# TSultanov/cfd-demo

Measured on AMD Instinct MI355X. Metric: cell-updates/s (Poisson iter) + ms/timestep, 4096² grid, 1/2/4/8 GPU, higher is better.
Workload: dtype f32

## Files before the change

cfd-demo_amd/cfdamd/__init__.py:

```python
from __future__ import annotations

import ctypes as C
import enum
from dataclasses import dataclass
from typing import List, Optional

import numpy as np

from . import _lib
from ._lib import (CFD_ENONFINITE, CfdError, CfdGrid, CfdParams, CfdResiduals, CfdState, check,
                   load)

__all__ = [
    "VelocityScheme", "InletProfile", "PressureSolver", "BoundaryKind", "Cylinder", "Grid",
    "SimulationParams", "Residuals", "SimSnapshot", "Model", "SimulationControlHandle",
    "CfdError", "default_grid", "cavity_grid", "rccl_unique_id", "device_count", "load", "LocalHub",
    "VisualizationMode", "CFD_ENONFINITE",
]


class VelocityScheme(enum.IntEnum):
    FirstOrder = 0
    SecondOrder = 1

# ... 222 lines not shown
        p = params._c()
        check("cfd_set_params", load().cfd_set_params(self._hh(), C.byref(p)))
        self.params = params

    def get_snapshot(self) -> SimSnapshot:
        su, sv, sp = self._sizes()
        u, v, p = (np.empty(n, np.float32) for n in (su, sv, sp))
        dt = C.c_float()
        check("cfd_get_snapshot",
              load().cfd_get_snapshot(self._hh(), _fp(u), _fp(v), _fp(p), C.byref(dt)))
        return SimSnapshot(p=p, u=u, v=v, dt=float(dt.value))

    def get_residuals(self) -> Residuals:
        r = CfdResiduals()
        check("cfd_get_residuals", load().cfd_get_residuals(self._hh(), C.byref(r)))
        return Residuals(int(r.simulation_step), float(r.simulation_time), float(r.dt),
                         float(r.p), float(r.u), float(r.v), float(r.step_time_s),
                         int(r.piso_substeps), int(r.jacobi_sweeps_total))

    def get_state(self) -> dict:
        su, sv, sp = self._sizes()
        arrs = {k: np.empty(n, np.float32) for k, n in
                (("u", su), ("v", sv), ("p", sp), ("u_star", su), ("v_star", sv),
                 ("p_prime", sp), ("rhs", sp))}
        st = CfdState(*(_fp(arrs[k]) for k in ("u", "v", "p", "u_star", "v_star", "p_prime",
                                               "rhs")))
        check("cfd_get_state", load().cfd_get_state(self._hh(), C.byref(st)))
        arrs.update(dt=np.float32(st.dt), simulation_time=np.float32(st.simulation_time),
                    simulation_step=int(st.simulation_step),
                    last_p_residual=np.float32(st.last_p_residual),
                    last_u_residual=np.float32(st.last_u_residual),
                    last_v_residual=np.float32(st.last_v_residual),
                    jacobi_sweeps_total=int(st.jacobi_sweeps_total))
        return arrs

    def set_state(self, **kw) -> None:
        cur = self.get_state()
        arrs = {}
        for k in ("u", "v", "p", "u_star", "v_star", "p_prime", "rhs"):
            a = kw.get(k, cur[k])
            arrs[k] = np.ascontiguousarray(a, dtype=np.float32)
            if arrs[k].size != cur[k].size:
                raise ValueError(f"{k}: expected {cur[k].size} values, got {arrs[k].size}")
        st = CfdState(*(_fp(arrs[k]) for k in ("u", "v", "p", "u_star", "v_star", "p_prime",
                                               "rhs")))
        st.dt = float(kw.get("dt", cur["dt"]))
        st.simulation_time = float(kw.get("simulation_time", cur["simulation_time"]))
        st.simulation_step = int(kw.get("simulation_step", cur["simulation_step"]))
        st.last_p_residual = float(kw.get("last_p_residual", cur["last_p_residual"]))
        st.last_u_residual = float(kw.get("last_u_residual", cur["last_u_residual"]))
        st.last_v_residual = float(kw.get("last_v_residual", cur["last_v_residual"]))
        st.jacobi_sweeps_total = int(kw.get("jacobi_sweeps_total", cur["jacobi_sweeps_total"]))
        check("cfd_set_state", load().cfd_set_state(self._hh(), C.byref(st)))

    def get_masks(self):
        su, sv, _ = self._sizes()
        mu, mv = np.empty(su, np.uint8), np.empty(sv, np.uint8)
        check("cfd_get_masks", load().cfd_get_masks(
            self._hh(), mu.ctypes.data_as(C.POINTER(C.c_uint8)),
            mv.ctypes.data_as(C.POINTER(C.c_uint8))))
        return mu, mv

    def profile_sweeps(self, n: int) -> float:
        ms = C.c_double()
        check("cfd_profile_sweeps", load().cfd_profile_sweeps(self._hh(), n, C.byref(ms)))
        return float(ms.value)

    def timing_begin(self) -> None:
        check("cfd_timing_begin", load().cfd_timing_begin(self._hh()))

    def timing_end(self):
        a, b, c, d = C.c_double(), C.c_uint64(), C.c_double(), C.c_uint64()
        check("cfd_timing_end", load().cfd_timing_end(self._hh(), C.byref(a), C.byref(b),
                                                      C.byref(c), C.byref(d)))
        return {"solve_ms": a.value, "sweeps": int(b.value), "step_ms": c.value,
                "steps": int(d.value)}

    def timing_phases(self, on: bool = True) -> None:
        check("cfd_timing_phases", load().cfd_timing_phases(self._hh(), 1 if on else 0))

    def timing_phase_ms(self) -> dict:
        a, b = C.c_double(), C.c_double()
        check("cfd_timing_phase_ms",
              load().cfd_timing_phase_ms(self._hh(), C.byref(a), C.byref(b)))
        return {"predict_ms": a.value, "finish_ms": b.value}

    def timing_exchange_ms(self) -> dict:
        a, n = C.c_double(), C.c_uint64()
        check("cfd_timing_exchange_ms",
              load().cfd_timing_exchange_ms(self._hh(), C.byref(a), C.byref(n)))
        return {"exchange_ms": a.value, "exchanges": int(n.value)}

    @property
    def kernel_config(self) -> dict:
        fd, tb = C.c_int(), C.c_int()
        check("cfd_get_kernel_config",
              load().cfd_get_kernel_config(self._hh(), C.byref(fd), C.byref(tb)))
        return {"fastdiv": fd.value, "temporal": tb.value}

    def render(self, mode: "VisualizationMode" = VisualizationMode.Pressure):
        img = np.empty((self.nyl, self.grid.nx, 4), np.uint8)
        mm = np.empty(2, np.float32)
        check("cfd_render", load().cfd_render(
            self._hh(), int(mode), img.ctypes.data_as(C.POINTER(C.c_uint8)), _fp(mm)))
        return img, (float(mm[0]), float(mm[1]))

    def derive_field(self, mode: "VisualizationMode"):
        out = np.empty((self.nyl, self.grid.nx), np.float32)
        mm = np.empty(2, np.float32)
        check("cfd_derive_field", load().cfd_derive_field(self._hh(), int(mode), _fp(out), _fp(mm)))
        return out, (float(mm[0]), float(mm[1]))

    def launches_per_solve(self) -> int:
        tmax = self.kernel_config["temporal"]
        iters = self.params.jacobi_iters
        hg = self.halo_depth if self.n_ranks > 1 else 0
        T, lo, hi, ex = C.c_int(), C.c_int(), C.c_int(), C.c_int()
        it = n = 0
        while it < iters:
            check("cfd_plan_block", load().cfd_plan_block(
                self.j0, self.nyl, self.grid.ny, hg, it, tmax, iters, C.byref(T), C.byref(lo),
                C.byref(hi), C.byref(ex)))
            it += T.value
            n += 1
        return n

    @property
    def jacobi_kernel(self) -> dict:
        kind, name = C.c_int(), C.create_string_buffer(96)
        check("cfd_get_jacobi_kernel",
              load().cfd_get_jacobi_kernel(self._hh(), C.byref(kind), name, 96))
        return {"kind": kind.value, "name": name.value.decode()}

    def jacobi_geometry(self, persist: bool = True) -> dict:
        v = [C.c_int32() for _ in range(4)]
        check("cfd_get_jacobi_geometry",
              load().cfd_get_jacobi_geometry(self._hh(), int(bool(persist)), *(C.byref(x) for x in v)))
        return dict(lds_pad=v[0].value, wgs_per_cu=v[1].value, wave_cols=v[2].value,
                    segments=v[3].value)

    @property
    def persist_steals(self) -> int:
        n = C.c_uint64()
        check("cfd_get_persist_steals", load().cfd_get_persist_steals(self._hh(), C.byref(n)))
        return int(n.value)

    @property
    def persist_sums(self) -> int:
        n = C.c_uint64()
        check("cfd_get_persist_sums", load().cfd_get_persist_sums(self._hh(), C.byref(n)))
        return int(n.value)

    @property
    def comm_calls(self) -> int:
        n = C.c_uint64()
        check("cfd_get_comm_calls", load().cfd_get_comm_calls(self._hh(), C.byref(n)))
        return int(n.value)

    @property
    def recoveries(self) -> int:
        n = C.c_uint64()
        check("cfd_get_recoveries", load().cfd_get_recoveries(self._hh(), C.byref(n)))
        return int(n.value)

    @property
    def resident_solves(self) -> int:
        n = C.c_uint64()
        check("cfd_get_resident_solves", load().cfd_get_resident_solves(self._hh(), C.byref(n)))
        return int(n.value)

    @property
    def persist_blocks(self) -> int:
        n = C.c_int()
        check("cfd_get_persist_blocks", load().cfd_get_persist_blocks(self._hh(), C.byref(n)))
        return n.value

    @property
    def comm_size(self) -> int:
        n = C.c_int()
        check("cfd_get_comm_size", load().cfd_get_comm_size(self._hh(), C.byref(n)))
        return int(n.value)

    @property
    def halo_depth(self) -> int:
        return int(load().cfd_get_halo_depth(self._hh()))

    def run(self) -> "SimulationControlHandle":
        return SimulationControlHandle(self)

    def _hh(self):
        if self._runner is not None:
            raise CfdError("Model", -4, "the model is owned by a running SimulationControlHandle; "
                                        "stop() it first")
        return self._h

    def close(self) -> None:
        r = getattr(self, "_runner", None)
        if r is not None:
            r.stop()
        if getattr(self, "_h", None) and self._h.value:
            load().cfd_destroy(self._h)
            self._h = C.c_void_p()

    def __del__(self):
        try:
            self.close()
        except Exception:
            pass


class SimulationControlHandle:

    def __init__(self, model: Model):
        self._model = model
        self._r = C.c_void_p()
        check("cfd_run_start", load().cfd_run_start(model._hh(), C.byref(self._r)))
        model._runner = self

    def _live(self):
        if not self._r.value:
            raise CfdError("cfd_run", -4, "runner stopped")
        return self._r

    def stop(self):
        if self._r.value:
            check("cfd_run_stop", load().cfd_run_stop(self._r))
            self._r = C.c_void_p()
            if self._model._runner is self:
                self._model._runner = None

    def join(self, timeout=None):
        self.stop()

    def status(self):
        buf = C.create_string_buffer(256)
        rc = load().cfd_run_status(self._live(), buf, 256)
        return rc, buf.value.decode()

    @property
    def steps(self) -> int:
        return int(load().cfd_run_steps(self._live()))

    def get_last_available_snapshot(self) -> Optional[SimSnapshot]:
        su, sv, sp = self._model._sizes()
        u, v, p = (np.empty(n, np.float32) for n in (su, sv, sp))
        dt, paused, avail = C.c_float(), C.c_int(), C.c_int()
        check("cfd_run_last_snapshot", load().cfd_run_last_snapshot(
            self._live(), _fp(u), _fp(v), _fp(p), C.byref(dt), C.byref(paused), C.byref(avail)))
        if not avail.value:
            return None
        return SimSnapshot(p=p, u=u, v=v, dt=float(dt.value), paused=bool(paused.value))

    def get_new_log_messages(self) -> List[Residuals]:
        out: List[Residuals] = []
        buf = (CfdResiduals * 256)()
        n = C.c_int()
        while True:
            check("cfd_run_new_residuals",
                  load().cfd_run_new_residuals(self._live(), buf, 256, C.byref(n)))
            for r in buf[:n.value]:
                out.append(Residuals(int(r.simulation_step), float(r.simulation_time),
                                     float(r.dt), float(r.p), float(r.u), float(r.v),
                                     float(r.step_time_s), int(r.piso_substeps),
                                     int(r.jacobi_sweeps_total)))
            if n.value < 256:
                return out

    def request_snapshot(self):
        check("cfd_run_request_snapshot", load().cfd_run_request_snapshot(self._live()))

    def set_params(self, params: SimulationParams):
        p = params._c()
        check("cfd_run_set_params", load().cfd_run_set_params(self._live(), C.byref(p)))
        self._model.params = params

    def pause(self):
        check("cfd_run_pause", load().cfd_run_pause(self._live()))

    def resume(self):
        check("cfd_run_resume", load().cfd_run_resume(self._live()))

    def __del__(self):
        try:
            self.stop()
        except Exception:
            pass
```

cfd-demo_amd/cfdamd/_lib.py:

```python
from __future__ import annotations

import ctypes as C
import os

PKG_DIR = os.path.dirname(os.path.abspath(__file__))
ROOT = os.path.dirname(PKG_DIR)
LIB_PATH = os.environ.get("CFD_LIB") or os.path.join(ROOT, "lib", "libcfd_amd.so")

EXPORTS = [
    "cfd_default_params", "cfd_default_grid", "cfd_create", "cfd_rccl_unique_id",
    "cfd_create_sharded", "cfd_local_hub_create", "cfd_local_hub_destroy",
    "cfd_create_sharded_local", "cfd_device_count", "cfd_get_comm_size", "cfd_get_slab", "cfd_update", "cfd_update_n", "cfd_piso_step",
    "cfd_pressure_solve", "cfd_run_phase", "cfd_set_params", "cfd_get_snapshot",
    "cfd_get_residuals", "cfd_get_state", "cfd_set_state", "cfd_get_masks", "cfd_synchronize",
    "cfd_profile_sweeps", "cfd_timing_begin", "cfd_timing_end", "cfd_timing_phases",
    "cfd_timing_phase_ms", "cfd_timing_exchange_ms", "cfd_get_halo_depth",
    "cfd_get_kernel_config", "cfd_get_jacobi_kernel", "cfd_get_persist_blocks", "cfd_get_persist_steals", "cfd_get_persist_sums", "cfd_get_recoveries", "cfd_get_comm_calls", "cfd_get_resident_solves", "cfd_get_jacobi_geometry", "cfd_plan_slab", "cfd_plan_sweep", "cfd_plan_halo", "cfd_plan_block", "cfd_plan_overlap",
    "cfd_render", "cfd_derive_field", "cfd_last_error", "cfd_abi_version", "cfd_destroy",
    "cfd_get_config", "cfd_run_start", "cfd_run_stop", "cfd_run_pause", "cfd_run_resume",
    "cfd_run_set_params", "cfd_run_request_snapshot", "cfd_run_last_snapshot",
    "cfd_run_new_residuals", "cfd_run_status", "cfd_run_steps",
    "cfd_polygon_new", "cfd_polygon_new_rect", "cfd_polygon_new_regular", "cfd_polygon_add_hole",
    "cfd_polygon_contains_point", "cfd_polygon_intersects_aabb",
    "cfd_polygon_edges_intersect_aabb", "cfd_polygon_bounding_box",
    "cfd_polygon_bounding_square", "cfd_polygon_edges", "cfd_polygon_destroy",
    "cfd_geom_do_intersect", "cfd_geom_segment_intersection", "cfd_geom_intersect_quad_edge",
    "cfd_tesselate", "cfd_quadtree_size", "cfd_quadtree_nodes", "cfd_quadtree_destroy",
    "cfd_mesh_from_quadtree", "cfd_mesh_sizes", "cfd_mesh_cells", "cfd_mesh_neighbors",
    "cfd_mesh_intersections", "cfd_mesh_full_bounding_box", "cfd_mesh_build_ms",
    "cfd_mesh_destroy",
]


class CfdGrid(C.Structure):
    _fields_ = [("nx", C.c_uint64), ("ny", C.c_uint64), ("lx", C.c_float), ("ly", C.c_float),
                ("has_cylinder", C.c_int32), ("cylinder_x", C.c_float),
                ("cylinder_y", C.c_float), ("cylinder_radius", C.c_float)]


class CfdParams(C.Structure):
    _fields_ = [("dt", C.c_float), ("viscosity", C.c_float),
                ("target_inlet_velocity", C.c_float), ("velocity_scheme", C.c_int32),
                ("inlet_profile", C.c_int32), ("pressure_solver", C.c_int32),
                ("jacobi_iters", C.c_int32), ("corrector_passes", C.c_int32),
                ("tol_enabled", C.c_int32), ("p_tol", C.c_float), ("bc_kind", C.c_int32)]


class CfdResiduals(C.Structure):
    _fields_ = [("simulation_step", C.c_uint64), ("simulation_time", C.c_float),
                ("dt", C.c_float), ("p", C.c_float), ("u", C.c_float), ("v", C.c_float),
                ("step_time_s", C.c_double), ("piso_substeps", C.c_uint32),
                ("jacobi_sweeps_total", C.c_uint64)]


FP = C.POINTER(C.c_float)


class CfdState(C.Structure):
    _fields_ = [("u", FP), ("v", FP), ("p", FP), ("u_star", FP), ("v_star", FP),
                ("p_prime", FP), ("rhs", FP), ("dt", C.c_float), ("simulation_time", C.c_float),
                ("simulation_step", C.c_uint64), ("last_p_residual", C.c_float),
                ("last_u_residual", C.c_float), ("last_v_residual", C.c_float),
                ("jacobi_sweeps_total", C.c_uint64)]


class CfdPoint(C.Structure):
    _fields_ = [("x", C.c_double), ("y", C.c_double)]


class CfdAabb(C.Structure):
    _fields_ = [("center", CfdPoint), ("half_width", C.c_double), ("half_height", C.c_double)]


CFD_EINVAL, CFD_EHIP, CFD_ERCCL, CFD_ESTATE, CFD_ENONFINITE, CFD_ETIMEOUT = -1, -2, -3, -4, -5, -6


class CfdError(RuntimeError):
    def __init__(self, fn: str, code: int, msg: str):
        super().__init__(f"{fn} failed ({code}): {msg}")
        self.code = code


_lib = None


def load():
    global _lib
    if _lib is not None:
        return _lib
    if not os.path.exists(LIB_PATH):
        raise RuntimeError(
            f"HIP library {LIB_PATH} not built: run `make -C {ROOT}` "
            "(or __graft_entry__.build()). There is no CPU fallback.")
    L = C.CDLL(LIB_PATH)
    vp, i32, f32 = C.c_void_p, C.c_int, C.c_float
    sig = {
        "cfd_default_params": (None, [C.POINTER(CfdParams)]),
        "cfd_default_grid": (None, [C.POINTER(CfdGrid)]),
        "cfd_create": (i32, [C.POINTER(CfdGrid), C.POINTER(CfdParams), i32, C.POINTER(vp)]),
        "cfd_rccl_unique_id": (i32, [C.c_char_p]),
        "cfd_create_sharded": (i32, [C.POINTER(CfdGrid), C.POINTER(CfdParams), i32, i32, i32,
                                     C.c_char_p, C.POINTER(vp)]),
        "cfd_local_hub_create": (vp, [i32]),
        "cfd_local_hub_destroy": (None, [vp]),
        "cfd_create_sharded_local": (i32, [C.POINTER(CfdGrid), C.POINTER(CfdParams), i32, i32,
                                           i32, vp, C.POINTER(vp)]),
        "cfd_device_count": (i32, [C.POINTER(i32)]),
        "cfd_get_comm_size": (i32, [vp, C.POINTER(i32)]),
        "cfd_get_slab": (i32, [vp, C.POINTER(C.c_uint64), C.POINTER(C.c_uint64)]),
        "cfd_update": (i32, [vp]),
        "cfd_update_n": (i32, [vp, i32]),
        "cfd_piso_step": (i32, [vp, f32]),
        "cfd_pressure_solve": (i32, [vp, FP]),
        "cfd_run_phase": (i32, [vp, i32, f32]),
        "cfd_set_params": (i32, [vp, C.POINTER(CfdParams)]),
        "cfd_get_snapshot": (i32, [vp, FP, FP, FP, FP]),
        "cfd_get_residuals": (i32, [vp, C.POINTER(CfdResiduals)]),
        "cfd_get_state": (i32, [vp, C.POINTER(CfdState)]),
        "cfd_set_state": (i32, [vp, C.POINTER(CfdState)]),
        "cfd_get_masks": (i32, [vp, C.POINTER(C.c_uint8), C.POINTER(C.c_uint8)]),
        "cfd_synchronize": (i32, [vp]),
        "cfd_profile_sweeps": (i32, [vp, i32, C.POINTER(C.c_double)]),
        "cfd_timing_begin": (i32, [vp]),
        "cfd_timing_end": (i32, [vp, C.POINTER(C.c_double), C.POINTER(C.c_uint64),
                                 C.POINTER(C.c_double), C.POINTER(C.c_uint64)]),
        "cfd_timing_phases": (i32, [vp, i32]),
        "cfd_timing_phase_ms": (i32, [vp, C.POINTER(C.c_double), C.POINTER(C.c_double)]),
        "cfd_timing_exchange_ms": (i32, [vp, C.POINTER(C.c_double), C.POINTER(C.c_uint64)]),
        "cfd_get_halo_depth": (i32, [vp]),
        "cfd_get_kernel_config": (i32, [vp, C.POINTER(i32), C.POINTER(i32)]),
        "cfd_get_jacobi_kernel": (i32, [vp, C.POINTER(i32), C.c_char_p, C.c_size_t]),
        "cfd_get_persist_blocks": (i32, [vp, C.POINTER(i32)]),
        "cfd_get_persist_steals": (i32, [vp, C.POINTER(C.c_uint64)]),
        "cfd_get_persist_sums": (i32, [vp, C.POINTER(C.c_uint64)]),
        "cfd_get_recoveries": (i32, [vp, C.POINTER(C.c_uint64)]),
        "cfd_get_comm_calls": (i32, [vp, C.POINTER(C.c_uint64)]),
        "cfd_get_resident_solves": (i32, [vp, C.POINTER(C.c_uint64)]),
        "cfd_get_jacobi_geometry": (i32, [vp, i32, C.POINTER(i32), C.POINTER(i32), C.POINTER(i32),
                                          C.POINTER(i32)]),
        "cfd_plan_slab": (i32, [C.c_uint64, i32, i32, C.POINTER(C.c_uint64),
                                C.POINTER(C.c_uint64)]),
        "cfd_plan_sweep": (i32, [i32, i32, i32, i32, i32, i32, C.POINTER(i32), C.POINTER(i32),
                                 C.POINTER(i32)]),
        "cfd_plan_halo": (i32, [i32, i32, i32, i32, i32, C.POINTER(i32)]),
        "cfd_plan_overlap": (i32, [i32, i32, i32, i32, i32, i32, C.POINTER(i32)]),
        "cfd_plan_block": (i32, [i32, i32, i32, i32, i32, i32, i32, C.POINTER(i32),
                                 C.POINTER(i32), C.POINTER(i32), C.POINTER(i32)]),
        "cfd_render": (i32, [vp, i32, C.POINTER(C.c_uint8), FP]),
        "cfd_derive_field": (i32, [vp, i32, FP, FP]),
        "cfd_last_error": (C.c_char_p, []),
        "cfd_abi_version": (i32, []),
        "cfd_destroy": (None, [vp]),
        "cfd_get_config": (i32, [vp, C.POINTER(CfdGrid), C.POINTER(CfdParams)]),
        "cfd_run_start": (i32, [vp, C.POINTER(vp)]),
        "cfd_run_stop": (i32, [vp]),
        "cfd_run_pause": (i32, [vp]),
        "cfd_run_resume": (i32, [vp]),
        "cfd_run_set_params": (i32, [vp, C.POINTER(CfdParams)]),
        "cfd_run_request_snapshot": (i32, [vp]),
        "cfd_run_last_snapshot": (i32, [vp, FP, FP, FP, FP, C.POINTER(i32), C.POINTER(i32)]),
        "cfd_run_new_residuals": (i32, [vp, C.POINTER(CfdResiduals), i32, C.POINTER(i32)]),
        "cfd_run_status": (i32, [vp, C.c_char_p, C.c_size_t]),
        "cfd_run_steps": (C.c_uint64, [vp]),
        "cfd_polygon_new": (i32, [C.POINTER(CfdPoint), C.c_size_t, C.POINTER(C.c_uint64),
                                  C.c_size_t, C.POINTER(vp), C.POINTER(i32)]),
        "cfd_polygon_new_rect": (i32, [C.c_double] * 4 + [C.POINTER(vp)]),
        "cfd_polygon_new_regular": (i32, [CfdPoint, C.c_double, C.c_size_t, C.c_double,
                                          C.POINTER(vp)]),
        "cfd_polygon_add_hole": (i32, [vp, vp, C.POINTER(i32)]),
        "cfd_polygon_contains_point": (i32, [vp, CfdPoint, C.POINTER(i32)]),
        "cfd_polygon_intersects_aabb": (i32, [vp, C.POINTER(CfdAabb), C.POINTER(i32)]),
        "cfd_polygon_edges_intersect_aabb": (i32, [vp, C.POINTER(CfdAabb), C.POINTER(i32)]),
        "cfd_polygon_bounding_box": (i32, [vp, C.POINTER(CfdAabb)]),
        "cfd_polygon_bounding_square": (i32, [vp, C.POINTER(CfdAabb)]),
        "cfd_polygon_edges": (i32, [vp, C.POINTER(CfdPoint), C.c_size_t, C.POINTER(C.c_size_t)]),
        "cfd_polygon_destroy": (None, [vp]),
        "cfd_geom_do_intersect": (i32, [CfdPoint] * 4 + [C.POINTER(i32)]),
        "cfd_geom_segment_intersection": (i32, [CfdPoint] * 4 + [C.POINTER(CfdPoint),
                                                                 C.POINTER(i32)]),
        "cfd_geom_intersect_quad_edge": (i32, [CfdPoint, C.c_double, C.c_double, CfdPoint,
                                               CfdPoint, C.POINTER(CfdPoint), C.POINTER(i32)]),
        "cfd_tesselate": (i32, [vp, C.c_double, C.c_double, C.POINTER(vp)]),
        "cfd_quadtree_size": (i32, [vp, C.POINTER(C.c_uint64), C.POINTER(C.c_uint64)]),
        "cfd_quadtree_nodes": (i32, [vp, C.POINTER(CfdAabb), C.POINTER(C.c_int64)]),
        "cfd_quadtree_destroy": (None, [vp]),
        "cfd_mesh_from_quadtree": (i32, [vp, vp, i32, C.POINTER(vp)]),
        "cfd_mesh_sizes": (i32, [vp, C.POINTER(C.c_uint64)]),
        "cfd_mesh_cells": (i32, [vp] + [C.POINTER(C.c_double)] * 4),
        "cfd_mesh_neighbors": (i32, [vp, i32, C.POINTER(C.c_uint64), C.POINTER(C.c_uint64)]),
        "cfd_mesh_intersections": (i32, [vp, C.POINTER(C.c_uint64), C.POINTER(CfdPoint)]),
        "cfd_mesh_full_bounding_box": (i32, [vp, C.POINTER(CfdAabb)]),
        "cfd_mesh_build_ms": (i32, [vp, C.POINTER(C.c_double)]),
        "cfd_mesh_destroy": (None, [vp]),
    }
    for name, (res, args) in sig.items():
        if os.environ.get("CFD_LIB") and not hasattr(L, name):
            continue
        fn = getattr(L, name)
        fn.restype = res
        fn.argtypes = args
    _lib = L
    return L


def check(fn: str, rc: int):
    if rc != 0:
        msg = load().cfd_last_error()
        raise CfdError(fn, rc, msg.decode() if msg else "")
```

cfd-demo_amd/csrc/cfd_device.h:

```cpp
#pragma once
#include "cfd_internal.h"

#include <algorithm>

namespace cfd {
namespace {

inline int cdiv(long a, long b) { return (int)((a + b - 1) / b); }


constexpr int kBlock = 256;
typedef unsigned int u32x4 __attribute__((ext_vector_type(4)));

__device__ __forceinline__ float dt_of(const Ctl *c, float dt_override) {
    return __builtin_isnan(dt_override) ? c->dt : dt_override;
}

__device__ __forceinline__ bool pass_off(const Ctl *c, int pass) {
    return pass >= 0 && c->go[pass] == 0;
}

__device__ __forceinline__ float wave_max(float m) {
#pragma unroll
    for (int o = 32; o > 0; o >>= 1) m = fmaxf(m, __shfl_xor(m, o, 64));
    return m;
}

__device__ __forceinline__ void publish_max(uint32_t *set, int key, float m) {
    if (m > 0.0f) atomicMax(&set[(key & (kResSlots - 1)) * kResStride], __float_as_uint(m));
}

__device__ __forceinline__ bool nonfinite(float x) { return !(fabsf(x) <= 3.40282347e38f); }
__device__ __forceinline__ void flag_nonfinite(Ctl *c, bool bad) {
    if (bad) atomicOr(&c->red[4], 1u);
}

__device__ __forceinline__ float read_max(const uint32_t *set, uint32_t base) {
    const int lane = (int)threadIdx.x & 63;
    const float v = lane < kResSlots ? __uint_as_float(set[lane * kResStride]) : 0.0f;
    return fmaxf(wave_max(v), __uint_as_float(base));
}

__device__ __forceinline__ int xcd_block(const Geom &g) {
    const int b = (int)blockIdx.x, G = (int)gridDim.x;
    if (!g.xcd_remap) return b;
    const int per = G >> 3;
    if (b >= (per << 3)) return b;
    return (b & 7) * per + (b >> 3);
}

__device__ __forceinline__ float from_left(float x) {
    return __builtin_bit_cast(
        float, __builtin_amdgcn_update_dpp(0, __builtin_bit_cast(int, x), 0x138, 0xf, 0xf, true));
}
__device__ __forceinline__ float from_right(float x) {
    return __builtin_bit_cast(
        float, __builtin_amdgcn_update_dpp(0, __builtin_bit_cast(int, x), 0x130, 0xf, 0xf, true));
}

constexpr float kDivGuardMin = 0x1p-96f;
template <int FAST>
__device__ __forceinline__ float fdiv(float x, float c, float r) {
    if (FAST == 1) return x * r;
    if (FAST == 2) {
        const float q0 = x * r;
        const float q = __builtin_fmaf(__builtin_fmaf(-q0, c, x), r, q0);
        return __builtin_isfinite(q0) ? q : q0;
    }
    if (FAST == 3) {
        const float q0 = x * r;
        const float qc = __builtin_fmaf(__builtin_fmaf(-q0, c, x), r, q0);
        float q = __builtin_isfinite(q0) && x != 0.0f ? qc : q0;
        const bool ok = __builtin_fabsf(x) >= kDivGuardMin || x == 0.0f;
        if (__builtin_expect(!__all(ok), 0)) q = ok ? q : x / c;
        return q;
    }
    return x / c;
}

template <int SP>
__device__ __forceinline__ float sdiv(float x, float c, float r) {
    return SP ? x * r : x / c;
}

typedef float f2 __attribute__((ext_vector_type(2)));

template <int FAST>
__device__ __forceinline__ f2 fdiv2(f2 x, float c, float r) {
    if (FAST == 1) return x * r;
    return (f2){fdiv<FAST>(x.x, c, r), fdiv<FAST>(x.y, c, r)};
}

__device__ __forceinline__ void solve_finalize_body(const Geom &g, const Fields &f, int pass,
                                                    int iters, int check_break, int flips,
                                                    int exact_flips) {
    Ctl *c = f.ctl;
    __shared__ int go_s;
    const int k_lo = g.tol_enabled ? 0 : (iters > 0 ? iters - 1 : 0);
    const int wv = (int)threadIdx.x >> 6, nw = (int)blockDim.x >> 6;
    for (int k = k_lo + wv; k < iters; k += nw) {
        uint32_t *set = f.err_slots + (size_t)k * kResSlots * kResStride;
        const float v = read_max(set, c->err[k]);
        if ((threadIdx.x & 63) < kResSlots) set[(threadIdx.x & 63) * kResStride] = 0u;
        if ((threadIdx.x & 63) == 0) c->err[k] = __float_as_uint(v);
    }
    __syncthreads();
    if (threadIdx.x == 0) {
        const int go = pass < 0 ? 1 : c->go[pass];
        if (go) {
            int n = iters;
            if (g.tol_enabled && iters > 0) {
                n = 1;
                while (n < iters && !(__uint_as_float(c->err[n - 1]) < g.p_tol)) ++n;
            }
            const float res = n > 0 ? __uint_as_float(c->err[n - 1]) : 0.0f;
            c->cur = (c->cur + (exact_flips == 2 ? c->spec_launches
                                : (g.tol_enabled && !exact_flips) ? n : flips)) & 1;
            c->last_p = res;
            c->red[5] = __float_as_uint(res);
            c->n_exec_last = (uint32_t)n;
            c->sweeps_total += (uint64_t)n;
        }
        if (pass >= 0 && pass + 1 <= kMaxPasses)
            c->go[pass + 1] = (go && !(check_break && g.tol_enabled && c->last_p < g.p_tol)) ? 1 : 0;
        if (exact_flips >= 2) c->spec_stop = c->spec_redo = c->spec_launch = c->spec_launches = 0;
        go_s = go;
    }
    __syncthreads();
    if (go_s)
        for (int k = threadIdx.x; k < iters; k += blockDim.x) c->err[k] = 0u;
}

template <int FAST>
__device__ __forceinline__ float4 jacobi_row4(const float4 &B, const float4 &C, const float4 &T,
                                              const float4 &Rh, float L0, float R3, float dx_sq,
                                              float dy_sq, float denom, float r_dx_sq,
                                              float r_dy_sq, float r_denom) {
    const f2 c01 = {C.x, C.y}, c23 = {C.z, C.w};
    const f2 h01 = __builtin_shufflevector(c01, c01, 1, 0) + (f2){L0, C.z};
    const f2 h23 = __builtin_shufflevector(c23, c23, 1, 0) + (f2){C.y, R3};
    const f2 v01 = (f2){T.x, T.y} + (f2){B.x, B.y};
    const f2 v23 = (f2){T.z, T.w} + (f2){B.z, B.w};
    const f2 hz01 = fdiv2<FAST>(h01, dx_sq, r_dx_sq), hz23 = fdiv2<FAST>(h23, dx_sq, r_dx_sq);
    const f2 vt01 = fdiv2<FAST>(v01, dy_sq, r_dy_sq), vt23 = fdiv2<FAST>(v23, dy_sq, r_dy_sq);
    const f2 pu01 = fdiv2<FAST>(hz01 + vt01 - (f2){Rh.x, Rh.y}, denom, r_denom);
    const f2 pu23 = fdiv2<FAST>(hz23 + vt23 - (f2){Rh.z, Rh.w}, denom, r_denom);
    const float omega = 0.75f;
    const float om1 = 1.0f - omega;
    const f2 n01 = omega * pu01 + om1 * c01;
    const f2 n23 = omega * pu23 + om1 * c23;
    return make_float4(n01.x, n01.y, n23.x, n23.y);
}

}
}
```

cfd-demo_amd/csrc/cfd_internal.h:

```cpp
#pragma once
#include <hip/hip_runtime.h>
#include <stdint.h>

#include "../../include/cfd.h"

namespace cfd {

constexpr int kGhostUV = 2;
constexpr int kMaxSweeps = 4096;
constexpr int kMaxPasses = 64;

constexpr int kResSlots = 32;
constexpr int kResStride = 16;
constexpr int kPersistFlagStride = 16;
constexpr int kPersistHeadLines = 21;
constexpr int kPersistBlockBits = 10;
static_assert((1 << kPersistBlockBits) > kMaxSweeps / 8, "persistent flag layout");
constexpr int kPersistMaxGroups = 16384;
constexpr size_t kPersistWords = (size_t)(kPersistMaxGroups + kPersistHeadLines) * kPersistFlagStride;
constexpr size_t kSlotWords = (size_t)(kMaxSweeps + 16) * kResSlots * kResStride + kPersistWords;

struct Ctl {
    float dt;
    float time;
    uint32_t step;
    float inlet;
    int32_t cur;
    uint32_t n_exec_last;
    float last_p;
    float res_u, res_v;
    uint32_t red[7];
    uint32_t nonfinite_step;
    uint32_t vis[2];
    uint32_t done;
    uint64_t sweeps_total;
    int32_t spec_stop, spec_redo, spec_launch, spec_launches;
    uint32_t spec_done;
    int32_t go[kMaxPasses + 1];
    uint32_t err[kMaxSweeps];
};

struct Geom {
    int32_t nx, ny;
    int32_t j0, nyl;
    int32_t hg;
    float dx, dy, nu, ly;
    float target_inlet;
    int32_t scheme, profile, bc_kind;
    int32_t tol_enabled;
    float p_tol;
    int32_t jacobi_iters;
    float dx_sq, dy_sq, denom;
    float r_dx_sq, r_dy_sq, r_denom;
    int32_t fastdiv;
    int32_t tb_rows;
    int32_t tb_bpc;
    int32_t n_cu;
    int32_t tb_kind;
    int32_t xcd_remap;
    float r_dx, r_dy, r_dxx, r_dyy;
    int32_t sp_pow2;
    int32_t pred_div;
    int32_t res_div;
};

struct Fields {
    float *u, *v, *u_old, *v_old, *u_star, *v_star;
    float *p, *rhs;
    float *pp[2];
    const uint8_t *mask_u, *mask_v;
    const int32_t *obs;
    uint32_t *err_slots;
    uint32_t *red_slots;
    uint32_t *vis_slots;
    int32_t n_obs;
    int32_t any_pmask;
    size_t u_alloc, v_alloc;
    float *u_alloc_base, *v_alloc_base, *u_old_base, *v_old_base, *u_star_base, *v_star_base;
    Ctl *ctl;
    uint32_t *host_nonfinite;
    uint32_t *host_progress;
    uint32_t *persist;
};

void launch_step_begin(const Geom &g, const Fields &f, int copy, hipStream_t s);
void launch_copy_star(const Geom &g, const Fields &f, int pass, hipStream_t s);
void launch_copy_star_div(const Geom &g, const Fields &f, int pass, float dt_override,
                          hipStream_t s);
void launch_u_predictor(const Geom &g, const Fields &f, float dt_override, hipStream_t s);
void launch_v_predictor(const Geom &g, const Fields &f, float dt_override, hipStream_t s);
void launch_predict(const Geom &g, const Fields &f, float dt_override, hipStream_t s);
bool predict_div_fused(const Geom &g, const Fields &f);
void launch_predict_div(const Geom &g, const Fields &f, float dt_override, hipStream_t s);
bool predict_march_ok(const Geom &g, const Fields &f);
void launch_predict_march(const Geom &g, const Fields &f, float dt_override, hipStream_t s,
                          bool set_inlet = false, int row_lo = 0, int row_hi = -1);
void launch_divergence(const Geom &g, const Fields &f, int pass, float dt_override,
                       hipStream_t s);
void launch_jacobi_sweep(const Geom &g, const Fields &f, int pass, int it, int row_lo,
                         int row_hi, int res, hipStream_t s);
void launch_jacobi_block(const Geom &g, const Fields &f, int pass, int it, int par, int T,
                         int out_lo, int out_hi, int res, hipStream_t s);
bool launch_jacobi_persist(const Geom &g, const Fields &f, int pass, int par0, int nblk,
                           int out_lo, int out_hi, uint32_t epoch, int res_it, hipStream_t s);
void lds_geometry8(const Geom &g, int out_lo, int out_hi, bool persist, int *pad, int *occ, int *nwc,
                   int *nseg);
void launch_tb1(const Geom &g, const Fields &f, int T, int pass, int it, int par, int out_lo,
                int out_hi, uint32_t *res_slots, hipStream_t s);
void launch_pipe4(const Geom &g, const Fields &f, int T, int pass, int it, int par, int out_lo,
                  int out_hi, uint32_t *res_slots, hipStream_t s);
void launch_pipe2(const Geom &g, const Fields &f, int T, int pass, int it, int par, int out_lo,
                  int out_hi, uint32_t *res_slots, hipStream_t s);
bool launch_lds_persist8(const Geom &g, const Fields &f, int pass, int par0, int nblk, int out_lo,
                         int out_hi, uint32_t epoch, uint32_t *rs, hipStream_t s);
void launch_lds(const Geom &g, const Fields &f, int T, int pass, int it, int par, int out_lo,
                int out_hi, uint32_t *res_slots, hipStream_t s, int mode = 0, int lag = 0);
void launch_jacobi_spec(const Geom &g, const Fields &f, int pass, int it, int par, int T,
                        int out_lo, int out_hi, hipStream_t s, int lag = 0);
void launch_spec_check(const Geom &g, const Fields &f, int pass, int it, int T, int par,
                       hipStream_t s);
bool launch_jacobi_resident(const Geom &g, const Fields &f, int pass, int iters, int fin,
                            int check_break, hipStream_t s);
bool jacobi_resident_geometry(const Geom &g, int *br, int *bc, int *tiles, int *wgs);
void launch_spec_align(const Geom &g, const Fields &f, int pass, int n, hipStream_t s);
void launch_jacobi_redo(const Geom &g, const Fields &f, int pass, int out_lo, int out_hi,
                        hipStream_t s, int last_it = 0, int last_par = 0, int last_T = 0);
void launch_fold_slots(uint32_t *dst, uint32_t *slots, int n, hipStream_t s);
void launch_vis_field(const Geom &g, const Fields &f, int mode, float *out, uint32_t *slots,
                      hipStream_t s);
void launch_vis_color(const Geom &g, const Fields &f, int mode, const float *field, uint32_t *px,
                      const uint32_t *keys, int has_cyl, float cx, float cy, float radius,
                      hipStream_t s);
void launch_verify_division(float c, float r, unsigned long long *dev_counts, hipStream_t s);
void launch_finalize_solve(const Geom &g, const Fields &f, int pass, int iters, int check_break,
                           int flips, hipStream_t s, int exact_flips = 0);

struct SorConst {
    double dx2, dy2, denom;
    double r_dx2, r_dy2, r_denom;
    int32_t fast;
};
struct MgLevel {
    float *a, *b, *rhs, *r;
    int32_t nx, ny;
    double dx2, dy2, denom;
    double r_dx2, r_dy2, r_denom;
    int32_t fast;
    int32_t ys, ye;
    int32_t lo, hi;
};
constexpr int kMgMaxLevels = 40;
void launch_sor_color(float *pp, const float *rhs, int nx, int ny, const SorConst &k, int color,
                      Ctl *ctl, uint32_t *err_slots, int pass, int it, int tol, float p_tol, int res,
                      hipStream_t s);
bool sor_fused_ok(int nx, int nrows);
void launch_sor_fused(float *pa, float *pb, const float *rhs, int nx, int ny, const SorConst &k,
                      Ctl *ctl, uint32_t *err_slots, int pass, int it, int tol, float p_tol, int res,
                      int row_lo, int row_hi, int j0, int lo_clamp, int hi_clamp, hipStream_t s);
void launch_fill_zero(float *p, size_t n, const Ctl *ctl, int pass, hipStream_t s);
void launch_mg_smooth(const MgLevel &L, const float *src, float *dst, const Ctl *ctl, int pass,
                      hipStream_t s);
void launch_mg_smooth5(const MgLevel &L, const float *src, float *dst, const Ctl *ctl, int pass,
                       hipStream_t s);
bool mg_smooth_wave_form();
void launch_mg_prolong_smooth5(const MgLevel &Cl, const float *e, const MgLevel &L, const float *src,
                               float *dst, const Ctl *ctl, int pass, hipStream_t s);
void launch_mg_smooth5_residual(const MgLevel &L, const float *src, float *dst, const Ctl *ctl,
                                int pass, hipStream_t s);
void launch_mg_residual(const MgLevel &L, const float *p, const Ctl *ctl, int pass, hipStream_t s);
void launch_mg_restrict(const MgLevel &F, const MgLevel &Cl, const Ctl *ctl, int pass, hipStream_t s);
void launch_mg_prolong_add(const MgLevel &Cl, const float *e, const MgLevel &F, float *p,
                           const Ctl *ctl, int pass, hipStream_t s);
void launch_mg_tail(const MgLevel *dev_levels, int s_level, int coarsest, float *a0, float *b0,
                    int fast, const Ctl *ctl, int pass, hipStream_t s);
void launch_mg_final_residual(const MgLevel &L, const float *p, uint32_t *slots, const Ctl *ctl,
                              int pass, hipStream_t s);
void launch_corrector(const Geom &g, const Fields &f, int pass, float dt_override,
                      hipStream_t s);
void launch_boundary(const Geom &g, const Fields &f, hipStream_t s);
void launch_correct_finish(const Geom &g, const Fields &f, float dt_override, hipStream_t s);
void launch_step_reduce(const Geom &g, const Fields &f, hipStream_t s);
bool correct_head_ok(const Geom &g, const Fields &f);
void launch_correct_head(const Geom &g, const Fields &f, int pass, float dt_override, bool has_next,
                         hipStream_t s);
void launch_step_finalize(const Geom &g, const Fields &f, hipStream_t s);
void launch_abort_to_red(const Fields &f, hipStream_t s);
void launch_abort_from_red(const Fields &f, hipStream_t s);

constexpr int kJacRowsPerWave = 16;
constexpr int kMaxTemporal = 8;
constexpr int kTbRowsPerWave = 32;
constexpr int kJacWavesPerBlock = 4;

}
```

cfd-demo_amd/csrc/cfd_jacobi_lds.h:

```cpp
#pragma once
#include <cmath>
#include <type_traits>

#include "cfd_device.h"

namespace cfd {
namespace {

constexpr int kLdsWaves = 4;
#ifndef CFD_LDS_SB
#define CFD_LDS_SB 0
#endif
#ifndef CFD_LDS_PD
#define CFD_LDS_PD 3
#endif
#ifndef CFD_LDS_DIAG
#define CFD_LDS_DIAG 0
#endif
#ifndef CFD_LDS_WPE
#define CFD_LDS_WPE 0
#endif
typedef unsigned int u32x2 __attribute__((ext_vector_type(2)));
#ifndef CFD_LDS_PRIO
#define CFD_LDS_PRIO 1
#endif
#ifndef CFD_LDS_COMPACT
#define CFD_LDS_COMPACT 0
#endif
#ifndef CFD_LDS_STAMP
#define CFD_LDS_STAMP 0
#endif
#if CFD_LDS_STAMP
constexpr int kStampWaves = 1 << 15;
__device__ unsigned long long g_lds_stamp[kStampWaves * 4];
#endif

#ifndef CFD_LDS_ST_AUX
#define CFD_LDS_ST_AUX 16
#endif

#ifndef CFD_LDS_LD_AUX
#define CFD_LDS_LD_AUX 0
#endif

#ifndef CFD_LDS_HOIST
#define CFD_LDS_HOIST 0
#endif

#ifndef CFD_LDS_SPLIT
#define CFD_LDS_SPLIT 1
#endif
constexpr int lds_gcd(int a, int b) { return b == 0 ? a : lds_gcd(b, a % b); }
constexpr int lds_off(int s, int T, int G) { return s <= 0 ? 0 : ((s - 1) * G) / T; }
constexpr int lds_nw(int G) { return G > 1 ? 4 : 3; }
constexpr int ring_depth(int T, int PD, int G) {
    const int nw = lds_nw(G);
    const int q = nw / lds_gcd(nw, PD) * PD;
    const int need = T + lds_off(T, T, G) + 1;
    return ((need + q - 1) / q) * q;
}

template <int T, int FAST, int MODE, bool SUMS = false>
struct LdsMarch {
    static constexpr bool RES = MODE == 1 || MODE == 5, SPEC = MODE == 2, REDO = MODE == 3;
    static constexpr bool PERSIST = MODE == 4 || MODE == 5;
#ifndef CFD_PROBE_NOTRACK
#define CFD_PROBE_NOTRACK 0
#endif
    static constexpr bool TRACK_IN = PERSIST && !SUMS && !CFD_PROBE_NOTRACK;
    static constexpr bool TRACK_OUT = PERSIST && !CFD_PROBE_NOTRACK;
    static_assert(!SUMS || FAST == 1, "SUMS: reciprocal multiply");
    static constexpr int PLD_AUX = PERSIST ? 16 : CFD_LDS_LD_AUX;
    static constexpr int PST_AUX = PERSIST ? 16 : CFD_LDS_ST_AUX;
    static constexpr int G = CFD_LDS_SPLIT;
    static constexpr int NW = lds_nw(G);
    static constexpr int PD = CFD_LDS_PD;
    static constexpr int OFFT = lds_off(T, T, G);
    static constexpr int D = ring_depth(T, PD, G);
    static constexpr int U = D;
    static constexpr int WARM = 2 * T + OFFT;
    static constexpr int H = (T + 1) / 2;
    static constexpr int OUTL = 64 - 2 * H;
    static constexpr int off(int s) { return lds_off(s, T, G); }
    static constexpr int start(int s) { return 2 * s + off(s); }
    static_assert(D % PD == 0 && D % NW == 0 && D >= T + OFFT + 1, "ring geometry");
    static_assert(G >= 1 && G <= T, "stage groups");

    f2 W[T][NW];
    f2 PQ[PD];
    f2 RQ[PD];
    f2 *ring;
    int lane;
    int k_first, S, lo_clamp, hi_clamp, nch, g_first, g_last, g_top, g_zero, row_bytes;
    int wbase;
    int ch, vo_ld, vo_st, abase, dir;
    bool e0, e1;
    float dx_sq, r_dx_sq, dy_sq, r_dy_sq, denom, r_denom;
    __amdgpu_buffer_rsrc_t rs_p, rs_r, rs_d;
    float m;
    float omax, imax, rmax;
    float mm[SPEC ? T : 1];
    int r0v, r1v;
    int nst;
    int nyl_;

    LdsMarch() = default;

    __device__ __forceinline__ int act(int vrow) const { return abase + dir * vrow; }

    template <int AUX = 0>
    __device__ __forceinline__ f2 ld(__amdgpu_buffer_rsrc_t rs, int vrow) const {
        if (CFD_LDS_DIAG & 1) return (f2){__int_as_float(vo_ld + vrow), 1.0f};
        vrow = vrow < k_first + S ? vrow : k_first + S - 1;
        int row = act(vrow);
        row = row < lo_clamp ? lo_clamp : (row > hi_clamp ? hi_clamp : row);
        const u32x2 v = __builtin_amdgcn_raw_buffer_load_b64(rs, vo_ld, (row - wbase) * row_bytes, AUX);
        return (f2){__uint_as_float(v.x), __uint_as_float(v.y)};
    }
    __device__ __forceinline__ void st(const f2 &x, int row) const {
        if (CFD_LDS_DIAG & 4) {
            asm volatile("" ::"v"(x.x), "v"(x.y));
            return;
        }
        const u32x2 v = {__float_as_uint(x.x), __float_as_uint(x.y)};
        __builtin_amdgcn_raw_buffer_store_b64(v, rs_d, vo_st, (row - wbase) * row_bytes, PST_AUX);
    }

    __device__ __forceinline__ f2 update(const f2 &B, const f2 &C, const f2 &Tp, const f2 &Rh) const {
        const float hx = C.y + from_left(C.y);
        const float hy = C.x + from_right(C.x);
        const f2 h = {hx, hy};
        const f2 v = Tp + B;
        f2 s;
        if constexpr (SUMS) {
            s = (h + v) * r_dx_sq;
        } else {
            const f2 hz = fdiv2<FAST>(h, dx_sq, r_dx_sq);
            const f2 vt = fdiv2<FAST>(v, dy_sq, r_dy_sq);
            s = hz + vt;
        }
        const f2 pu = fdiv2<FAST>(s - Rh, denom, r_denom);
        const float omega = 0.75f;
        const float om1 = 1.0f - omega;
        return omega * pu + om1 * C;
    }

    static constexpr int kCol = 1, kRow = 2;

    template <int E>
    __device__ __forceinline__ f2 stage(const f2 &B, const f2 &C, const f2 &Tp, const f2 &Rh) const {
        f2 o = update(B, C, Tp, Rh);
        if (E & kCol) {
            if (ch == 0) o.x = o.y;
            if (ch == nch - 1) o.y = 0.0f;
        }
        return o;
    }

    template <int V_, int GUARD, int E>
    __device__ __forceinline__ void slot(int v) {
        if ((GUARD == 2 || GUARD == 3) && v >= S) return;
        if (CFD_LDS_SB >= 1) __builtin_amdgcn_sched_barrier(0);
        const int k = k_first + v;
        W[0][V_ % NW] = PQ[V_ % PD];
        PQ[V_ % PD] = ld<PLD_AUX>(rs_p, k + PD);
        if (!(CFD_LDS_DIAG & 2))
            ring[(V_ % D) * 64 + lane] = RQ[V_ % PD];
        RQ[V_ % PD] = ld(rs_r, k + PD);
        f2 rhv[T];
        if (CFD_LDS_HOIST && !(CFD_LDS_DIAG & 2)) {
#pragma unroll
            for (int s = 1; s <= T; ++s) rhv[s - 1] = ring[((V_ - s - off(s) + 8 * D) % D) * 64 + lane];
        }
#pragma unroll
        for (int s = 1; s <= T; ++s) {
            if (GUARD == 0 && V_ < start(s)) continue;
            if (GUARD == 3 && v < start(s)) continue;
            if (CFD_LDS_SB >= 2 && s > 1) __builtin_amdgcn_sched_barrier(0);
            const int r = k - s - off(s);
            const f2 rh = (CFD_LDS_DIAG & 2) ? RQ[(V_ + s) % PD]
                                             : (CFD_LDS_HOIST ? rhv[s - 1]
                                                              : ring[((V_ - s - off(s) + 8 * D) % D) * 64 + lane]);
            constexpr int kW = 4 * NW;
            const int dl = off(s) - off(s - 1);
            const f2 &B = W[s - 1][(V_ - dl - 2 + kW) % NW];
            const f2 &C = W[s - 1][(V_ - dl - 1 + kW) % NW];
            const f2 &Tp = W[s - 1][(V_ - dl + kW) % NW];
            if (REDO && s > nst) continue;
            if constexpr (TRACK_IN) {
                if (s == 1) {
                    imax = fmaxf(fmaxf(imax, fabsf(Tp.x)), fabsf(Tp.y));
                    rmax = fmaxf(fmaxf(rmax, fabsf(rh.x)), fabsf(rh.y));
                }
            }
            f2 n = stage<E>(B, C, Tp, rh);
            if constexpr (SPEC) {
                bool in_seg;
                if constexpr (!(E & kRow))
                    in_seg = true;
                else if constexpr (GUARD == 0)
                    in_seg = V_ - s - T >= 0 && v - s - T < r1v - r0v;
                else
                    in_seg = v - s - T >= 0 && v - s - T < r1v - r0v;
                if (in_seg) {
                    const f2 d = n - C;
                    if (!(E & kCol)) {
                        mm[s - 1] = fmaxf(fmaxf(mm[s - 1], fabsf(d.x)), fabsf(d.y));
                    } else {
                        if (e0) mm[s - 1] = fmaxf(mm[s - 1], fabsf(d.x));
                        if (e1) mm[s - 1] = fmaxf(mm[s - 1], fabsf(d.y));
                    }
                }
            }
            if (REDO && s == nst) {
                if (r >= r0v && r < r1v) {
                    const int ra = act(r);
                    st(n, ra);
                    if ((E & kRow) && r == g_first) st(n, g_zero);
                    if ((E & kRow) && r == g_last) st(n, g_top);
                }
            } else if (s < T) {
                if ((E & kRow) && r == g_top) n = W[s][(V_ - 1 + kW) % NW];
                W[s][V_ % NW] = n;
                if ((E & kRow) && r == g_first) W[s][(V_ - 1 + kW) % NW] = n;
            } else {
                const int ra = act(r);
                if (RES && ra >= 0 && ra < nyl_) {
                    const f2 d = n - C;
                    if (!(E & kCol)) {
                        m = fmaxf(fmaxf(m, fabsf(d.x)), fabsf(d.y));
                    } else {
                        if (e0) m = fmaxf(m, fabsf(d.x));
                        if (e1) m = fmaxf(m, fabsf(d.y));
                    }
                }
                st(n, ra);
                if ((E & kRow) && r == g_first) st(n, g_zero);
                if ((E & kRow) && r == g_last) st(n, g_top);
#ifndef CFD_PROBE_NOOMAX
#define CFD_PROBE_NOOMAX 0
#endif
                if constexpr (TRACK_OUT && !CFD_PROBE_NOOMAX)
                    omax = fmaxf(fmaxf(omax, fabsf(n.x)), fabsf(n.y));
            }
        }
    }

    template <int V_, int E>
    __device__ __forceinline__ void warmup() {
        if constexpr (V_ < WARM) {
            slot<V_, 0, E>(V_);
            warmup<V_ + 1, E>();
        }
    }

    template <int J, int GUARD, int E, int OFF = WARM>
    __device__ __forceinline__ void group(int base) {
        if constexpr (J < U) {
            slot<OFF + J, GUARD, E>(base + J);
            group<J + 1, GUARD, E, OFF>(base);
        }
    }

    __device__ __forceinline__ void set_prio(int done) const {
        if (!CFD_LDS_PRIO) return;
        const int rows = S - WARM, d4 = 4 * done;
        if (d4 >= 3 * rows)
            __builtin_amdgcn_s_setprio(0);
        else if (d4 >= 2 * rows)
            __builtin_amdgcn_s_setprio(1);
        else if (d4 >= rows)
            __builtin_amdgcn_s_setprio(2);
        else
            __builtin_amdgcn_s_setprio(3);
    }

    template <int E>
    __device__ __forceinline__ void run() {
        if (CFD_LDS_COMPACT) {
            static_assert(2 * U >= WARM, "warm-up fits two groups");
            set_prio(0);
            group<0, 3, E, 0>(0);
            group<0, 3, E, 0>(U);
            int base = 2 * U;
            for (; base + U <= S; base += U) {
                set_prio(base - WARM);
                group<0, 1, E, 0>(base);
            }
            set_prio(base - WARM);
            if (base < S) group<0, 3, E, 0>(base);
            return;
        }
        set_prio(0);
        warmup<0, E>();
        int base = WARM;
        const int full_end = WARM + ((S - WARM) / U) * U;
        for (; base < full_end; base += U) {
            set_prio(base - WARM);
            group<0, 1, E>(base);
        }
        set_prio(base - WARM);
        if (base < S) group<0, 2, E>(base);
    }
};

template <int T, int FAST, int MODE, bool SUMS = false>
__device__ __forceinline__ void lds_block(const Geom &g, float *__restrict__ pa,
                                          float *__restrict__ pb, const float *__restrict__ rhs,
                                          Ctl *ctl, uint32_t *res_slots, int par, int out_lo,
                                          int out_hi, int nwc, int nseg, int wlo, int whi, f2 *lds,
                                          int nst, int bid, float *trk = nullptr) {
    using M = LdsMarch<T, FAST, MODE, SUMS>;
    constexpr bool RES = M::RES;
    M w;
    w.nst = nst;
    const int wave = __builtin_amdgcn_readfirstlane((int)threadIdx.x >> 6);
    const int lane = (int)threadIdx.x & 63;
    if (M::PERSIST && trk && lane == 0) trk[3 * wave] = trk[3 * wave + 1] = trk[3 * wave + 2] = 0.0f;
    const int wc = bid % nwc;
    const int seg = (bid / nwc) * kLdsWaves + wave;
    const int nrows = out_hi - out_lo;
    if (seg >= nseg) return;
    const long total = nseg == 1 ? 16 : wlo + whi + 16L * (nseg - 2);
    auto cum = [&](int i) -> long { return i <= 0 ? 0 : (i >= nseg ? total : wlo + 16L * (i - 1)); };
    const int r0 = out_lo + (int)(cum(seg) * nrows / total);
    const int r1 = out_lo + (int)(cum(seg + 1) * nrows / total);
    if (r0 >= r1) return;
    const int nx = g.nx;
    w.ring = lds + wave * M::D * 64;
    w.lane = lane;
    w.nch = nx / 2;
    w.nyl_ = g.nyl;
    w.lo_clamp = -g.hg;
    w.hi_clamp = g.nyl + g.hg - 1;
    w.ch = wc * M::OUTL - M::H + lane;
    const bool in_dom = w.ch >= 0 && w.ch < w.nch;
    const bool out_lane = in_dom && lane >= M::H && lane < 64 - M::H;
    const int col = 2 * w.ch;
    w.row_bytes = nx * 4;
    constexpr int kFar = 0x7FFF0000;
    w.vo_ld = in_dom ? col * 4 : kFar;
    w.vo_st = out_lane ? col * 4 : kFar;
    const int si = (ctl->cur + par) & 1;
    float *src_alloc = si ? pb : pa;
    float *dst_alloc = si ? pa : pb;
    const int wb = max(w.lo_clamp, r0 - T - 1), wt = min(w.hi_clamp, r1 + T);
    w.wbase = wb;
    const long woff = (long)(wb - w.lo_clamp) * nx;
    const int wbytes = (wt - wb + 1) * nx * 4;
    w.rs_p = __builtin_amdgcn_make_buffer_rsrc(src_alloc + woff, 0, wbytes, 0x00020000);
    w.rs_d = __builtin_amdgcn_make_buffer_rsrc(dst_alloc + woff, 0, wbytes, 0x00020000);
    w.rs_r = __builtin_amdgcn_make_buffer_rsrc((void *)(rhs - (long)g.hg * nx + woff), 0, wbytes,
                                               0x00020000);
    w.dx_sq = g.dx_sq;
    w.r_dx_sq = g.r_dx_sq;
    w.dy_sq = g.dy_sq;
    w.r_dy_sq = g.r_dy_sq;
    w.denom = g.denom;
    w.r_denom = g.r_denom;
    w.e0 = out_lane && col >= 1 && col <= nx - 8;
    w.e1 = out_lane && col + 1 >= 1 && col + 1 <= nx - 8;
    w.g_first = 1 - g.j0;
    w.g_last = g.ny - 2 - g.j0;
    w.g_top = g.ny - 1 - g.j0;
    w.g_zero = -g.j0;
    w.m = 0.0f;
    w.omax = w.imax = w.rmax = 0.0f;
#pragma unroll
    for (int s = 0; s < (M::SPEC ? T : 1); ++s) w.mm[s] = 0.0f;
    w.r0v = r0;
    w.r1v = r1;
    w.k_first = r0 - T;
    w.S = (r1 - r0) + M::WARM;
    w.abase = 0;
    w.dir = 1;
    const f2 z = {0.0f, 0.0f};
#pragma unroll
    for (int s = 0; s < T; ++s)
#pragma unroll
        for (int q = 0; q < M::NW; ++q) w.W[s][q] = z;
    const int ch_lo = wc * M::OUTL - M::H, ch_hi = ch_lo + 63;
    const bool col_edge = ch_lo <= 0 || 2 * (ch_hi + 1) > nx - 8;
    const int lo_row = w.k_first - 2, hi_row = r1 + T + M::OFFT + 2;
    auto hits = [&](int r) { return r >= lo_row && r <= hi_row; };
    const bool row_edge = hits(w.g_zero) || hits(w.g_first) || hits(w.g_last) || hits(w.g_top);
    const bool edge = col_edge || row_edge;
    if (!edge && (seg & 1)) {
        w.abase = r0 + r1 - 1;
        w.dir = -1;
    }
#pragma unroll
    for (int q = 0; q < M::PD; ++q) {
        w.PQ[q] = w.template ld<M::PLD_AUX>(w.rs_p, w.k_first + q);
        w.RQ[q] = w.ld(w.rs_r, w.k_first + q);
    }
    if (row_edge)
        w.template run<M::kCol | M::kRow>();
    else if (col_edge)
        w.template run<M::kCol>();
    else
        w.template run<0>();
    if (M::PERSIST && trk) {
        const float o = wave_max(out_lane ? w.omax : 0.0f);
        const float im = M::TRACK_IN ? wave_max(w.imax) : 0.0f;
        const float rm = M::TRACK_IN ? wave_max(w.rmax) : 0.0f;
        if (lane == 0) {
            trk[3 * wave] = o;
            trk[3 * wave + 1] = im;
            trk[3 * wave + 2] = rm;
        }
    }
    if (M::SPEC) {
#pragma unroll
        for (int s = 0; s < T; ++s) {
            const float ms = wave_max(out_lane ? w.mm[s] : 0.0f);
            if (lane == 0 && ms > 0.0f)
                atomicMax(res_slots + (size_t)s * kResSlots * kResStride +
                              ((bid * kLdsWaves + wave) & (kResSlots - 1)) * kResStride,
                          __float_as_uint(ms));
        }
    }
    if (!RES) return;
    const float m = wave_max(out_lane ? w.m : 0.0f);
    if (lane == 0) publish_max(res_slots, bid * kLdsWaves + wave, m);
}

#ifndef CFD_LDS_SPEC_WPE
#define CFD_LDS_SPEC_WPE 5
#endif
constexpr int lds_min_waves(int mode) {
    return mode == 2 ? CFD_LDS_SPEC_WPE : (CFD_LDS_WPE > 0 ? CFD_LDS_WPE : 1);
}
__device__ __forceinline__ int spec_lag_first(const Geom &g, Ctl *ctl, const uint32_t *set0, int it0,
                                              int T, int lpar, bool stop = true) {
    __shared__ float e_s[kMaxTemporal];
    const int wv = (int)threadIdx.x >> 6;
    for (int s = wv; s < T; s += kLdsWaves) {
        const float v = read_max(set0 + (size_t)s * kResSlots * kResStride, ctl->err[it0 + s]);
        if ((threadIdx.x & 63) == 0) e_s[s] = v;
    }
    __syncthreads();
    int j = 0;
    while (j < T && !(e_s[j] < g.p_tol)) ++j;
    if (blockIdx.x == 0 && threadIdx.x == 0) {
        ctl->spec_launches = lpar + 1;
        if (stop && j < T) {
            ctl->spec_stop = 1;
            ctl->spec_launch = lpar;
            ctl->spec_redo = j + 1 < T ? j + 1 : 0;
        }
    }
    return j;
}

template <int T, int FAST, int MODE>
__global__ __launch_bounds__(kLdsWaves * 64, lds_min_waves(MODE)) void k_jacobi_lds(
    Geom g, float *__restrict__ pa, float *__restrict__ pb, const float *__restrict__ rhs,
    Ctl *ctl, uint32_t *res_slots, int pass, int par, int out_lo, int out_hi, int nwc, int nseg,
    int wlo, int whi, int it, int lag) {
    using M = LdsMarch<T, FAST, MODE>;
    [[maybe_unused]] constexpr bool RES = M::RES;
    __shared__ f2 lds[kLdsWaves * M::D * 64];
#if CFD_LDS_STAMP
    const unsigned long long st_rt0 = __builtin_amdgcn_s_memrealtime();
    const unsigned long long st_t0 = __builtin_amdgcn_s_memtime();
    struct StampOnExit {
        unsigned long long rt0, t0;
        unsigned long long bid;
        __device__ ~StampOnExit() {
            if (RES) return;
            const unsigned long long rt1 = __builtin_amdgcn_s_memrealtime();
            const unsigned long long t1 = __builtin_amdgcn_s_memtime();
            const unsigned hw = __builtin_amdgcn_s_getreg(4 | (31 << 11));
            const unsigned xcc = __builtin_amdgcn_s_getreg(20 | (31 << 11));
            const int idx = (int)blockIdx.x * kLdsWaves + ((int)threadIdx.x >> 6);
            if ((threadIdx.x & 63) == 0 && idx < kStampWaves) {
                g_lds_stamp[idx * 4 + 0] = rt0;
                g_lds_stamp[idx * 4 + 1] = rt1;
                g_lds_stamp[idx * 4 + 2] = (bid << 40) | ((t1 - t0) & 0xFFFFFFFFFFull);
                g_lds_stamp[idx * 4 + 3] = ((unsigned long long)xcc << 32) | hw;
            }
        }
    } stamp_guard{st_rt0, st_t0, (unsigned long long)xcd_block(g)};
#endif
    if (pass_off(ctl, pass)) return;
    int nst = 0;
    if constexpr (M::SPEC) {
        if (lag > 0) {
            __shared__ int stop_s;
            if (threadIdx.x == 0) stop_s = ctl->spec_stop;
            __syncthreads();
            if (stop_s) return;
            if (spec_lag_first(g, ctl, res_slots - (size_t)lag * kResSlots * kResStride, it - lag, lag,
                               par - 1) < lag)
                return;
        } else if (ctl->spec_stop) {
            return;
        }
    }
    if constexpr (M::REDO) {
        if (lag > 0 && !ctl->spec_stop) {
            const int j = spec_lag_first(g, ctl, res_slots, it, lag, par, false);
            nst = j + 1 < lag ? j + 1 : 0;
        } else {
            nst = ctl->spec_redo;
            par = ctl->spec_launch;
        }
        if (nst <= 0) return;
    }
    lds_block<T, FAST, MODE>(g, pa, pb, rhs, ctl, res_slots, par, out_lo, out_hi, nwc, nseg, wlo,
                             whi, lds, nst, xcd_block(g));
}

constexpr int kStealDepth = 16;
#ifndef CFD_PERSIST_WPE
#define CFD_PERSIST_WPE 3
#endif
template <int T, int FAST>
__global__ __launch_bounds__(kLdsWaves * 64, CFD_PERSIST_WPE) void k_jacobi_persist(
    Geom g, float *__restrict__ pa, float *__restrict__ pb, const float *__restrict__ rhs,
    Ctl *ctl, uint32_t *persist, uint32_t *host_fail, uint32_t *res_slots, uint32_t epoch, int pass,
    int par0, int nblk, int out_lo, int out_hi, int nwc, int nseg, int wlo, int whi, int ngrp,
    int acq, uint32_t deadline, uint32_t steal, int late, int sums, float plim, float rlim) {
    using M = LdsMarch<T, FAST, 4>;
    __shared__ f2 lds[kLdsWaves * M::D * 64];
    __shared__ int run_tile_s, run_blk_s, abort_s, own_next_s, sp_s, fast_s;
    __shared__ int stk_tile[kStealDepth], stk_blk[kStealDepth];
    __shared__ float trk_s[3 * kLdsWaves], own_im_s[2], own_rm_s;
    __shared__ int own_ok_s[2], nfast_s;
    if (pass_off(ctl, pass)) return;
    const int ntiles = ngrp * nwc;
    const int own = xcd_block(g);
    if (own >= ntiles) return;
    const unsigned base = epoch << kPersistBlockBits;
    uint32_t *lines = persist + kPersistHeadLines * kPersistFlagStride;
    const int lane = (int)threadIdx.x & 63;
    auto count = [&](unsigned v) -> int { return v < base ? 0 : (int)(v - base); };
    auto claim = [&](int t, unsigned v, bool all) -> int {
        uint32_t *w = lines + (size_t)t * kPersistFlagStride + 1;
        for (;;) {
            const int c = count(v);
            if (c >= nblk) return -1;
            unsigned exp = v;
            if (__hip_atomic_compare_exchange_strong(w, &exp, base + (unsigned)(all ? nblk : c + 1),
                                                     __ATOMIC_RELAXED, __ATOMIC_RELAXED,
                                                     __HIP_MEMORY_SCOPE_AGENT))
                return c;
            if (!all) return -1;
            v = exp;
        }
    };
    if (threadIdx.x == 0) {
        sp_s = 0;
        own_next_s = -2;
        own_ok_s[0] = own_ok_s[1] = 0;
        own_im_s[0] = own_im_s[1] = own_rm_s = 0.0f;
        nfast_s = 0;
        abort_s = __hip_atomic_load(persist + 1, __ATOMIC_RELAXED, __HIP_MEMORY_SCOPE_AGENT) != 0;
        if (late > 0 && own % late == 1) {
            const uint64_t t0 = __builtin_amdgcn_s_memrealtime();
            while (__builtin_amdgcn_s_memrealtime() - t0 < 200000u) __builtin_amdgcn_s_sleep(127);
        }
    }
    __syncthreads();
    if (abort_s) return;
    for (;;) {
        if (threadIdx.x < 64) {
            int sp = sp_s, run_t = -1, run_b = -1;
            bool fail = false, fast = false;
            if (sp == 0) {
                int nb = own_next_s;
                if (nb == -2) {
                    int c = -1;
                    if (lane == 0) c = claim(own, 0u, true);
                    nb = __builtin_amdgcn_readfirstlane(c);
                }
                if (nb >= 0) {
                    if (lane == 0) {
                        stk_tile[0] = own;
                        stk_blk[0] = nb;
                    }
                    sp = 1;
                }
                own_next_s = -1;
            }
            while (sp > 0) {
                __builtin_amdgcn_fence(__ATOMIC_RELEASE, "workgroup");
                const int tt = stk_tile[sp - 1], bb = stk_blk[sp - 1];
                if (bb == 0) {
                    run_t = tt, run_b = bb;
                    --sp;
                    break;
                }
                const int wc = tt % nwc, gi = tt / nwc;
                const int c = wc + lane % 3 - 1, r = gi + lane / 3 - 1;
                const bool nbr = lane < 9 && c >= 0 && c < nwc && r >= 0 && r < ngrp;
                const int nt = nbr ? r * nwc + c : -1;
                const uint32_t *w = nbr ? lines + (size_t)nt * kPersistFlagStride
                                        : (lane == 9 ? persist + 1 : nullptr);
                const unsigned want = base + (unsigned)bb;
                const uint64_t t0 = __builtin_amdgcn_s_memrealtime();
                bool ready = false, pushed = false;
                for (;;) {
                    const unsigned v = w ? __hip_atomic_load(w, __ATOMIC_RELAXED, __HIP_MEMORY_SCOPE_AGENT)
                                         : 0u;
                    const bool ok = lane < 9 ? (!nbr || v >= want) : v == 0u;
                    if (__all(ok)) {
                        ready = true;
                        break;
                    }
                    const uint64_t el = __builtin_amdgcn_s_memrealtime() - t0;
                    if (__any(lane == 9 && v != 0u) || el > (uint64_t)deadline) {
                        fail = true;
                        break;
                    }
                    if (el > (uint64_t)steal && sp < kStealDepth) {
                        const unsigned cw = nbr && v < want
                                                ? __hip_atomic_load(w + 1, __ATOMIC_RELAXED,
                                                                    __HIP_MEMORY_SCOPE_AGENT)
                                                : 0u;
                        const bool cand = nbr && v < want && count(cw) < bb;
                        const uint64_t m = __ballot(cand);
                        if (m) {
                            const int l = __builtin_ctzll(m);
                            const int st = __shfl(nt, l, 64);
                            const unsigned sv = __shfl(cw, l, 64);
                            int got = -1;
                            if (lane == 0) {
                                got = claim(st, sv, false);
                                if (got >= 0)
                                    __hip_atomic_fetch_add(persist + 2, 1u, __ATOMIC_RELAXED,
                                                           __HIP_MEMORY_SCOPE_AGENT);
                            }
                            got = __builtin_amdgcn_readfirstlane(got);
                            if (got >= 0) {
                                if (lane == 0) {
                                    stk_tile[sp] = st;
                                    stk_blk[sp] = got;
                                }
                                ++sp;
                                pushed = true;
                                break;
                            }
                        }
                    }
                    __builtin_amdgcn_s_sleep(2);
                }
                if (fail) break;
                if (pushed) continue;
                if (ready) {
                    run_t = tt, run_b = bb;
                    --sp;
                    if (acq) {
                        __builtin_amdgcn_fence(__ATOMIC_ACQUIRE, "agent");
                        asm volatile("s_waitcnt vmcnt(0)" ::: "memory");
                    } else {
                        __builtin_amdgcn_fence(__ATOMIC_ACQUIRE, "wavefront");
                    }
                    if (sums && tt == own && bb >= 2 && own_ok_s[bb & 1] && own_rm_s < rlim &&
                        own_im_s[bb & 1] < plim) {
                        float mo = 0.0f;
                        if (nbr) {
                            const uint32_t *q = w + 2 + 4 * ((bb - 1) & 1);
#pragma unroll
                            for (int k = 0; k < kLdsWaves; ++k)
                                mo = fmaxf(mo, __uint_as_float(__hip_atomic_load(
                                                   q + k, __ATOMIC_RELAXED, __HIP_MEMORY_SCOPE_AGENT)));
                        }
                        fast = wave_max(mo) < plim;
                    }
                    break;
                }
            }
            if (lane == 0) {
                sp_s = sp;
                run_tile_s = run_t;
                run_blk_s = run_b;
                fast_s = fast;
                abort_s = fail;
                if (fail) {
                    __hip_atomic_store(persist + 1, 1u, __ATOMIC_RELAXED, __HIP_MEMORY_SCOPE_AGENT);
                    if (host_fail)
                        __hip_atomic_store(host_fail, 1u, __ATOMIC_RELAXED, __HIP_MEMORY_SCOPE_SYSTEM);
                }
            }
        }
        __syncthreads();
        const int tile = run_tile_s, b = run_blk_s;
        if (abort_s || tile < 0) {
            if (threadIdx.x == 0 && nfast_s)
                __hip_atomic_fetch_add(persist + 3, (uint32_t)nfast_s, __ATOMIC_RELAXED,
                                       __HIP_MEMORY_SCOPE_AGENT);
            return;
        }
        const bool fast = fast_s;
        const bool res = res_slots && b == nblk - 1;
#ifndef CFD_PROBE_NOSUMS
#define CFD_PROBE_NOSUMS 0
#endif
        if constexpr (FAST == 1 && !CFD_PROBE_NOSUMS) {
            if (fast) {
                if (res)
                    lds_block<T, FAST, 5, true>(g, pa, pb, rhs, ctl, res_slots, par0 + b, out_lo, out_hi,
                                                nwc, nseg, wlo, whi, lds, 0, tile, trk_s);
                else
                    lds_block<T, FAST, 4, true>(g, pa, pb, rhs, ctl, nullptr, par0 + b, out_lo, out_hi,
                                                nwc, nseg, wlo, whi, lds, 0, tile, trk_s);
            }
        }
        if (!fast) {
            if (res)
                lds_block<T, FAST, 5>(g, pa, pb, rhs, ctl, res_slots, par0 + b, out_lo, out_hi, nwc,
                                      nseg, wlo, whi, lds, 0, tile, trk_s);
            else
                lds_block<T, FAST, 4>(g, pa, pb, rhs, ctl, nullptr, par0 + b, out_lo, out_hi, nwc,
                                      nseg, wlo, whi, lds, 0, tile, trk_s);
        }
        if (sums && lane == 0) {
            const int wv = (int)threadIdx.x >> 6;
            __hip_atomic_store(lines + (size_t)tile * kPersistFlagStride + 2 + 4 * (b & 1) + wv,
                               __float_as_uint(trk_s[3 * wv]), __ATOMIC_RELAXED, __HIP_MEMORY_SCOPE_AGENT);
        }
        asm volatile("s_waitcnt vmcnt(0)" ::: "memory");
        __syncthreads();
        if (threadIdx.x == 0) {
            if (tile == own) {
                own_next_s = b + 1 < nblk ? b + 1 : -1;
                if (fast) {
                    ++nfast_s;
                } else {
                    float im = 0.0f, rm = 0.0f;
#pragma unroll
                    for (int k = 0; k < kLdsWaves; ++k) {
                        im = fmaxf(im, trk_s[3 * k + 1]);
                        rm = fmaxf(rm, trk_s[3 * k + 2]);
                    }
                    own_im_s[b & 1] = fmaxf(own_im_s[b & 1], im);
                    own_ok_s[b & 1] = 1;
                    own_rm_s = fmaxf(own_rm_s, rm);
                }
            }
            __hip_atomic_store(lines + (size_t)tile * kPersistFlagStride, base + (unsigned)b + 1u,
                               __ATOMIC_RELAXED, __HIP_MEMORY_SCOPE_AGENT);
        }
    }
}

inline int lds_pad_bytes(const Geom &g, int mode) {
    static const int forced = [] {
        const char *e = getenv("CFD_LDS_PAD");
        return e ? std::max(0, std::min(64 * 1024, atoi(e))) : -1;
    }();
    if (forced >= 0) return forced;
    constexpr uint64_t kMallResident = 200ull << 20;
    const uint64_t ws = 3ull * (uint64_t)g.nyl * (uint64_t)g.nx * 4u;
    return mode <= 1 && ws <= kMallResident ? 24 * 1024 : 0;
}
template <int T, int FAST, int MODE>
int lds_blocks_per_cu(int pad) {
    static int cache[2] = {0, 0};
    int &nb = cache[pad > 0 ? 1 : 0];
    if (nb == 0) {
        int n = 0;
        if (hipOccupancyMaxActiveBlocksPerMultiprocessor(
                &n, reinterpret_cast<const void *>(&k_jacobi_lds<T, FAST, MODE>), kLdsWaves * 64, pad) !=
                hipSuccess ||
            n < 1)
            n = 1;
        nb = n;
    }
    return nb;
}

template <int T, int FAST, int MODE>
int lds_segments(const Geom &g, int nrows, int nwc, int pad, int occ_override = 0) {
    if (g.tb_rows > 0) return cdiv(nrows, g.tb_rows);
    constexpr int kMaxRows = 160, kMinRows = 8;
    const int bpc = occ_override > 0 ? occ_override : lds_blocks_per_cu<T, FAST, MODE>(pad);
    const int wgs_per_col = std::max(1, g.n_cu * bpc / nwc);
    const int per_round = kLdsWaves * wgs_per_col;
    const int rounds =
        occ_override > 0 ? 1 : std::max(1, cdiv(nrows, (long)per_round * kMaxRows));
    return std::max(1, std::min(per_round * rounds, nrows / kMinRows));
}

template <int T, int MODE>
void launch_lds_t(const Geom &g, const Fields &f, int pass, int par, int it, int out_lo, int out_hi,
                  uint32_t *rs, hipStream_t s, int lag = 0) {
    const int nch = g.nx / 2;
    const int nwc = cdiv(nch, LdsMarch<T, 1, MODE>::OUTL);
    const int nrows = out_hi - out_lo;
    const int pad = lds_pad_bytes(g, MODE);
    const int nseg = g.fastdiv == 1   ? lds_segments<T, 1, MODE>(g, nrows, nwc, pad)
                     : g.fastdiv == 2 ? lds_segments<T, 2, MODE>(g, nrows, nwc, pad)
                                      : lds_segments<T, 0, MODE>(g, nrows, nwc, pad);
    const dim3 grid(nwc * cdiv(nseg, kLdsWaves)), block(kLdsWaves * 64);
    float *pa = f.pp[0] - (long)g.hg * g.nx, *pb = f.pp[1] - (long)g.hg * g.nx;
    constexpr int kEdgeWeight = 11;
    const int reach = T + 2;
    const int wlo = out_lo - reach <= 1 - g.j0 ? kEdgeWeight : 16;
    const int whi = out_hi + reach >= g.ny - 2 - g.j0 ? kEdgeWeight : 16;
#define CFD_LDS_LAUNCH(FASTV)                                                                      \
    hipLaunchKernelGGL((k_jacobi_lds<T, FASTV, MODE>), grid, block, pad, s, g, pa, pb, f.rhs, f.ctl, \
                       rs, pass, par, out_lo, out_hi, nwc, nseg, wlo, whi, it, lag)
    if (g.fastdiv == 1)
        CFD_LDS_LAUNCH(1);
    else if (g.fastdiv == 2)
        CFD_LDS_LAUNCH(2);
    else
        CFD_LDS_LAUNCH(0);
#undef CFD_LDS_LAUNCH
}

template <int T>
void launch_lds_T(const Geom &g, const Fields &f, int pass, int par, int it, int out_lo, int out_hi,
                  uint32_t *rs, int mode, hipStream_t s, int lag = 0) {
    if (mode == 2) {
        launch_lds_t<T, 2>(g, f, pass, par, it, out_lo, out_hi, rs, s, lag);
        return;
    }
    if constexpr (T == 8) {
        if (mode == 3) {
            launch_lds_t<8, 3>(g, f, pass, par, it, out_lo, out_hi, rs, s, lag);
            return;
        }
    }
    if (rs)
        launch_lds_t<T, 1>(g, f, pass, par, it, out_lo, out_hi, rs, s);
    else
        launch_lds_t<T, 0>(g, f, pass, par, it, out_lo, out_hi, rs, s);
}

template <int T, int FAST>
int persist_blocks_per_cu(int pad) {
    static int cache[2] = {0, 0};
    int &nb = cache[pad > 0 ? 1 : 0];
    if (nb == 0) {
        int n = 0;
        if (hipOccupancyMaxActiveBlocksPerMultiprocessor(
                &n, reinterpret_cast<const void *>(&k_jacobi_persist<T, FAST>), kLdsWaves * 64, pad) !=
                hipSuccess ||
            n < 1)
            n = 1;
        nb = std::min(n, 6);
    }
    return nb;
}

template <int T>
bool launch_lds_persist_t(const Geom &g, const Fields &f, int pass, int par0, int nblk, int out_lo,
                          int out_hi, uint32_t epoch, uint32_t *rs, hipStream_t s) {
    const int nch = g.nx / 2;
    const int nwc = cdiv(nch, LdsMarch<T, 1, 0>::OUTL);
    const int nrows = out_hi - out_lo;
    const int pad = lds_pad_bytes(g, 0);
    const int occ = g.fastdiv == 1   ? persist_blocks_per_cu<T, 1>(pad)
                    : g.fastdiv == 2 ? persist_blocks_per_cu<T, 2>(pad)
                                     : persist_blocks_per_cu<T, 0>(pad);
    const int nseg = g.fastdiv == 1   ? lds_segments<T, 1, 0>(g, nrows, nwc, pad, occ)
                     : g.fastdiv == 2 ? lds_segments<T, 2, 0>(g, nrows, nwc, pad, occ)
                                      : lds_segments<T, 0, 0>(g, nrows, nwc, pad, occ);
    const int ngrp = cdiv(nseg, kLdsWaves);
    if (ngrp * nwc > kPersistMaxGroups || nrows < ngrp * 2 * T) return false;
    const char *ge = getenv("CFD_PERSIST_GRID");
    const int nwg = std::max(ngrp * nwc, ge ? atoi(ge) : 0);
    const dim3 grid(nwg), block(kLdsWaves * 64);
    float *pa = f.pp[0] - (long)g.hg * g.nx, *pb = f.pp[1] - (long)g.hg * g.nx;
    constexpr int kEdgeWeight = 11;
    const int reach = T + 2;
    const int wlo = out_lo - reach <= 1 - g.j0 ? kEdgeWeight : 16;
    const int whi = out_hi + reach >= g.ny - 2 - g.j0 ? kEdgeWeight : 16;
    const int acq = 1;
    const char *de = getenv("CFD_PERSIST_DEADLINE_US");
    const double dl_us = de ? std::max(0.0, atof(de)) : 10e6;
    const uint32_t deadline = (uint32_t)std::min(4.0e9, dl_us * 100.0);
    const char *se = getenv("CFD_PERSIST_STEAL_US");
    const double st_us = se ? std::max(0.0, atof(se)) : 50.0;
    const uint32_t steal = (uint32_t)std::min(4.0e9, st_us * 100.0);
    const char *le = getenv("CFD_PERSIST_LATE");
    const int late = le ? std::max(0, atoi(le)) : 0;
    const char *ue = getenv("CFD_JACOBI_SUMS");
    int exp2 = 0;
    const float R = g.r_dx_sq;
    const bool pow2 = R >= 1.0f && std::frexp(R, &exp2) == 0.5f;
    const int sums = !(ue && atoi(ue) == 0) && g.fastdiv == 1 && g.dx_sq == g.dy_sq &&
                     g.r_dx_sq == g.r_dy_sq && pow2;
    const float plim = sums ? std::ldexp(1.0f, 124) / R : 0.0f, rlim = std::ldexp(1.0f, 124);
#define CFD_LDS_PLAUNCH(FASTV)                                                                     \
    hipLaunchKernelGGL((k_jacobi_persist<T, FASTV>), grid, block, pad, s, g, pa, pb, f.rhs, f.ctl, \
                       f.persist, f.host_nonfinite ? f.host_nonfinite + 2 : nullptr, rs, epoch, pass, \
                       par0, nblk, out_lo, out_hi, nwc, nseg, wlo, whi, ngrp, acq, deadline, steal,  \
                       late, sums, plim, rlim)
    if (g.fastdiv == 1)
        CFD_LDS_PLAUNCH(1);
    else if (g.fastdiv == 2)
        CFD_LDS_PLAUNCH(2);
    else
        CFD_LDS_PLAUNCH(0);
#undef CFD_LDS_PLAUNCH
    return true;
}

}

void launch_lds_t567(const Geom &g, const Fields &f, int T, int pass, int par, int it, int out_lo,
                     int out_hi, uint32_t *rs, int mode, hipStream_t s, int lag);
void launch_lds_t8(const Geom &g, const Fields &f, int pass, int par, int it, int out_lo, int out_hi,
                   uint32_t *rs, int mode, hipStream_t s, int lag);
bool launch_lds_persist8(const Geom &g, const Fields &f, int pass, int par0, int nblk, int out_lo,
                         int out_hi, uint32_t epoch, uint32_t *rs, hipStream_t s);

}
```

cfd-demo_amd/csrc/cfd_kernels.hip:

```cpp
#include "cfd_device.h"
#include "cfd_predict.h"

namespace cfd {

typedef float f4u __attribute__((ext_vector_type(4), aligned(4)));

namespace {
__global__ __launch_bounds__(kBlock) void k_verify_division(float c, float r,
                                                            unsigned long long *counts) {
    const uint32_t tid = blockIdx.x * blockDim.x + threadIdx.x;
    const uint32_t stride = gridDim.x * blockDim.x;
    uint32_t bad1 = 0, bad2 = 0, bad3 = 0;
    for (uint64_t k = tid; k < (1ull << 32); k += stride) {
        const float x = __uint_as_float((uint32_t)k);
        const float ref = x / c;
        const float m1 = fdiv<1>(x, c, r);
        const float m2 = fdiv<2>(x, c, r);
        const float m3 = fdiv<3>(x, c, r);
        const bool rn = ref != ref;
        bad1 += (rn ? (m1 == m1) : (__float_as_uint(m1) != __float_as_uint(ref))) ? 1u : 0u;
        bad2 += (rn ? (m2 == m2) : (__float_as_uint(m2) != __float_as_uint(ref))) ? 1u : 0u;
        bad3 += (rn ? (m3 == m3) : (__float_as_uint(m3) != __float_as_uint(ref))) ? 1u : 0u;
    }
#pragma unroll
// ... 896 lines not shown
}

template <int SP>
__device__ __forceinline__ float cf_u_face(const Geom &g, float inlet, float dt, int i, int j,
                                           float ustar, float p_right, float p_left) {
    const int nx = g.nx;
    if (j == 0) return 0.0f;
    if (j == g.ny - 1) return (g.bc_kind == 1 && i > 0 && i < nx) ? inlet : 0.0f;
    if (i == 0) return g.bc_kind == 0 ? inlet_value(g, inlet, j) : 0.0f;
    if (i == nx)
        return g.bc_kind == 0 ? ustar - sdiv<SP>(dt * (p_right - p_left), g.dx, g.r_dx) : 0.0f;
    return (i >= nx - 7) ? ustar - sdiv<SP>(dt * (p_right - p_left), g.dx, g.r_dx)
                         : ustar - dt * sdiv<SP>(p_right - p_left, g.dx, g.r_dx);
}

__device__ __forceinline__ void step_finalize_body(const Geom &g, const Fields &f) {
    auto ld_ctl = [](const uint32_t *p) { return *p; };
    Ctl *c = f.ctl;
    if (threadIdx.x < 4) {
        uint32_t *set = f.red_slots + (size_t)threadIdx.x * kResSlots * kResStride;
        uint32_t v = ld_ctl(&c->red[threadIdx.x]);
        for (int s = 0; s < kResSlots; ++s) {
            v = max(v, ld_ctl(&set[s * kResStride]));
            set[s * kResStride] = 0u;
        }
        c->red[threadIdx.x] = v;
    }
    __syncthreads();
    if (threadIdx.x != 0) return;
    if (ld_ctl(&c->red[4]) && !c->nonfinite_step) {
        c->nonfinite_step = c->step + 1u;
        if (f.host_nonfinite) *f.host_nonfinite = c->step + 1u;
    }
    c->res_u = __uint_as_float(c->red[0]);
    c->res_v = __uint_as_float(c->red[1]);
    const float max_vel = fmaxf(__uint_as_float(c->red[2]), __uint_as_float(c->red[3]));
    c->step += 1u;
    if (f.host_progress) *f.host_progress = c->step;
    c->time = c->time + c->dt;
    const float previous_dt = c->dt;
    float new_dt;
    if (max_vel == 0.0f) {
        new_dt = c->dt;
    } else {
        const float cfl = 0.2f;
        const float dt_cfl = cfl * fminf(g.dx, g.dy) / max_vel;
        new_dt = fminf(dt_cfl, c->dt);
    }
    c->dt = (new_dt > previous_dt) ? fminf(new_dt, previous_dt * 1.1f) : new_dt;
    c->last_p = __uint_as_float(ld_ctl(&c->red[5]));
    c->red[0] = c->red[1] = c->red[2] = c->red[3] = c->red[4] = c->red[5] = 0u;
    if (ld_ctl(&c->red[6])) {
        if (f.persist) __hip_atomic_store(f.persist + 1, 1u, __ATOMIC_RELAXED, __HIP_MEMORY_SCOPE_AGENT);
        if (f.host_nonfinite)
            __hip_atomic_store(f.host_nonfinite + 2, 1u, __ATOMIC_RELAXED, __HIP_MEMORY_SCOPE_SYSTEM);
    }
}

__global__ void k_abort_to_red(Fields f) {
    if (threadIdx.x == 0 && f.persist)
        f.ctl->red[6] = __hip_atomic_load(f.persist + 1, __ATOMIC_RELAXED, __HIP_MEMORY_SCOPE_AGENT) ? 1u : 0u;
}

__global__ void k_abort_from_red(Fields f) {
    if (threadIdx.x != 0 || !f.ctl->red[6]) return;
    if (f.persist) __hip_atomic_store(f.persist + 1, 1u, __ATOMIC_RELAXED, __HIP_MEMORY_SCOPE_AGENT);
    if (f.host_nonfinite)
        __hip_atomic_store(f.host_nonfinite + 2, 1u, __ATOMIC_RELAXED, __HIP_MEMORY_SCOPE_SYSTEM);
}

__global__ void k_step_finalize(Geom g, Fields f) { step_finalize_body(g, f); }

template <int SP>
__device__ __forceinline__ void cf4_row(const Geom &g, const Fields &f, const float *__restrict__ pp,
                                        float inlet, float dt, int i0, int lj, const float4 &pc,
                                        const float4 &pb, float &du, float &dv, float &mu,
                                        float &mv, bool &bad) {
    const int nx = g.nx, W = nx + 1;
    const int j = g.j0 + lj;
    const long rp = (long)lj * nx + i0;
    const bool vrow = (j != 0 && j != g.ny);
    if (lj < g.nyl) {
        const long k = (long)lj * W + i0;
        const float pl = (i0 > 0) ? pp[rp - 1] : 0.0f;
        const f4u su = *reinterpret_cast<const f4u *>(f.u_star + k);
        const float s0 = su.x, s1 = su.y, s2 = su.z, s3 = su.w;
        float n0 = cf_u_face<SP>(g, inlet, dt, i0, j, s0, pc.x, pl);
        float n1 = cf_u_face<SP>(g, inlet, dt, i0 + 1, j, s1, pc.y, pc.x);
        float n2 = cf_u_face<SP>(g, inlet, dt, i0 + 2, j, s2, pc.z, pc.y);
        float n3 = cf_u_face<SP>(g, inlet, dt, i0 + 3, j, s3, pc.w, pc.z);
        if (f.n_obs > 0) {
            if (f.mask_u[k] & 2) n0 = 0.0f;
            if (f.mask_u[k + 1] & 2) n1 = 0.0f;
            if (f.mask_u[k + 2] & 2) n2 = 0.0f;
            if (f.mask_u[k + 3] & 2) n3 = 0.0f;
        }
        const f4u uo = *reinterpret_cast<const f4u *>(f.u + k);
        const float o0 = uo.x, o1 = uo.y, o2 = uo.z, o3 = uo.w;
        *reinterpret_cast<f4u *>(f.u + k) = (f4u){n0, n1, n2, n3};
        du = fmaxf(fmaxf(fmaxf(du, fabsf(n0 - o0)), fmaxf(fabsf(n1 - o1), fabsf(n2 - o2))),
                   fabsf(n3 - o3));
        mu = fmaxf(fmaxf(fmaxf(mu, fabsf(n0)), fmaxf(fabsf(n1), fabsf(n2))), fabsf(n3));
        bad |= nonfinite(n0) || nonfinite(n1) || nonfinite(n2) || nonfinite(n3);
        if (i0 + 4 == nx) {
            float n4 = cf_u_face<SP>(g, inlet, dt, nx, j, s3, pc.w, pc.z);
            if (f.n_obs > 0 && (f.mask_u[k + 4] & 2)) n4 = 0.0f;
            const float o4 = f.u[k + 4];
            f.u[k + 4] = n4;
            du = fmaxf(du, fabsf(n4 - o4));
            mu = fmaxf(mu, fabsf(n4));
            bad |= nonfinite(n4);
        }
    }
    float4 nv = make_float4(0.f, 0.f, 0.f, 0.f);
    if (vrow) {
        const float4 vs = *reinterpret_cast<const float4 *>(f.v_star + rp);
        nv.x = vs.x - dt * sdiv<SP>(pc.x - pb.x, g.dy, g.r_dy);
        nv.y = vs.y - dt * sdiv<SP>(pc.y - pb.y, g.dy, g.r_dy);
        nv.z = vs.z - dt * sdiv<SP>(pc.z - pb.z, g.dy, g.r_dy);
        nv.w = vs.w - dt * sdiv<SP>(pc.w - pb.w, g.dy, g.r_dy);
    }
    if (f.n_obs > 0) {
        if (f.mask_v[rp] & 2) nv.x = 0.0f;
        if (f.mask_v[rp + 1] & 2) nv.y = 0.0f;
        if (f.mask_v[rp + 2] & 2) nv.z = 0.0f;
        if (f.mask_v[rp + 3] & 2) nv.w = 0.0f;
    }
    const float4 ov = *reinterpret_cast<const float4 *>(f.v + rp);
    *reinterpret_cast<float4 *>(f.v + rp) = nv;
    dv = fmaxf(fmaxf(fmaxf(dv, fabsf(nv.x - ov.x)), fmaxf(fabsf(nv.y - ov.y), fabsf(nv.z - ov.z))),
               fabsf(nv.w - ov.w));
    mv = fmaxf(fmaxf(fmaxf(mv, fabsf(nv.x)), fmaxf(fabsf(nv.y), fabsf(nv.z))), fabsf(nv.w));
    bad |= nonfinite(nv.x) || nonfinite(nv.y) || nonfinite(nv.z) || nonfinite(nv.w);
    if (lj < g.nyl) {
        float4 p = *reinterpret_cast<const float4 *>(f.p + rp);
        p.x = p.x + pc.x;
        p.y = p.y + pc.y;
        p.z = p.z + pc.z;
        p.w = p.w + pc.w;
        *reinterpret_cast<float4 *>(f.p + rp) = p;
    }
}

#ifndef CFD_CF_ROWS
#define CFD_CF_ROWS 16
#endif
constexpr int kCfRows = CFD_CF_ROWS;
template <int SP, int ROWS>
__global__ __launch_bounds__(kBlock) void k_correct_finish4m(Geom g, Fields f, float dt_override,
                                                             int nbx) {
    Ctl *c = f.ctl;
    const int nx = g.nx;
    float du = 0.f, dv = 0.f, mu = 0.f, mv = 0.f;
    bool bad = false;
    const int bid = xcd_block(g);
    const int i0 = 4 * ((bid % nbx) * kBlock + (int)threadIdx.x);
    const int l0 = (bid / nbx) * ROWS, l1 = min(l0 + ROWS, g.nyl + 1);
    const float dt = dt_of(c, dt_override);
    const float inlet = c->inlet;
    const float *__restrict__ pp = c->cur ? f.pp[1] : f.pp[0];
    if (i0 < nx) {
        float4 pb = make_float4(0.f, 0.f, 0.f, 0.f);
        {
            const int j = g.j0 + l0;
            if (j != 0 && j != g.ny) pb = *reinterpret_cast<const float4 *>(pp + (long)(l0 - 1) * nx + i0);
        }
        for (int lj = l0; lj < l1; ++lj) {
            const int j = g.j0 + lj;
            const bool vrow = (j != 0 && j != g.ny);
            float4 pc = make_float4(0.f, 0.f, 0.f, 0.f);
            if (lj < g.nyl || vrow) pc = *reinterpret_cast<const float4 *>(pp + (long)lj * nx + i0);
            cf4_row<SP>(g, f, pp, inlet, dt, i0, lj, pc, vrow ? pb : make_float4(0.f, 0.f, 0.f, 0.f),
                        du, dv, mu, mv, bad);
            pb = pc;
        }
    }
    flag_nonfinite(c, bad);
    __shared__ float red[kBlock / 64][4];
    du = wave_max(du);
    dv = wave_max(dv);
    mu = wave_max(mu);
    mv = wave_max(mv);
    const int wv = threadIdx.x >> 6;
    if ((threadIdx.x & 63) == 0) {
        red[wv][0] = du;
        red[wv][1] = dv;
        red[wv][2] = mu;
        red[wv][3] = mv;
    }
    __syncthreads();
    if (threadIdx.x < 4) {
        float r = 0.f;
#pragma unroll
        for (int w = 0; w < kBlock / 64; ++w) r = fmaxf(r, red[w][threadIdx.x]);
        publish_max(f.red_slots + (size_t)threadIdx.x * kResSlots * kResStride, bid, r);
    }
}


__global__ __launch_bounds__(kBlock) void k_step_reduce(Geom g, Fields f) {
    const size_t tid = blockIdx.x * (size_t)blockDim.x + threadIdx.x;
    const size_t stride = (size_t)gridDim.x * blockDim.x;
    const size_t nu = (size_t)g.nyl * (g.nx + 1), nv = (size_t)(g.nyl + 1) * g.nx;
    float du = 0.f, dv = 0.f, mu = 0.f, mv = 0.f;
    bool bad = false;
    for (size_t k = tid; k < nu; k += stride) {
        const float a = f.u[k];
        du = fmaxf(du, fabsf(a - f.u_old[k]));
        mu = fmaxf(mu, fabsf(a));
        bad |= nonfinite(a);
    }
    for (size_t k = tid; k < nv; k += stride) {
        const float a = f.v[k];
        dv = fmaxf(dv, fabsf(a - f.v_old[k]));
        mv = fmaxf(mv, fabsf(a));
        bad |= nonfinite(a);
    }
    flag_nonfinite(f.ctl, bad);
    du = wave_max(du);
    dv = wave_max(dv);
    mu = wave_max(mu);
    mv = wave_max(mv);
    if ((threadIdx.x & 63) == 0) {
        const int key = (int)(tid >> 6);
        constexpr size_t S = (size_t)kResSlots * kResStride;
        publish_max(f.red_slots, key, du);
        publish_max(f.red_slots + S, key, dv);
        publish_max(f.red_slots + 2 * S, key, mu);
        publish_max(f.red_slots + 3 * S, key, mv);
    }
}



inline int copy_grid(size_t n4) {
    long b = cdiv((long)n4, kBlock);
    return (int)(b < 2048 ? (b < 1 ? 1 : b) : 2048);
}

}


void launch_step_begin(const Geom &g, const Fields &f, int copy, hipStream_t s) {
    size_t n4 = f.u_alloc > f.v_alloc ? f.u_alloc / 4 : f.v_alloc / 4;
    hipLaunchKernelGGL(k_step_begin, dim3(copy ? copy_grid(n4) : 1), dim3(kBlock), 0, s, g, f,
                       copy);
}

void launch_copy_star(const Geom &g, const Fields &f, int pass, hipStream_t s) {
    size_t n4 = f.u_alloc > f.v_alloc ? f.u_alloc / 4 : f.v_alloc / 4;
    hipLaunchKernelGGL(k_copy_star, dim3(copy_grid(n4)), dim3(kBlock), 0, s, f, pass);
}

void launch_u_predictor(const Geom &g, const Fields &f, float dt_override, hipStream_t s) {
    const int glo = g.j0 > 1 ? g.j0 : 1;
    const int ghi = (g.j0 + g.nyl - 1) < (g.ny - 2) ? (g.j0 + g.nyl - 1) : (g.ny - 2);
    if (ghi < glo) return;
    const int nbx = cdiv(g.nx, kBlock);
    const dim3 grid(nbx * (ghi - glo + 1));
#define CFD_LAUNCH_U(SC, SPV) hipLaunchKernelGGL((k_u_predictor<SC, SPV>), grid, dim3(kBlock), 0, s, \
                                                 g, f, dt_override, glo - g.j0, nbx)
    if (g.scheme == 0) {
        if (g.sp_pow2) CFD_LAUNCH_U(0, 1); else CFD_LAUNCH_U(0, 0);
    } else {
        if (g.sp_pow2) CFD_LAUNCH_U(1, 1); else CFD_LAUNCH_U(1, 0);
    }
#undef CFD_LAUNCH_U
}

void launch_v_predictor(const Geom &g, const Fields &f, float dt_override, hipStream_t s) {
    const int glo = g.j0 > 1 ? g.j0 : 1;
    const int ghi = (g.j0 + g.nyl) < (g.ny - 1) ? (g.j0 + g.nyl) : (g.ny - 1);
    if (ghi < glo) return;
    const int nbx = cdiv(g.nx - 1, kBlock);
    const dim3 grid(nbx * (ghi - glo + 1));
#define CFD_LAUNCH_V(SC, SPV) hipLaunchKernelGGL((k_v_predictor<SC, SPV>), grid, dim3(kBlock), 0, s, \
                                                 g, f, dt_override, glo - g.j0, nbx)
    if (g.scheme == 0) {
        if (g.sp_pow2) CFD_LAUNCH_V(0, 1); else CFD_LAUNCH_V(0, 0);
    } else {
        if (g.sp_pow2) CFD_LAUNCH_V(1, 1); else CFD_LAUNCH_V(1, 0);
    }
#undef CFD_LAUNCH_V
}

void launch_predict(const Geom &g, const Fields &f, float dt_override, hipStream_t s) {
    const int glo = g.j0 > 1 ? g.j0 : 1;
    const int u_hi = (g.j0 + g.nyl - 1) < (g.ny - 2) ? (g.j0 + g.nyl - 1) : (g.ny - 2);
    const int v_hi = (g.j0 + g.nyl) < (g.ny - 1) ? (g.j0 + g.nyl) : (g.ny - 1);
    const int ghi = u_hi > v_hi ? u_hi : v_hi;
    if (ghi < glo) return;
    static const int vec = [] {
        const char *e = getenv("CFD_PRED_VEC");
        return e ? atoi(e) : 1;
    }();
    auto a16 = [](const void *p) { return ((uintptr_t)p & 15u) == 0; };
    if (vec && g.scheme == 0 && g.nx % 4 == 0 && a16(f.v) && a16(f.v_star)) {
        const int nbx4 = cdiv(g.nx / 4, kBlock);
        const dim3 gr(nbx4 * cdiv(ghi - glo + 1, 2));
        if (g.sp_pow2)
            hipLaunchKernelGGL((k_predict4r<1, 2>), gr, dim3(kBlock), 0, s, g, f, dt_override,
                               glo - g.j0, u_hi - g.j0, v_hi - g.j0, nbx4);
        else
            hipLaunchKernelGGL((k_predict4r<0, 2>), gr, dim3(kBlock), 0, s, g, f, dt_override,
                               glo - g.j0, u_hi - g.j0, v_hi - g.j0, nbx4);
        return;
    }
    const int nbx = cdiv(g.nx, kBlock);
    const dim3 grid(nbx * (ghi - glo + 1));
#define CFD_LAUNCH_P(SC, SPV) hipLaunchKernelGGL((k_predict<SC, SPV>), grid, dim3(kBlock), 0, s, g, f, \
                                                 dt_override, glo - g.j0, u_hi - g.j0, v_hi - g.j0, nbx)
    if (g.scheme == 0) {
        if (g.sp_pow2) CFD_LAUNCH_P(0, 1); else CFD_LAUNCH_P(0, 0);
    } else {
        if (g.sp_pow2) CFD_LAUNCH_P(1, 1); else CFD_LAUNCH_P(1, 0);
    }
#undef CFD_LAUNCH_P
}

bool predict_div_fused(const Geom &g, const Fields &f) {
    auto a16 = [](const void *p) { return ((uintptr_t)p & 15u) == 0; };
    return g.pred_div == 1 && g.scheme == 0 && g.nx % 4 == 0 && g.nx >= 8 && a16(f.v) && a16(f.v_star) &&
           a16(f.rhs);
}

void launch_predict_div(const Geom &g, const Fields &f, float dt_override, hipStream_t s) {
    const int glo = (g.j0 > 1 ? g.j0 : 1) - g.j0;
    const int u_hi = ((g.j0 + g.nyl - 1) < (g.ny - 2) ? (g.j0 + g.nyl - 1) : (g.ny - 2)) - g.j0;
    const int v_hi = ((g.j0 + g.nyl) < (g.ny - 1) ? (g.j0 + g.nyl) : (g.ny - 1)) - g.j0;
    constexpr int rpt = 2;
// ... 212 lines not shown
```

cfd-demo_amd/csrc/cfd_model.hip:

```cpp
#include <hip/hip_runtime.h>
#include <rccl/rccl.h>

#include <chrono>
#include <cmath>
#include <initializer_list>
#include <condition_variable>
#include <memory>
#include <mutex>
#include <thread>
#include <cstdio>
#include <cstring>
#include <string>
#include <functional>
#include <vector>

#include "../../include/cfd.h"
#include "cfd_internal.h"
#include "slab_plan.h"

using namespace cfd;

namespace {

thread_local std::string g_last_error;
// ... 1461 lines not shown
        launch_step_finalize(g, f, stream);
        HIP_TRY(hipGetLastError());
        if (rec_step) HIP_TRY(hipEventRecord(ev_step1, stream));
        if (timing) timed_steps++;
        if (rec_step) stepped = true;
        return 0;
    }
    std::vector<hipEvent_t> step_events;

    hipGraphExec_t step_graph = nullptr;
    int graph_cur_delta = 0;
    int graph_steps = 4;
    bool graph_enabled = [] {
        const char *e = getenv("CFD_GRAPH");
        return e && atoi(e) != 0;
    }();
    bool graph_ok() const {
        return graph_enabled && !sharded() && !timing &&
               params.pressure_solver == CFD_SOLVER_JACOBI;
    }
    void drop_graph() {
        if (step_graph) (void)hipGraphExecDestroy(step_graph);
        step_graph = nullptr;
    }
    int update_graph(int n) {
        if (!step_graph) {
            const int hc0 = host_cur;
            HIP_TRY(hipStreamBeginCapture(stream, hipStreamCaptureModeThreadLocal));
            int rc = 0;
            capturing = true;
            for (int k = 0; k < graph_steps && !rc; ++k) rc = enqueue_update(false);
            capturing = false;
            hipGraph_t graph = nullptr;
            const hipError_t ce = hipStreamEndCapture(stream, &graph);
            if (rc || ce != hipSuccess) {
                if (graph) (void)hipGraphDestroy(graph);
                host_cur = hc0;
                return rc ? rc : fail(CFD_EHIP, std::string("hipStreamEndCapture: ") + hipGetErrorString(ce));
            }
            const hipError_t ie = hipGraphInstantiate(&step_graph, graph, nullptr, nullptr, 0);
            (void)hipGraphDestroy(graph);
            if (ie != hipSuccess) {
                step_graph = nullptr;
                host_cur = hc0;
                return fail(CFD_EHIP, std::string("hipGraphInstantiate: ") + hipGetErrorString(ie));
            }
            graph_cur_delta = (host_cur - hc0) & 1;
            host_cur = hc0;
        }
        int k = 0;
        for (; k + graph_steps <= n - 1; k += graph_steps) {
            HIP_TRY(hipGraphLaunch(step_graph, stream));
            host_cur = (host_cur + graph_cur_delta) & 1;
        }
        for (; k < n; ++k) {
            int rc = enqueue_update(k == n - 1);
            if (rc) return rc;
        }
        return 0;
    }

    int abort_allreduce() {
        if (!(sharded() && persist_env && persist_sharded_env)) return 0;
        launch_abort_to_red(f, stream);
        int rc = allreduce_max_u32(f.ctl->red + 6, 1);
        if (rc) return rc;
        launch_abort_from_red(f, stream);
        HIP_TRY(hipGetLastError());
        return 0;
    }

    int sync() {
        HIP_TRY(hipSetDevice(device));
        int rc = wait_done(nullptr);
        if (rc) return rc;
        rc = persist_timeout_check(true);
        if (rc) return rc;
        ck_commit();
        return 0;
    }
    int persist_timeout_check(bool at_sync) {
        if (!h_nonfinite || !*(volatile uint32_t *)(h_nonfinite + 2)) return 0;
        if (!at_sync && sharded()) return 0;
        const char *which = last_abort_resident ? "resident tolerance-mode" : "persistent";
        HIP_TRY(hipStreamSynchronize(stream));
        if (cstream) HIP_TRY(hipStreamSynchronize(cstream));
        *(volatile uint32_t *)(h_nonfinite + 2) = 0u;
        persist_env = false;
        resident_off = true;
        if (ck_open) {
            const size_t n_entries = ck_replay.size();
            int rc = recover();
            if (rc) return rc;
            return fail(CFD_ETIMEOUT, std::string(which) + " Jacobi solve timed out waiting for a "
                                      "workgroup; recovered: the state was restored from the "
                                      "model's checkpoint and " + std::to_string(n_entries) +
                                      " call(s) re-run with one launch per block (the state is "
                                      "valid); per-launch solves from now on");
        }
        clear_abort_words();
        return fail(CFD_ETIMEOUT, std::string(which) + " Jacobi solve timed out waiting for a "
                                  "workgroup (no checkpoint was open); its result is invalid; "
                                  "per-launch solves from now on");
    }

    struct CkSeg {
        void *ptr;
        size_t bytes;
    };
    std::vector<CkSeg> ck_segs;
    char *ck_pool = nullptr;
    size_t ck_bytes = 0;
    bool ck_open = false;
    int ck_host_cur = 0;
    bool ck_shallow = false;
    std::vector<std::function<int()>> ck_replay;
    uint64_t recoveries = 0;
    bool last_abort_resident = false;
    bool ckpt_env = [] {
        const char *e = getenv("CFD_CKPT");
        return !(e && atoi(e) == 0);
    }();
    bool ckpt_needed() const {
        if (!ckpt_env || params.pressure_solver != CFD_SOLVER_JACOBI) return false;
        if (persist_env && (sharded() ? persist_sharded_env : persist_req > 0)) return true;
        return resident_mode();
    }
    int ck_begin() {
        if (ck_open || !ckpt_needed()) return 0;
        if (!ck_pool) {
            size_t tot = 0;
            for (const CkSeg &sg : ck_segs) tot += (sg.bytes + 255) & ~(size_t)255;
            HIP_TRY(hipMalloc((void **)&ck_pool, tot));
            ck_bytes = tot;
        }
        size_t off = 0;
        for (const CkSeg &sg : ck_segs) {
            HIP_TRY(hipMemcpyAsync(ck_pool + off, sg.ptr, sg.bytes, hipMemcpyDeviceToDevice, stream));
            off += (sg.bytes + 255) & ~(size_t)255;
        }
        ck_host_cur = host_cur;
        ck_shallow = pp_ghosts_shallow;
        ck_replay.clear();
        ck_open = true;
        return 0;
    }
    void ck_record(std::function<int()> fn) {
        if (ck_open) ck_replay.push_back(std::move(fn));
    }
    void ck_commit() {
        ck_open = false;
        ck_replay.clear();
    }
    int clear_abort_words() {
        HIP_TRY(hipMemset(f.persist, 0, (size_t)kPersistHeadLines * kPersistFlagStride * 4));
        return 0;
    }
    int recover() {
        size_t off = 0;
        for (const CkSeg &sg : ck_segs) {
            HIP_TRY(hipMemcpy(sg.ptr, ck_pool + off, sg.bytes, hipMemcpyDeviceToDevice));
            off += (sg.bytes + 255) & ~(size_t)255;
        }
        HIP_TRY(hipMemset(f.err_slots, 0, (size_t)kMaxSweeps * kResSlots * kResStride * 4));
        int rc = clear_abort_words();
        if (rc) return rc;
        *(volatile uint32_t *)h_nonfinite = 0u;
        host_cur = ck_host_cur;
        pp_ghosts_shallow = ck_shallow;
        ++recoveries;
        std::vector<std::function<int()>> replay;
        replay.swap(ck_replay);
        ck_open = false;
        const bool tm = timing;
        timing = false;
        for (auto &fn : replay) {
            rc = fn();
            if (rc) break;
        }
        timing = tm;
        if (rc) return rc;
        rc = wait_done(nullptr);
        if (rc) return rc;
        if (*(volatile uint32_t *)(h_nonfinite + 2))
            return fail(CFD_ETIMEOUT, "the re-run after a solve timeout timed out");
        return 0;
    }

    int read_ctl(Ctl *out) {
        int rc = sync();
        if (rc) return rc;
        HIP_TRY(hipMemcpy(out, f.ctl, offsetof(Ctl, go), hipMemcpyDeviceToHost));
        return 0;
    }

    void destroy() {
        {
            PersistGate &gate = persist_gate(device);
            std::lock_guard<std::mutex> lk(gate.mu);
            if (gate.last == stream) gate.last = nullptr;
        }
        (void)hipSetDevice(device);
        if (stream) (void)hipStreamSynchronize(stream);
        if (comm) ncclCommDestroy(comm);
        comm = nullptr;
        for (hipEvent_t e : ev_res)
            if (e) (void)hipEventDestroy(e);
        if (h_res) (void)hipHostFree(h_res);
        for (hipEvent_t e : ev_spec)
            if (e) (void)hipEventDestroy(e);
        if (h_spec) (void)hipHostFree(h_spec);
        for (void *ptr : {(void *)u_all, (void *)v_all, (void *)uo_all, (void *)vo_all,
                          (void *)us_all, (void *)vs_all, (void *)p, (void *)rhs,
                          (void *)pp_all[0], (void *)pp_all[1], (void *)mask_u, (void *)mask_v,
                          (void *)obs, (void *)ctl, (void *)slots, (void *)vis_buf,
                          (void *)mg_pool, (void *)mg_dev})
            if (ptr) (void)hipFree(ptr);
        if (h_nonfinite) (void)hipHostFree(h_nonfinite);
        if (ck_pool) (void)hipFree(ck_pool);
        drop_graph();
        for (hipEvent_t e : ev_pool) (void)hipEventDestroy(e);
        if (ev_step0) (void)hipEventDestroy(ev_step0);
        if (ev_step1) (void)hipEventDestroy(ev_step1);
        if (ev_prof0) (void)hipEventDestroy(ev_prof0);
        if (ev_prof1) (void)hipEventDestroy(ev_prof1);
        if (stream) (void)hipStreamDestroy(stream);
        if (cstream) (void)hipStreamDestroy(cstream);
        if (ev_ov0) (void)hipEventDestroy(ev_ov0);
        if (ev_ov1) (void)hipEventDestroy(ev_ov1);
        if (ev_rhs) (void)hipEventDestroy(ev_rhs);
        if (ev_uv) (void)hipEventDestroy(ev_uv);
    }
};

namespace {

int validate(const cfd_grid *grid, const cfd_params *p) {
    if (!grid || !p) return fail(CFD_EINVAL, "null grid or params");
    if (grid->nx < 16 || grid->nx % 8 != 0)
        return fail(CFD_EINVAL, "nx must be a multiple of 8 and >= 16 (model.rs:541 precondition)");
    if (grid->ny < 4) return fail(CFD_EINVAL, "ny must be >= 4");
    if ((grid->nx + 1) * grid->ny > (1ull << 31))
        return fail(CFD_EINVAL, "grid too large for 32-bit row indexing");
    if (!(grid->lx > 0.f) || !(grid->ly > 0.f)) return fail(CFD_EINVAL, "lx, ly must be > 0");
    if (p->jacobi_iters < 0 || p->jacobi_iters > kMaxSweeps)
        return fail(CFD_EINVAL, "jacobi_iters out of range [0, 4096]");
    if (p->corrector_passes < 0 || p->corrector_passes > kMaxPasses - 1)
        return fail(CFD_EINVAL, "corrector_passes out of range [0, 63]");
    if (p->velocity_scheme != 0 && p->velocity_scheme != 1)
        return fail(CFD_EINVAL, "velocity_scheme must be 0 or 1");
    if (p->inlet_profile != 0 && p->inlet_profile != 1)
        return fail(CFD_EINVAL, "inlet_profile must be 0 or 1");
    if (p->pressure_solver < CFD_SOLVER_JACOBI || p->pressure_solver > CFD_SOLVER_MULTIGRID)
        return fail(CFD_EINVAL, "pressure_solver must be 0 (Jacobi), 1 (SOR) or 2 (multigrid)");
    if (p->bc_kind != 0 && p->bc_kind != 1) return fail(CFD_EINVAL, "bc_kind must be 0 or 1");
    return 0;
}

int validate_sharded(const cfd_model *m, const cfd_params *p) {
    if (m->n_ranks <= 1 || p->pressure_solver != CFD_SOLVER_SOR) return 0;
    const int lo = std::max(0, 1 - (int)m->j0);
    const int hi = std::min((int)(m->j1 - m->j0), (int)m->grid.ny - 1 - (int)m->j0);
    if (p->jacobi_iters < 1 || m->g.hg < 2 || !sor_fused_ok((int)m->grid.nx, hi - lo))
        return fail(CFD_EINVAL, "sharded SOR needs >= 1 iteration, halo depth >= 2 and >= 16 "
                                "interior rows per slab (rank " + std::to_string(m->rank) + " has " +
                                    std::to_string(hi - lo) + ", halo depth " +
                                    std::to_string(m->g.hg) + ")");
    return 0;
}

void apply_params(cfd_model *m, const cfd_params *p) {
    m->params = *p;
    m->g.nu = p->viscosity;
    m->g.target_inlet = p->target_inlet_velocity;
    m->g.scheme = p->velocity_scheme;
    m->g.profile = p->inlet_profile;
    m->g.bc_kind = p->bc_kind;
    m->g.tol_enabled = p->tol_enabled ? 1 : 0;
    m->g.p_tol = p->p_tol;
    m->g.jacobi_iters = p->jacobi_iters;
}

std::mutex g_div_mu;
std::vector<std::pair<uint32_t, int>> g_div_cache;

int division_ok_mask(hipStream_t s, float c, float r, int *mask) {
    uint32_t bits;
    std::memcpy(&bits, &c, 4);
    {
        std::lock_guard<std::mutex> lk(g_div_mu);
        for (auto &e : g_div_cache)
            if (e.first == bits) {
                *mask = e.second;
                return 0;
            }
    }
    unsigned long long *d = nullptr, h[3] = {0, 0, 0};
    HIP_TRY(hipMalloc((void **)&d, 24));
    HIP_TRY(hipMemsetAsync(d, 0, 24, s));
    launch_verify_division(c, r, d, s);
    HIP_TRY(hipGetLastError());
    HIP_TRY(hipMemcpyAsync(h, d, 24, hipMemcpyDeviceToHost, s));
    HIP_TRY(hipStreamSynchronize(s));
    HIP_TRY(hipFree(d));
    *mask = (h[0] == 0 ? 1 : 0) | (h[1] == 0 ? 2 : 0) | (h[2] == 0 ? 4 : 0);
    std::lock_guard<std::mutex> lk(g_div_mu);
    g_div_cache.emplace_back(bits, *mask);
    return 0;
}

int choose_division(hipStream_t s, Geom &g) {
    g.fastdiv = 0;
    g.res_div = 0;
    const char *env = getenv("CFD_FASTDIV");
    if (env && atoi(env) == 0) return 0;
    int m1, m2, m3;
    int rc;
    if ((rc = division_ok_mask(s, g.dx_sq, g.r_dx_sq, &m1)) ||
        (rc = division_ok_mask(s, g.dy_sq, g.r_dy_sq, &m2)) ||
        (rc = division_ok_mask(s, g.denom, g.r_denom, &m3)))
        return rc;
    const int all = m1 & m2 & m3;
    g.fastdiv = (all & 1) ? 1 : (all & 2) ? 2 : 0;
    if (env && atoi(env) == 2 && (all & 2)) g.fastdiv = 2;
    const char *rd = getenv("CFD_RESIDENT_DIV");
    g.res_div = g.fastdiv != 0 ? g.fastdiv : (rd && atoi(rd) == 3 && (all & 4)) ? 3 : 0;
    return 0;
}

int build_model(cfd_model *m, const cfd_grid *grid, const cfd_params *p, int device, int hg) {
    m->device = device;
    m->grid = *grid;
    HIP_TRY(hipSetDevice(device));
    HIP_TRY(hipStreamCreateWithFlags(&m->stream, hipStreamNonBlocking));
    HIP_TRY(hipStreamCreateWithFlags(&m->cstream, hipStreamNonBlocking));
    HIP_TRY(hipEventCreateWithFlags(&m->ev_ov0, hipEventDisableTiming));
    HIP_TRY(hipEventCreateWithFlags(&m->ev_ov1, hipEventDisableTiming));
    HIP_TRY(hipEventCreateWithFlags(&m->ev_rhs, hipEventDisableTiming));
    HIP_TRY(hipEventCreateWithFlags(&m->ev_uv, hipEventDisableTiming));
    HIP_TRY(hipEventCreate(&m->ev_step0));
    HIP_TRY(hipEventCreate(&m->ev_step1));
    HIP_TRY(hipEventCreate(&m->ev_prof0));
    HIP_TRY(hipEventCreate(&m->ev_prof1));
    const int nx = (int)grid->nx, ny = (int)grid->ny;
    Geom &g = m->g;
    g.nx = nx;
    g.ny = ny;
    g.j0 = (int)m->j0;
    g.nyl = (int)(m->j1 - m->j0);
    g.hg = hg;
    if ((uint64_t)(g.nyl + 2 * hg + 2 * kGhostUV + 1) * (uint64_t)(nx + 1) * 4u >= (1ull << 31))
        return fail(CFD_EINVAL, "slab too large for 32-bit buffer offsets (2 GiB per field)");
    g.dx = grid->lx / (float)grid->nx;
    g.dy = grid->ly / (float)grid->ny;
    g.ly = grid->ly;
    apply_params(m, p);
    g.dx_sq = g.dx * g.dx;
    g.dy_sq = g.dy * g.dy;
    g.denom = 2.0f / (g.dx * g.dx) + 2.0f / (g.dy * g.dy);
    g.r_dx_sq = 1.0f / g.dx_sq;
    g.r_dy_sq = 1.0f / g.dy_sq;
    g.r_denom = 1.0f / g.denom;
    {
        auto pow2f = [](float c) {
            int e;
            return c > 0.0f && std::isfinite(c) && std::frexp(c, &e) == 0.5f &&
                   std::isnormal(1.0f / c);
        };
        g.r_dx = 1.0f / g.dx;
        g.r_dy = 1.0f / g.dy;
        g.r_dxx = 1.0f / (g.dx * g.dx);
        g.r_dyy = 1.0f / (g.dy * g.dy);
        g.sp_pow2 = pow2f(g.dx) && pow2f(g.dy) && pow2f(g.dx * g.dx) && pow2f(g.dy * g.dy) ? 1 : 0;
        if (const char *e = getenv("CFD_FASTDIV"))
            if (atoi(e) == 0) g.sp_pow2 = 0;
    }
    {
        int rc0 = choose_division(m->stream, g);
        if (rc0) return rc0;
    }
    g.tb_kind = g.fastdiv == 1 ? 5 : 4;
    g.pred_div = 2;
    if (const char *e = getenv("CFD_PRED_DIV")) g.pred_div = std::min(std::max(atoi(e), 0), 2);
    if (const char *kv = getenv("CFD_TB_KIND")) {
        const int k = atoi(kv);
        g.tb_kind = (k == 3 || k == 4 || k == 5) ? k : 1;
    }
    if (g.tb_kind != 5 && (uint64_t)(g.nyl + 2 * g.hg) * (uint64_t)nx * 4u > (1ull << 30))
        g.tb_kind = 1;
    m->t_max = g.tb_kind == 3 ? 6 : 4;
    {
        const uint64_t jac_ws = 3ull * (uint64_t)(g.nyl + 2 * g.hg) * (uint64_t)nx * 4u;
        if (g.tb_kind == 4 && g.fastdiv == 1 && m->n_ranks == 1 && jac_ws > (256ull << 20))
            m->t_max = 8;
        if (g.tb_kind == 5) m->t_max = 8;
    }
    if (const char *tv = getenv("CFD_TEMPORAL")) m->t_max = std::max(1, atoi(tv));
    m->t_max = std::min(m->t_max, g.tb_kind == 1 ? 4 : kMaxTemporal);
    g.tb_rows = g.tb_kind == 5 ? 0 : 24;
    if (const char *rv = getenv("CFD_TB_ROWS")) g.tb_rows = std::max(4, std::min(1024, atoi(rv)));
    g.tb_bpc = 3;
    if (const char *bv = getenv("CFD_TB_BPC")) {
        g.tb_bpc = std::max(1, std::min(16, atoi(bv)));
        g.tb_rows = 0;
    }
    g.xcd_remap = 1;
    if (const char *xv = getenv("CFD_XCD_REMAP")) g.xcd_remap = atoi(xv) ? 1 : 0;
    {
        int ncu = 0;
        if (hipDeviceGetAttribute(&ncu, hipDeviceAttributeMultiprocessorCount, device) != hipSuccess ||
            ncu <= 0)
            ncu = 256;
        g.n_cu = ncu;
    }


    const size_t W = (size_t)nx + 1, nyl = (size_t)g.nyl;
    const size_t u_alloc = round4(m->u_rows_alloc() * W);
    const size_t v_alloc = round4(m->v_rows_alloc() * (size_t)nx);
    const size_t p_n = nyl * nx;
    const size_t pp_n = (nyl + 2 * (size_t)hg) * nx;
    auto zalloc = [&](void **ptr, size_t bytes) -> int {
        HIP_TRY(hipMalloc(ptr, bytes));
        HIP_TRY(hipMemsetAsync(*ptr, 0, bytes, m->stream));
        return 0;
    };
    int rc = 0;
    if ((rc = zalloc((void **)&m->u_all, u_alloc * 4)) || (rc = zalloc((void **)&m->v_all, v_alloc * 4)) ||
        (rc = zalloc((void **)&m->uo_all, u_alloc * 4)) || (rc = zalloc((void **)&m->vo_all, v_alloc * 4)) ||
        (rc = zalloc((void **)&m->us_all, u_alloc * 4)) || (rc = zalloc((void **)&m->vs_all, v_alloc * 4)) ||
        (rc = zalloc((void **)&m->p, p_n * 4)) || (rc = zalloc((void **)&m->rhs, pp_n * 4)) ||
        (rc = zalloc((void **)&m->pp_all[0], pp_n * 4)) || (rc = zalloc((void **)&m->pp_all[1], pp_n * 4)) ||
        (rc = zalloc((void **)&m->mask_u, nyl * W + 16)) || (rc = zalloc((void **)&m->mask_v, (nyl + 1) * nx + 16)) ||
        (rc = zalloc((void **)&m->ctl, sizeof(Ctl))) ||
        (rc = zalloc((void **)&m->slots, kSlotWords * 4)))
        return rc;
    m->ck_segs = {{m->u_all, u_alloc * 4}, {m->v_all, v_alloc * 4}, {m->uo_all, u_alloc * 4},
                  {m->vo_all, v_alloc * 4}, {m->us_all, u_alloc * 4}, {m->vs_all, v_alloc * 4},
                  {m->p, p_n * 4},         {m->rhs, pp_n * 4},        {m->pp_all[0], pp_n * 4},
                  {m->pp_all[1], pp_n * 4}, {m->ctl, sizeof(Ctl)}};
    HIP_TRY(hipHostMalloc((void **)&m->h_nonfinite, 16, hipHostMallocMapped | hipHostMallocCoherent));
    *(volatile uint32_t *)m->h_nonfinite = 0u;
    *(volatile uint32_t *)(m->h_nonfinite + 1) = 0u;
    *(volatile uint32_t *)(m->h_nonfinite + 2) = 0u;
    HIP_TRY(hipHostMalloc((void **)&m->h_res, 4 * cfd_model::kResRing, hipHostMallocDefault));
    for (hipEvent_t &e : m->ev_res) HIP_TRY(hipEventCreateWithFlags(&e, hipEventDisableTiming));
    HIP_TRY(hipHostMalloc((void **)&m->h_spec, 4 * cfd_model::kSpecRing * kMaxTemporal, hipHostMallocDefault));
    for (hipEvent_t &e : m->ev_spec) HIP_TRY(hipEventCreateWithFlags(&e, hipEventDisableTiming));
    if (const char *to = getenv("CFD_RCCL_TIMEOUT_S")) m->rccl_timeout_s = std::max(1.0, atof(to));

    std::vector<uint8_t> mu(nyl * W, 0), mv((nyl + 1) * nx, 0);
    std::vector<int32_t> obs;
    if (grid->has_cylinder) {
        for (int j = 0; j < ny; ++j) {
            for (int i = 0; i < nx; ++i) {
                const float x = ((float)i + 0.5f) * g.dx;
                const float y = ((float)j + 0.5f) * g.dy;
                const float ddx = x - grid->cylinder_x;
                const float ddy = y - grid->cylinder_y;
                const float distance = std::sqrt(ddx * ddx + ddy * ddy);
                if (!(distance < grid->cylinder_radius)) continue;
                const long lj = (long)j - (long)m->j0;
                if (lj >= 0 && lj < (long)nyl) {
                    if (i > 0) mu[lj * W + i] = 1;
                    if (i < nx) mu[lj * W + i + 1] = 1;
                }
                if (j > 0 && lj >= 0 && lj <= (long)nyl) mv[lj * nx + i] = 1;
                if (j < ny && lj + 1 >= 0 && lj + 1 <= (long)nyl) mv[(lj + 1) * nx + i] = 1;
                if (lj >= 0 && lj <= (long)nyl) {
                    obs.push_back(i);
                    obs.push_back(j);
                }
            }
        }
    }
    m->h_mask_u = mu;
    m->h_mask_v = mv;
    std::vector<uint8_t> dmu(mu), dmv(mv);
    for (size_t k = 0; k < obs.size(); k += 2) {
        const long oi = obs[k], lj = (long)obs[k + 1] - (long)m->j0;
        if (lj >= 0 && lj < (long)nyl) dmu[lj * W + oi] |= 2;
        if (lj >= 0 && lj <= (long)nyl) dmv[lj * nx + oi] |= 2;
    }
    m->dmask_u = std::move(dmu);
    m->dmask_v = std::move(dmv);
    HIP_TRY(hipMemcpyAsync(m->mask_u, m->dmask_u.data(), m->dmask_u.size(), hipMemcpyHostToDevice,
                           m->stream));
    HIP_TRY(hipMemcpyAsync(m->mask_v, m->dmask_v.data(), m->dmask_v.size(), hipMemcpyHostToDevice,
                           m->stream));
    if (!obs.empty()) {
        HIP_TRY(hipMalloc((void **)&m->obs, obs.size() * 4));
        HIP_TRY(hipMemcpyAsync(m->obs, obs.data(), obs.size() * 4, hipMemcpyHostToDevice, m->stream));
    }

    Fields &f = m->f;
    const size_t uoff = (size_t)kGhostUV * W, voff = (size_t)kGhostUV * nx;
    f.u_alloc_base = m->u_all;
    f.v_alloc_base = m->v_all;
    f.u_old_base = m->uo_all;
    f.v_old_base = m->vo_all;
    f.u_star_base = m->us_all;
    f.v_star_base = m->vs_all;
    f.u_alloc = u_alloc;
    f.v_alloc = v_alloc;
    f.u = m->u_all + uoff;
    f.v = m->v_all + voff;
    f.u_old = m->uo_all + uoff;
    f.v_old = m->vo_all + voff;
    f.u_star = m->us_all + uoff;
    f.v_star = m->vs_all + voff;
    f.p = m->p;
    f.rhs = m->rhs + (size_t)hg * nx;
    f.pp[0] = m->pp_all[0] + (size_t)hg * nx;
    f.pp[1] = m->pp_all[1] + (size_t)hg * nx;
    f.mask_u = m->mask_u;
    f.mask_v = m->mask_v;
    f.obs = m->obs;
    f.n_obs = (int32_t)(obs.size() / 2);
    f.any_pmask = 0;
    for (uint8_t b : m->h_mask_u) f.any_pmask |= b & 1;
    for (uint8_t b : m->h_mask_v) f.any_pmask |= b & 1;
    f.ctl = m->ctl;
    {
        void *dp = nullptr;
        HIP_TRY(hipHostGetDevicePointer(&dp, m->h_nonfinite, 0));
        f.host_nonfinite = (uint32_t *)dp;
        f.host_progress = m->n_ranks > 1 ? (uint32_t *)dp + 1 : nullptr;
    }
    f.err_slots = m->slots;
    f.red_slots = m->slots + (size_t)kMaxSweeps * kResSlots * kResStride;
    f.vis_slots = f.red_slots + (size_t)4 * kResSlots * kResStride;
    f.persist = m->slots + (size_t)(kMaxSweeps + 16) * kResSlots * kResStride;

    Ctl c0;
    std::memset(&c0, 0, sizeof(c0));
    c0.dt = p->dt;
    c0.go[0] = 1;
    HIP_TRY(hipMemcpyAsync(m->ctl, &c0, sizeof(Ctl), hipMemcpyHostToDevice, m->stream));
    HIP_TRY(hipStreamSynchronize(m->stream));
    return 0;
}

struct CommInitJob {
    std::mutex mu;
    std::condition_variable cv;
    bool done = false, abandoned = false;
    ncclComm_t comm = nullptr;
    ncclResult_t r = ncclSuccess;
    hipError_t he = hipSuccess;
};

int comm_init(cfd_model *m, const ncclUniqueId &id, int n_ranks, int rank) {
    auto job = std::make_shared<CommInitJob>();
    const int device = m->device;
    std::thread([job, id, n_ranks, rank, device] {
        ncclComm_t c = nullptr;
        ncclResult_t r = ncclInternalError;
        const hipError_t he = hipSetDevice(device);
        if (he == hipSuccess) r = ncclCommInitRank(&c, n_ranks, id, rank);
        std::lock_guard<std::mutex> lk(job->mu);
        if (job->abandoned) {
            if (r == ncclSuccess && c) ncclCommAbort(c);
            return;
        }
        job->comm = c;
        job->r = r;
        job->he = he;
        job->done = true;
        job->cv.notify_all();
    }).detach();
    std::unique_lock<std::mutex> lk(job->mu);
    const auto limit = std::chrono::duration<double>(m->rccl_timeout_s);
    if (!job->cv.wait_for(lk, limit, [&] { return job->done; })) {
        job->abandoned = true;
        return fail(CFD_ERCCL, "ncclCommInitRank: rank " + std::to_string(rank) + " of " +
                                   std::to_string(n_ranks) + ": not every rank joined within " +
                                   std::to_string((int)m->rccl_timeout_s) +
                                   " s (CFD_RCCL_TIMEOUT_S); creation abandoned");
    }
    if (job->he != hipSuccess)
        return fail(CFD_EHIP, std::string("hipSetDevice (RCCL init thread): ") + hipGetErrorString(job->he));
    if (job->r != ncclSuccess)
        return fail(CFD_ERCCL, std::string("ncclCommInitRank: ") + ncclGetErrorString(job->r));
    m->comm = job->comm;
    return 0;
}

int create_common(const cfd_grid *grid, const cfd_params *params, int device, int n_ranks, int rank,
                  const void *uid, LocalHub *hub, cfd_model **out) {
    if (!out) return fail(CFD_EINVAL, "null out");
    *out = nullptr;
    int rc = validate(grid, params);
    if (rc) return rc;
    if (n_ranks < 1 || rank < 0 || rank >= n_ranks) return fail(CFD_EINVAL, "bad rank/n_ranks");
    int ndev = 0;
    if (hipGetDeviceCount(&ndev) != hipSuccess || ndev == 0)
        return fail(CFD_EHIP, "no HIP device available");
    if (device < 0 || device >= ndev) return fail(CFD_EINVAL, "device ordinal out of range");
    cfd_model *m = new cfd_model();
    m->n_ranks = n_ranks;
    m->rank = rank;
    plan_slab(grid->ny, n_ranks, rank, &m->j0, &m->j1);
    int hg = 1;
    if (n_ranks > 1) {
        uint64_t min_rows = grid->ny / (uint64_t)n_ranks;
        const char *env = getenv("CFD_HALO_DEPTH");
        hg = env ? atoi(env)
                 : (int)std::max<uint64_t>(kMaxTemporal, std::min<uint64_t>(32, min_rows / 32));
        if (hg < 1) hg = 1;
        if ((uint64_t)hg + 2 > min_rows) hg = (int)(min_rows > 3 ? min_rows - 2 : 1);
        if (min_rows < 4) {
            delete m;
            return fail(CFD_EINVAL, "each slab needs at least 4 rows");
        }
    }
    rc = build_model(m, grid, params, device, hg);
    if (!rc) rc = validate_sharded(m, params);
    if (!rc && n_ranks > 1 && hub) {
        if (hub->n != n_ranks) {
            rc = fail(CFD_EINVAL, "local hub size != n_ranks");
        } else {
            std::lock_guard<std::mutex> lk(hub->mu);
            hub->members[rank] = m;
            m->hub = hub;
        }
    } else if (!rc && n_ranks > 1) {
        ncclUniqueId id;
        std::memcpy(&id, uid, sizeof(id));
        rc = comm_init(m, id, n_ranks, rank);
    }
    if (rc) {
        m->destroy();
        delete m;
        return rc;
    }
    *out = m;
    return 0;
}

}


extern "C" {

const char *cfd_last_error(void) { return g_last_error.c_str(); }
void cfdrt_set_error(const char *msg) { g_last_error = msg ? msg : ""; }
int cfdrt_check_params(const cfd_model *m, const cfd_params *p) {
    if (!m) return fail(CFD_EINVAL, "null model");
    int rc = validate(&m->grid, p);
    if (rc) return rc;
    return validate_sharded(m, p);
}

int cfd_get_config(const cfd_model *m, cfd_grid *grid, cfd_params *params) {
    if (!m) return fail(CFD_EINVAL, "null model");
    if (grid) *grid = m->grid;
    if (params) *params = m->params;
    return 0;
}
int cfd_abi_version(void) { return CFD_ABI_VERSION; }

void cfd_default_params(cfd_params *o) {
    if (!o) return;
    o->dt = 0.005f;
    o->viscosity = 0.000001f;
    o->target_inlet_velocity = 1.0f;
    o->velocity_scheme = CFD_SCHEME_FIRST_ORDER;
    o->inlet_profile = CFD_INLET_UNIFORM;
    o->pressure_solver = CFD_SOLVER_JACOBI;
    o->jacobi_iters = 50;
    o->corrector_passes = 20;
    o->tol_enabled = 1;
    o->p_tol = 1e-4f;
    o->bc_kind = CFD_BC_CHANNEL;
}

void cfd_default_grid(cfd_grid *o) {
    if (!o) return;
    o->nx = 800;
    o->ny = 264;
    o->lx = 30.0f;
    o->ly = 10.0f;
    o->has_cylinder = 1;
    o->cylinder_x = 30.0f / 4.0f;
    o->cylinder_y = 10.0f / 2.0f;
    o->cylinder_radius = 0.75f;
}

int cfd_create(const cfd_grid *grid, const cfd_params *params, int device_ordinal, cfd_model **out) {
    return create_common(grid, params, device_ordinal, 1, 0, nullptr, nullptr, out);
}

int cfd_rccl_unique_id(void *out) {
    if (!out) return fail(CFD_EINVAL, "null out");
    ncclUniqueId id;
    RCCL_TRY(ncclGetUniqueId(&id));
    static_assert(sizeof(ncclUniqueId) == 128, "ncclUniqueId is 128 bytes");
    std::memcpy(out, &id, sizeof(id));
    return 0;
}

int cfd_create_sharded(const cfd_grid *grid, const cfd_params *params, int device_ordinal,
                       int n_ranks, int rank, const void *uid, cfd_model **out) {
    if (n_ranks > 1 && !uid) return fail(CFD_EINVAL, "null rccl unique id");
    return create_common(grid, params, device_ordinal, n_ranks, rank, uid, nullptr, out);
}

void *cfd_local_hub_create(int n_ranks) {
    if (n_ranks < 1) return nullptr;
    LocalHub *h = new LocalHub();
    h->n = n_ranks;
    h->members.assign(n_ranks, nullptr);
    return h;
}

void cfd_local_hub_destroy(void *hub) { delete static_cast<LocalHub *>(hub); }

int cfd_create_sharded_local(const cfd_grid *grid, const cfd_params *params, int device_ordinal,
                             int n_ranks, int rank, void *hub, cfd_model **out) {
    if (!hub) return fail(CFD_EINVAL, "null local hub");
    return create_common(grid, params, device_ordinal, n_ranks, rank, nullptr,
                         static_cast<LocalHub *>(hub), out);
}

int cfd_device_count(int *n_out) {
    if (!n_out) return fail(CFD_EINVAL, "null out");
    *n_out = 0;
    int n = 0;
    const hipError_t e = hipGetDeviceCount(&n);
    if (e != hipSuccess && e != hipErrorNoDevice)
        return fail(CFD_EHIP, std::string("hipGetDeviceCount: ") + hipGetErrorString(e));
    *n_out = e == hipSuccess ? n : 0;
    return 0;
}

int cfd_get_comm_size(const cfd_model *m, int *n_out) {
    if (!m || !n_out) return fail(CFD_EINVAL, "null model or out");
    if (m->hub) {
        *n_out = m->hub->n;
    } else if (m->comm) {
        int n = 0;
        RCCL_TRY(ncclCommCount(m->comm, &n));
        *n_out = n;
    } else if (m->n_ranks > 1) {
        return fail(CFD_ERCCL, "the RCCL communicator was aborted after an earlier failure");
    } else {
        *n_out = 1;
    }
    return 0;
}

int cfd_get_slab(const cfd_model *m, uint64_t *j0, uint64_t *j1) {
    if (!m) return fail(CFD_EINVAL, "null model");
    if (j0) *j0 = m->j0;
    if (j1) *j1 = m->j1;
    return 0;
}

int cfd_update(cfd_model *m) { return cfd_update_n(m, 1); }

int cfd_update_n(cfd_model *m, int n) {
    if (!m) return fail(CFD_EINVAL, "null model");
    HIP_TRY(hipSetDevice(m->device));
    if (int rc = m->persist_timeout_check(false)) return rc;
    if (const uint32_t bad = *(volatile uint32_t *)m->h_nonfinite)
        return fail(CFD_ENONFINITE, "non-finite velocity (NaN/Inf) after step " + std::to_string(bad) +
                                        "; cfd_set_state clears it");
    if (n <= 0) return 0;
    if (int rc = m->ck_begin()) return rc;
    m->ck_record([m, n]() {
        for (int k = 0; k < n; ++k)
            if (int rc = m->enqueue_update(k == n - 1)) return rc;
        return 0;
    });
    if (m->timing) {
        hipEvent_t e0 = m->take_event();
        HIP_TRY(hipEventRecord(e0, m->stream));
        m->step_events.push_back(e0);
    }
    int rc = 0;
    if (m->graph_ok()) {
        rc = m->update_graph(n);
    } else {
        for (int k = 0; k < n && !rc; ++k) rc = m->enqueue_update(k == n - 1);
    }
    if (m->timing) {
        hipEvent_t e1 = m->take_event();
        HIP_TRY(hipEventRecord(e1, m->stream));
        m->step_events.push_back(e1);
    }
    return rc;
}

int cfd_piso_step(cfd_model *m, float dt_sub) {
    if (!m) return fail(CFD_EINVAL, "null model");
    HIP_TRY(hipSetDevice(m->device));
    if (int rc = m->ck_begin()) return rc;
    auto run = [m, dt_sub]() {
        int rc = m->exchange_uv();
        if (!rc) rc = m->enqueue_piso(dt_sub);
        return rc ? rc : m->abort_allreduce();
    };
    m->ck_record(run);
    return run();
}

int cfd_pressure_solve(cfd_model *m, float *residual_out) {
    if (!m) return fail(CFD_EINVAL, "null model");
    HIP_TRY(hipSetDevice(m->device));
    int rc;
    if (m->host_driven()) {
        return m->enqueue_solve_host_driven(residual_out);
    }
    if ((rc = m->ck_begin())) return rc;
    auto run = [m]() {
        int rc2 = m->enqueue_solve(-1);
        return rc2 ? rc2 : m->abort_allreduce();
    };
    m->ck_record(run);
    rc = run();
    if (rc) return rc;
    Ctl c;
    rc = m->read_ctl(&c);
    if (rc) return rc;
    if (residual_out) *residual_out = c.last_p;
    return 0;
}

int cfd_run_phase(cfd_model *m, int phase, float dt_sub) {
    if (!m) return fail(CFD_EINVAL, "null model");
    HIP_TRY(hipSetDevice(m->device));
    switch (phase) {
    case CFD_PHASE_U_PREDICTOR: {
        int rc = m->exchange_uv();
        if (rc) return rc;
        launch_u_predictor(m->g, m->f, dt_sub, m->stream);
        break;
    }
    case CFD_PHASE_V_PREDICTOR: {
        int rc = m->exchange_uv();
        if (rc) return rc;
        launch_v_predictor(m->g, m->f, dt_sub, m->stream);
        break;
    }
    case CFD_PHASE_DIVERGENCE: launch_divergence(m->g, m->f, -1, dt_sub, m->stream); break;
    case CFD_PHASE_CORRECTOR: launch_corrector(m->g, m->f, -1, dt_sub, m->stream); break;
    case CFD_PHASE_BOUNDARY: launch_boundary(m->g, m->f, m->stream); break;
    default: return fail(CFD_EINVAL, "unknown phase");
    }
    HIP_TRY(hipGetLastError());
    return m->sync();
}

int cfd_set_params(cfd_model *m, const cfd_params *p) {
    if (!m) return fail(CFD_EINVAL, "null model");
    int rc = validate(&m->grid, p);
    if (rc) return rc;
    rc = validate_sharded(m, p);
    if (rc) return rc;
    rc = m->sync();
    if (rc) return rc;
    m->drop_graph();
    {
        Ctl c;
        rc = m->read_ctl(&c);
        if (rc) return rc;
        m->host_cur = c.cur;
    }
    apply_params(m, p);
    HIP_TRY(hipMemcpy(&m->ctl->dt, &p->dt, 4, hipMemcpyHostToDevice));
    return 0;
}

int cfd_get_snapshot(cfd_model *m, float *u, float *v, float *p, float *dt_out) {
    if (!m) return fail(CFD_EINVAL, "null model");
    int rc = m->sync();
    if (rc) return rc;
    const size_t W = (size_t)m->g.nx + 1, nx = (size_t)m->g.nx, nyl = (size_t)m->g.nyl;
    if (u) HIP_TRY(hipMemcpy(u, m->f.u, nyl * W * 4, hipMemcpyDeviceToHost));
    if (v) HIP_TRY(hipMemcpy(v, m->f.v, (nyl + 1) * nx * 4, hipMemcpyDeviceToHost));
    if (p) HIP_TRY(hipMemcpy(p, m->f.p, nyl * nx * 4, hipMemcpyDeviceToHost));
    if (dt_out) HIP_TRY(hipMemcpy(dt_out, &m->ctl->dt, 4, hipMemcpyDeviceToHost));
    return 0;
}

namespace {

float decode_key(uint32_t k, bool is_min) {
    if (is_min) {
        if (!k) return INFINITY;
        k = ~k;
    } else if (!k) {
        return -INFINITY;
    }
    const uint32_t b = (k & 0x80000000u) ? (k & 0x7FFFFFFFu) : ~k;
    float x;
    std::memcpy(&x, &b, 4);
    return x;
}

int render_common(cfd_model *m, int mode, bool field, void *host_out, float *min_max_out) {
    if (!m) return fail(CFD_EINVAL, "null model");
    if (mode < CFD_VIS_PRESSURE || mode > CFD_VIS_VORTICITY)
        return fail(CFD_EINVAL, "unknown visualisation mode");
    HIP_TRY(hipSetDevice(m->device));
    const size_t n = (size_t)m->g.nx * (size_t)m->g.nyl;
    if (!m->vis_buf) HIP_TRY(hipMalloc((void **)&m->vis_buf, n * 4));
    if (mode == CFD_VIS_VORTICITY) {
        int rc = m->exchange_uv();
        if (rc) return rc;
    }
    Fields &f = m->f;
    launch_vis_field(m->g, f, mode, field ? m->vis_buf : nullptr, f.vis_slots, m->stream);
    launch_fold_slots(f.ctl->vis, f.vis_slots, 2, m->stream);
    int rc = m->allreduce_max_u32(f.ctl->vis, 2);
    if (rc) return rc;
    const cfd_grid &gr = m->grid;
    if (!field && host_out)
        launch_vis_color(m->g, f, mode, nullptr, (uint32_t *)m->vis_buf, f.ctl->vis,
                         gr.has_cylinder, gr.cylinder_x, gr.cylinder_y, gr.cylinder_radius,
                         m->stream);
    HIP_TRY(hipGetLastError());
    uint32_t keys[2] = {0u, 0u};
    HIP_TRY(hipMemcpyAsync(keys, f.ctl->vis, 8, hipMemcpyDeviceToHost, m->stream));
    HIP_TRY(hipMemsetAsync(f.ctl->vis, 0, 8, m->stream));
    if (host_out) HIP_TRY(hipMemcpyAsync(host_out, m->vis_buf, n * 4, hipMemcpyDeviceToHost, m->stream));
    if (int rc2 = m->wait_done(nullptr)) return rc2;
    if (min_max_out) {
        min_max_out[0] = decode_key(keys[1], true);
        min_max_out[1] = decode_key(keys[0], false);
    }
    return 0;
}

}

int cfd_render(cfd_model *m, int mode, uint8_t *rgba, float *min_max_out) {
    return render_common(m, mode, false, rgba, min_max_out);
}

int cfd_derive_field(cfd_model *m, int mode, float *out, float *min_max_out) {
    return render_common(m, mode, true, out, min_max_out);
}

int cfd_get_residuals(cfd_model *m, cfd_residuals *out) {
    if (!m || !out) return fail(CFD_EINVAL, "null argument");
    Ctl c;
    int rc = m->read_ctl(&c);
    if (rc) return rc;
    out->simulation_step = c.step;
    out->simulation_time = c.time;
    out->dt = c.dt;
    out->p = c.last_p;
    out->u = c.res_u;
    out->v = c.res_v;
    out->piso_substeps = 1;
    out->jacobi_sweeps_total = c.sweeps_total;
    float ms = 0.f;
    if (m->stepped && hipEventElapsedTime(&ms, m->ev_step0, m->ev_step1) == hipSuccess)
        out->step_time_s = ms * 1e-3;
    else
        out->step_time_s = 0.0;
    if (c.nonfinite_step)
        return fail(CFD_ENONFINITE, "non-finite velocity (NaN/Inf) after step " +
                                        std::to_string(c.nonfinite_step));
    return 0;
}

int cfd_get_state(cfd_model *m, cfd_state *st) {
    if (!m || !st) return fail(CFD_EINVAL, "null argument");
    Ctl c;
    int rc = m->read_ctl(&c);
    if (rc) return rc;
    const size_t W = (size_t)m->g.nx + 1, nx = (size_t)m->g.nx, nyl = (size_t)m->g.nyl;
    if (st->u) HIP_TRY(hipMemcpy(st->u, m->f.u, nyl * W * 4, hipMemcpyDeviceToHost));
    if (st->v) HIP_TRY(hipMemcpy(st->v, m->f.v, (nyl + 1) * nx * 4, hipMemcpyDeviceToHost));
    if (st->p) HIP_TRY(hipMemcpy(st->p, m->f.p, nyl * nx * 4, hipMemcpyDeviceToHost));
    if (st->u_star) HIP_TRY(hipMemcpy(st->u_star, m->f.u_star, nyl * W * 4, hipMemcpyDeviceToHost));
    if (st->v_star) HIP_TRY(hipMemcpy(st->v_star, m->f.v_star, (nyl + 1) * nx * 4, hipMemcpyDeviceToHost));
    if (st->p_prime) HIP_TRY(hipMemcpy(st->p_prime, m->f.pp[c.cur], nyl * nx * 4, hipMemcpyDeviceToHost));
    if (st->rhs) HIP_TRY(hipMemcpy(st->rhs, m->f.rhs, nyl * nx * 4, hipMemcpyDeviceToHost));
    st->dt = c.dt;
    st->simulation_time = c.time;
    st->simulation_step = c.step;
    st->last_p_residual = c.last_p;
    st->last_u_residual = c.res_u;
    st->last_v_residual = c.res_v;
    st->jacobi_sweeps_total = c.sweeps_total;
    return 0;
}

int cfd_set_state(cfd_model *m, const cfd_state *st) {
    if (!m || !st) return fail(CFD_EINVAL, "null argument");
    Ctl c;
    int rc = m->read_ctl(&c);
    if (rc) return rc;
    const size_t W = (size_t)m->g.nx + 1, nx = (size_t)m->g.nx, nyl = (size_t)m->g.nyl;
    if (st->u) HIP_TRY(hipMemcpy(m->f.u, st->u, nyl * W * 4, hipMemcpyHostToDevice));
    if (st->v) HIP_TRY(hipMemcpy(m->f.v, st->v, (nyl + 1) * nx * 4, hipMemcpyHostToDevice));
    if (st->p) HIP_TRY(hipMemcpy(m->f.p, st->p, nyl * nx * 4, hipMemcpyHostToDevice));
    if (st->u_star) HIP_TRY(hipMemcpy(m->f.u_star, st->u_star, nyl * W * 4, hipMemcpyHostToDevice));
    if (st->v_star) HIP_TRY(hipMemcpy(m->f.v_star, st->v_star, (nyl + 1) * nx * 4, hipMemcpyHostToDevice));
    if (st->p_prime) HIP_TRY(hipMemcpy(m->f.pp[c.cur], st->p_prime, nyl * nx * 4, hipMemcpyHostToDevice));
    if (st->rhs) HIP_TRY(hipMemcpy(m->f.rhs, st->rhs, nyl * nx * 4, hipMemcpyHostToDevice));
    c.dt = st->dt;
    c.time = st->simulation_time;
    c.step = (uint32_t)st->simulation_step;
    c.last_p = st->last_p_residual;
    c.res_u = st->last_u_residual;
    c.res_v = st->last_v_residual;
    c.sweeps_total = st->jacobi_sweeps_total;
    c.nonfinite_step = 0;
    c.red[4] = 0;
    c.red[6] = 0;
    rc = m->clear_abort_words();
    if (rc) return rc;
    HIP_TRY(hipMemcpy(m->f.ctl, &c, offsetof(Ctl, go), hipMemcpyHostToDevice));
    *(volatile uint32_t *)m->h_nonfinite = 0u;
    m->host_cur = c.cur;
    rc = m->exchange_uv();
    if (rc) return rc;
    rc = m->exchange_pp(c.cur, m->g.hg);
    if (rc) return rc;
    return m->sync();
}

int cfd_get_masks(cfd_model *m, uint8_t *mask_u, uint8_t *mask_v) {
    if (!m) return fail(CFD_EINVAL, "null model");
    if (mask_u) std::memcpy(mask_u, m->h_mask_u.data(), m->h_mask_u.size());
    if (mask_v) std::memcpy(mask_v, m->h_mask_v.data(), m->h_mask_v.size());
    return 0;
}

int cfd_synchronize(cfd_model *m) {
    if (!m) return fail(CFD_EINVAL, "null model");
    return m->sync();
}

int cfd_profile_sweeps(cfd_model *m, int n_sweeps, double *avg_ms_out) {
    if (!m) return fail(CFD_EINVAL, "null model");
    if (n_sweeps < 1 || n_sweeps > kMaxSweeps) return fail(CFD_EINVAL, "n_sweeps out of range");
    HIP_TRY(hipSetDevice(m->device));
    const int lo = std::max(0, 1 - (int)m->j0), hi = std::min(m->g.nyl, (int)m->g.ny - 1 - (int)m->j0);
    hipEvent_t a = m->ev_prof0, b = m->ev_prof1;
    Geom g = m->g;
    g.tol_enabled = 0;
    HIP_TRY(hipEventRecord(a, m->stream));
    for (int it = 0; it < n_sweeps; ++it)
        launch_jacobi_sweep(g, m->f, -1, it, lo, hi, it == n_sweeps - 1, m->stream);
    HIP_TRY(hipEventRecord(b, m->stream));
    launch_finalize_solve(g, m->f, -1, n_sweeps, 0, n_sweeps, m->stream);
    HIP_TRY(hipGetLastError());
    m->host_cur = (m->host_cur + n_sweeps) & 1;
    m->pp_ghosts_shallow = m->sharded();
    int rc = m->sync();
    if (rc) return rc;
    float ms = 0.f;
    HIP_TRY(hipEventElapsedTime(&ms, a, b));
    if (avg_ms_out) *avg_ms_out = ms / n_sweeps;
    return 0;
}

int cfd_timing_begin(cfd_model *m) {
    if (!m) return fail(CFD_EINVAL, "null model");
    int rc = m->sync();
    if (rc) return rc;
    m->timing = true;
    m->ev_next = 0;
    m->solve_events.clear();
    m->step_events.clear();
    for (auto &pe : m->phase_events) pe.clear();
    m->timed_sweeps = 0;
    m->timed_launches = 0;
    m->timed_steps = 0;
    return 0;
}

int cfd_timing_end(cfd_model *m, double *solve_ms, uint64_t *sweeps, double *step_ms, uint64_t *steps) {
    if (!m) return fail(CFD_EINVAL, "null model");
    int rc = m->sync();
    if (rc) return rc;
    double s_ms = 0.0, t_ms = 0.0;
    for (auto &pr : m->solve_events) {
        float ms = 0.f;
        HIP_TRY(hipEventElapsedTime(&ms, pr.first, pr.second));
        s_ms += ms;
    }
    for (size_t k = 0; k + 1 < m->step_events.size(); k += 2) {
        float ms = 0.f;
        HIP_TRY(hipEventElapsedTime(&ms, m->step_events[k], m->step_events[k + 1]));
        t_ms += ms;
    }
    for (int ph = 0; ph < 3; ++ph) {
        m->phase_ms[ph] = 0.0;
        m->phase_count[ph] = 0;
        for (auto &pr : m->phase_events[ph]) {
            float ms = 0.f;
            if (!pr.second) continue;
            HIP_TRY(hipEventElapsedTime(&ms, pr.first, pr.second));
            m->phase_ms[ph] += ms;
            ++m->phase_count[ph];
        }
        m->phase_events[ph].clear();
    }
    if (solve_ms) *solve_ms = s_ms;
    if (sweeps) *sweeps = m->timed_sweeps;
    if (step_ms) *step_ms = t_ms;
    if (steps) *steps = m->timed_steps;
    m->timing = false;
    m->ev_next = 0;
    m->solve_events.clear();
    m->step_events.clear();
    return 0;
}

int cfd_timing_phases(cfd_model *m, int on) {
    if (!m) return fail(CFD_EINVAL, "null model");
    m->timing_phases = on != 0;
    return 0;
}

int cfd_timing_phase_ms(const cfd_model *m, double *predict_ms, double *finish_ms) {
    if (!m) return fail(CFD_EINVAL, "null model");
    if (predict_ms) *predict_ms = m->phase_ms[0];
    if (finish_ms) *finish_ms = m->phase_ms[1];
    return 0;
}

int cfd_timing_exchange_ms(const cfd_model *m, double *exchange_ms, uint64_t *exchanges) {
    if (!m) return fail(CFD_EINVAL, "null model");
    if (exchange_ms) *exchange_ms = m->phase_ms[2];
    if (exchanges) *exchanges = m->phase_count[2];
    return 0;
}

int cfd_get_halo_depth(const cfd_model *m) { return m ? m->g.hg : 0; }

int cfd_get_kernel_config(const cfd_model *m, int *fastdiv, int *temporal) {
    if (!m) return fail(CFD_EINVAL, "null model");
    if (fastdiv) *fastdiv = m->g.fastdiv;
    if (temporal) *temporal = m->spec_mode() ? kMaxTemporal : m->g.tol_enabled ? 1 : m->t_max;
    return 0;
}

int cfd_get_jacobi_kernel(const cfd_model *m, int *kind, char *name, size_t name_len) {
    if (!m) return fail(CFD_EINVAL, "null model");
    const bool spec = m->spec_mode();
    const bool resident = m->resident_mode();
    const int T = spec ? kMaxTemporal : m->g.tol_enabled ? 1 : m->t_max;
    const int k = resident ? 6 : spec ? 5 : T <= 1 ? 0 : m->g.tb_kind;
    if (kind) *kind = k;
    if (name && name_len) {
        char buf[96];
        if (resident)
            snprintf(buf, sizeof buf, "k_jacobi_resident<%d>", m->g.res_div);
        else if (spec)
            snprintf(buf, sizeof buf, "k_jacobi_lds<%d, %d, 2>", T, m->g.fastdiv);
        else if (k == 0)
            snprintf(buf, sizeof buf, "k_jacobi<%d, %d>", kJacRowsPerWave, m->g.fastdiv);
        else if (k == 1)
            snprintf(buf, sizeof buf, "k_jacobi_tb<%d, %d>", T, m->g.fastdiv);
        else if (k == 5)
            snprintf(buf, sizeof buf, "k_jacobi_lds<%d, %d, 0>", T, m->g.fastdiv);
        else
            snprintf(buf, sizeof buf, "k_jacobi_pipe<%d, %d, %d>", T, m->g.fastdiv, k == 3 ? 4 : 2);
        snprintf(name, name_len, "%s", buf);
    }
    return 0;
}

int cfd_get_jacobi_geometry(const cfd_model *m, int persist, int *lds_pad, int *wgs_per_cu,
                            int *wave_cols, int *segments) {
    if (!m) return fail(CFD_EINVAL, "null model");
    if (hipSetDevice(m->device) != hipSuccess) return fail(CFD_EHIP, "hipSetDevice");
    int T, lo, hi, exch;
    plan_block((int)m->j0, m->g.nyl, m->g.ny, m->sharded() ? m->g.hg : 0, 0, 8,
               std::max(8, m->params.jacobi_iters), &T, &lo, &hi, &exch);
    if (!m->sharded()) lo = 1 - (int)m->j0, hi = (int)m->g.ny - 1 - (int)m->j0;
    int pad = 0, occ = 0, nwc = 0, nseg = 0;
    lds_geometry8(m->g, lo, hi, persist != 0, &pad, &occ, &nwc, &nseg);
    if (lds_pad) *lds_pad = pad;
    if (wgs_per_cu) *wgs_per_cu = occ;
    if (wave_cols) *wave_cols = nwc;
    if (segments) *segments = nseg;
    return 0;
}

int cfd_get_persist_steals(cfd_model *m, uint64_t *steals) {
    if (!m || !steals) return fail(CFD_EINVAL, "null argument");
    int rc = m->sync();
    if (rc) return rc;
    uint32_t v = 0;
    HIP_TRY(hipMemcpy(&v, m->f.persist + 2, 4, hipMemcpyDeviceToHost));
    *steals = v;
    return 0;
}

int cfd_get_persist_sums(cfd_model *m, uint64_t *blocks) {
    if (!m || !blocks) return fail(CFD_EINVAL, "null argument");
    int rc = m->sync();
    if (rc) return rc;
    uint32_t v = 0;
    HIP_TRY(hipMemcpy(&v, m->f.persist + 3, 4, hipMemcpyDeviceToHost));
    *blocks = v;
    return 0;
}

int cfd_get_comm_calls(const cfd_model *m, uint64_t *n) {
    if (!m || !n) return fail(CFD_EINVAL, "null argument");
    *n = m->comm_calls;
    return 0;
}

int cfd_get_recoveries(const cfd_model *m, uint64_t *n) {
    if (!m || !n) return fail(CFD_EINVAL, "null argument");
    *n = m->recoveries;
    return 0;
}

int cfd_get_resident_solves(const cfd_model *m, uint64_t *solves) {
    if (!m || !solves) return fail(CFD_EINVAL, "null argument");
    *solves = m->resident_solves;
    return 0;
}

int cfd_get_persist_blocks(const cfd_model *m, int *blocks) {
    if (!m || !blocks) return fail(CFD_EINVAL, "null argument");
    *blocks = m->last_persist_blocks;
    return 0;
}

int cfd_plan_slab(uint64_t ny, int n_ranks, int rank, uint64_t *j0, uint64_t *j1) {
    if (n_ranks < 1 || rank < 0 || rank >= n_ranks || !j0 || !j1)
        return fail(CFD_EINVAL, "bad plan_slab arguments");
    plan_slab(ny, n_ranks, rank, j0, j1);
    return 0;
}

int cfd_plan_sweep(int j0, int nyl, int ny, int halo_depth, int it, int iters, int *lo, int *hi,
                   int *exchange) {
    if (halo_depth < 1 || !lo || !hi || !exchange) return fail(CFD_EINVAL, "bad plan_sweep arguments");
    plan_sweep(j0, nyl, ny, halo_depth, it, iters, lo, hi, exchange);
    return 0;
}

int cfd_plan_block(int j0, int nyl, int ny, int halo_depth, int it, int t_max, int iters, int *T,
                   int *out_lo, int *out_hi, int *exchange) {
    if (t_max < 1 || !T || !out_lo || !out_hi || !exchange)
        return fail(CFD_EINVAL, "bad plan_block arguments");
    plan_block(j0, nyl, ny, halo_depth, it, t_max, iters, T, out_lo, out_hi, exchange);
    return 0;
}

int cfd_plan_overlap(int nyl, int halo_depth, int rank, int n_ranks, int lo, int hi, int *out6) {
    if (!out6 || n_ranks < 1 || rank < 0 || rank >= n_ranks) return fail(CFD_EINVAL, "bad plan_overlap arguments");
    return plan_overlap(nyl, halo_depth, rank, n_ranks, lo, hi, out6);
}

int cfd_plan_halo(int kind, int nyl, int depth, int rank, int n_ranks, int *out6) {
    if (kind < 0 || kind > 2 || !out6) return fail(CFD_EINVAL, "bad plan_halo arguments");
    plan_halo(kind, nyl, depth, rank, n_ranks, out6);
    return 0;
}

void cfd_destroy(cfd_model *m) {
    if (!m) return;
    m->destroy();
    delete m;
}

}
```

cfd-demo_amd/csrc/cfd_predict_march.hip:

```cpp
#include "cfd_device.h"
#include "cfd_predict.h"

namespace cfd {
namespace {

#ifndef CFD_PM_WPE
#define CFD_PM_WPE 3
#endif
#ifndef CFD_PM_USTORE
#define CFD_PM_USTORE 0
#endif
#ifndef CFD_PM_ROWS_FO
#define CFD_PM_ROWS_FO 8
#endif
#ifndef CFD_PM_PD
#define CFD_PM_PD 1
#endif

typedef float f4u __attribute__((ext_vector_type(4), aligned(4)));

template <int C>
struct MAcc {
    const float (&u)[6][8];
    const float (&v)[6][8];
    int q;
    __device__ __forceinline__ float U(int di, int dj) const { return u[C + dj][q + 2 + di]; }
    __device__ __forceinline__ float V(int di, int dj) const { return v[C + dj][q + 2 + di]; }
};

template <int SCHEME, int SP, bool MASK, int R>
struct PredMarch {
    static constexpr int PD = CFD_PM_PD;
    static constexpr int D = PD + 5;

    float UQ[D][4];
    float VQ[D][4];
    float UB[D], VB[D];
    float vs[4];
    const Geom *g;
    Fields f;
    __amdgpu_buffer_rsrc_t rs_u, rs_v, rs_us, rs_vs;
    int vo;
    int i0, c, nch;
    bool st_lane;
    int kb, r0, r1, glo, u_hi, v_hi, W;
    float dt;

    __device__ __forceinline__ void ld_u(float (&d)[4], int row) const {
        row = row < -kGhostUV ? -kGhostUV : (row > g->nyl + kGhostUV - 1 ? g->nyl + kGhostUV - 1 : row);
        const u32x4 x = __builtin_amdgcn_raw_buffer_load_b128(rs_u, vo, (row + kGhostUV) * W * 4, 0);
        d[0] = __uint_as_float(x.x); d[1] = __uint_as_float(x.y);
        d[2] = __uint_as_float(x.z); d[3] = __uint_as_float(x.w);
    }
    __device__ __forceinline__ void ld_v(float (&d)[4], int row) const {
        row = row < -kGhostUV ? -kGhostUV : (row > g->nyl + kGhostUV ? g->nyl + kGhostUV : row);
        const u32x4 x = __builtin_amdgcn_raw_buffer_load_b128(rs_v, vo, (row + kGhostUV) * g->nx * 4, 0);
        d[0] = __uint_as_float(x.x); d[1] = __uint_as_float(x.y);
        d[2] = __uint_as_float(x.z); d[3] = __uint_as_float(x.w);
    }

    __device__ __forceinline__ float ld_b(__amdgpu_buffer_rsrc_t rs, int row, int pitch, int hi) const {
        row = row < -kGhostUV ? -kGhostUV : (row > hi ? hi : row);
        return __uint_as_float(__builtin_amdgcn_raw_buffer_load_b32(rs, 0, (row + kGhostUV) * pitch * 4, 0));
    }
    __device__ __forceinline__ void ld_rows(int t, int slot) {
        ld_u(UQ[slot], kb - 2 + t);
        ld_v(VQ[slot], kb - 1 + t);
        UB[slot] = ld_b(rs_us, kb - 2 + t, W, g->nyl + kGhostUV - 1);
        VB[slot] = ld_b(rs_vs, kb - 1 + t, g->nx, g->nyl + kGhostUV);
    }

    template <int T_, bool GEN, bool INT>
    __device__ __forceinline__ void step(int t) {
        constexpr bool I = INT && !GEN;
        const int k = kb + t;
        const int nx = g->nx;
        Fields ff = f;
        if (!MASK) ff.any_pmask = 0;
        float ux[6][8], vx[6][8];
#pragma unroll
        for (int r = 0; r < 6; ++r)
#pragma unroll
            for (int x = 0; x < 8; ++x) ux[r][x] = vx[r][x] = 0.0f;
#pragma unroll
        for (int r = 0; r < 5; ++r)
#pragma unroll
            for (int x = 0; x < 4; ++x) ux[r][2 + x] = UQ[(T_ + r) % D][x];
#pragma unroll
        for (int r = 1; r < 6; ++r)
#pragma unroll
            for (int x = 0; x < 4; ++x) vx[r][2 + x] = VQ[(T_ + r - 1) % D][x];
        ux[2][0] = from_left(ux[2][4]);
        ux[2][1] = from_left(ux[2][5]);
        ux[2][6] = from_right(ux[2][2]);
        ux[2][7] = from_right(ux[2][3]);
        ux[3][6] = from_right(ux[3][2]);
        vx[2][1] = from_left(vx[2][5]);
        vx[3][0] = from_left(vx[3][4]);
        vx[3][1] = from_left(vx[3][5]);
        vx[3][6] = from_right(vx[3][2]);
        vx[3][7] = from_right(vx[3][3]);
        const float ub = UB[(T_ + 2) % D], vb = VB[(T_ + 2) % D];
        ld_rows(t + D, T_ % D);

        const int rv = k + 1;
        float vn[4];
        if (!GEN || (rv >= glo && rv <= v_hi)) {
#pragma unroll
            for (int q = 0; q < 4; ++q)
                vn[q] = v_pred_val<SCHEME, SP, I>(*g, ff, dt, min(i0 + q, nx - 1), rv,
                                               MAcc<3>{ux, vx, q});
            if (c == 0) vn[0] = vb;
            if (st_lane && c < nch && (!GEN || t > 0 || r0 == 0))
                *reinterpret_cast<float4 *>(f.v_star + (long)rv * nx + i0) =
                    make_float4(vn[0], vn[1], vn[2], vn[3]);
        } else {
            const float4 a = c < nch ? *reinterpret_cast<const float4 *>(f.v_star + (long)rv * nx + i0)
                                     : make_float4(0.f, 0.f, 0.f, 0.f);
            vn[0] = a.x; vn[1] = a.y; vn[2] = a.z; vn[3] = a.w;
        }
        if (!GEN || t > 0) {
            float us[4];
            const long ku = (long)k * W + i0;
            const bool upred = !GEN || (k >= glo && k <= u_hi);
            if (upred) {
#pragma unroll
                for (int q = 0; q < 4; ++q)
                    us[q] = u_pred_val<SCHEME, SP, I>(*g, ff, dt, min(i0 + q, nx), k, MAcc<2>{ux, vx, q});
                if (c == 0) us[0] = ub;
            } else if (c <= nch) {
                const f4u a = *reinterpret_cast<const f4u *>(f.u_star + ku);
                us[0] = a.x; us[1] = a.y; us[2] = a.z; us[3] = a.w;
            } else {
                us[0] = us[1] = us[2] = us[3] = 0.0f;
            }
            const float east = from_right(us[0]);
            if (st_lane) {
                if (c < nch) {
                    if (upred) {
                        if (CFD_PM_USTORE == 0) {
                            *reinterpret_cast<f4u *>(f.u_star + ku) = (f4u){us[0], us[1], us[2], us[3]};
                        } else {
                            f.u_star[ku] = us[0];
                            f.u_star[ku + 1] = us[1];
                            f.u_star[ku + 2] = us[2];
                            f.u_star[ku + 3] = us[3];
                        }
                    }
                    const float rdx = g->r_dx, rdy = g->r_dy, dx = g->dx, dy = g->dy;
                    float4 rh;
                    rh.x = (sdiv<SP>(us[1] - us[0], dx, rdx) + sdiv<SP>(vn[0] - vs[0], dy, rdy)) / dt;
                    rh.y = (sdiv<SP>(us[2] - us[1], dx, rdx) + sdiv<SP>(vn[1] - vs[1], dy, rdy)) / dt;
                    rh.z = (sdiv<SP>(us[3] - us[2], dx, rdx) + sdiv<SP>(vn[2] - vs[2], dy, rdy)) / dt;
                    rh.w = (sdiv<SP>(east - us[3], dx, rdx) + sdiv<SP>(vn[3] - vs[3], dy, rdy)) / dt;
                    *reinterpret_cast<float4 *>(f.rhs + (long)k * nx + i0) = rh;
                } else if (c == nch && upred) {
                    f.u_star[ku] = us[0];
                }
            }
        }
#pragma unroll
        for (int q = 0; q < 4; ++q) vs[q] = vn[q];
    }

    template <int J, bool GEN, int OFF>
    __device__ __forceinline__ void group(int base) {
        if constexpr (J < D) {
            step<(OFF + J) % D, GEN>(base + J);
            group<J + 1, GEN, OFF>(base);
        }
    }

    template <int T, bool INT>
    __device__ __forceinline__ void steps() {
        if constexpr (T <= R) {
            step<T % D, (T < 2 || T == R), INT>(T);
            steps<T + 1, INT>();
        }
    }
    template <bool INT>
    __device__ __forceinline__ void run() {
#pragma unroll
        for (int t = 0; t < D; ++t) ld_rows(t, t);
        steps<0, INT>();
    }
};

template <int SCHEME, int SP, bool MASK, int R>
__global__ __launch_bounds__(kBlock, CFD_PM_WPE) void k_predict_march(Geom g, Fields f, float dt_override,
                                                          int glo, int u_hi, int v_hi, int nwc,
                                                          int nseg, int set_inlet, int row_lo,
                                                          int row_hi) {
    if (set_inlet && blockIdx.x == 0 && threadIdx.x == 0) {
        Ctl *c = f.ctl;
        const uint32_t st = c->step;
        c->inlet = st < 100u ? ((float)st / 100.0f) * g.target_inlet : g.target_inlet;
        c->go[0] = 1;
    }
    PredMarch<SCHEME, SP, MASK, R> m;
    const int wave = __builtin_amdgcn_readfirstlane((int)threadIdx.x >> 6);
    const int lane = (int)threadIdx.x & 63;
    const int bid = xcd_block(g);
    const int wc = bid % nwc;
    const int seg = (bid / nwc) * (kBlock / 64) + wave;
    if (seg >= nseg) return;
    const int nx = g.nx;
    m.r0 = row_lo + min(seg * R, row_hi - row_lo - R);
    m.r1 = m.r0 + R;
    m.g = &g;
    m.f = f;
    m.W = nx + 1;
    m.nch = nx / 4;
    m.c = wc * 62 - 1 + lane;
    const bool in_dom = m.c >= 0 && m.c <= m.nch;
    m.i0 = in_dom ? 4 * m.c : 0;
    m.st_lane = in_dom && lane >= 1 && lane <= 62;
    m.vo = in_dom ? 4 * m.i0 : 0x7FFF0000;
    m.rs_u = __builtin_amdgcn_make_buffer_rsrc(f.u_alloc_base, 0, (int)(f.u_alloc * 4), 0x00020000);
    m.rs_v = __builtin_amdgcn_make_buffer_rsrc(f.v_alloc_base, 0, (int)(f.v_alloc * 4), 0x00020000);
    m.rs_us = __builtin_amdgcn_make_buffer_rsrc(f.u_star_base, 0, (int)(f.u_alloc * 4), 0x00020000);
    m.rs_vs = __builtin_amdgcn_make_buffer_rsrc(f.v_star_base, 0, (int)(f.v_alloc * 4), 0x00020000);
    m.glo = glo;
    m.u_hi = u_hi;
    m.v_hi = v_hi;
    m.kb = m.r0 - 1;
    m.dt = dt_of(f.ctl, dt_override);
#pragma unroll
    for (int q = 0; q < 4; ++q) m.vs[q] = 0.0f;
    const int c_lo = wc * 62 - 1, c_hi = wc * 62 + 62;
    const bool interior = 4 * c_lo >= 3 && 4 * c_hi + 3 <= nx - 3 &&
                          g.j0 + m.r0 + 1 >= 2 && g.j0 + m.r1 - 2 <= g.ny - 3;
    if (SCHEME == 1 && interior)
        m.template run<true>();
    else
        m.template run<false>();
}

}

bool predict_march_ok(const Geom &g, const Fields &f) {
    auto a16 = [](const void *p) { return ((uintptr_t)p & 15u) == 0; };
    return g.pred_div == 2 && g.nx % 4 == 0 && g.nx >= 8 && g.nyl >= 4 && a16(f.v) && a16(f.v_star) &&
           a16(f.rhs) && (uint64_t)f.u_alloc * 4u < (1ull << 31) &&
           (uint64_t)f.v_alloc * 4u < (1ull << 31);
}

void launch_predict_march(const Geom &g, const Fields &f, float dt_override, hipStream_t s,
                          bool set_inlet, int row_lo, int row_hi) {
    if (row_hi < 0) row_hi = g.nyl;
    const int glo = (g.j0 > 1 ? g.j0 : 1) - g.j0;
    const int u_hi = ((g.j0 + g.nyl - 1) < (g.ny - 2) ? (g.j0 + g.nyl - 1) : (g.ny - 2)) - g.j0;
    const int v_hi = ((g.j0 + g.nyl) < (g.ny - 1) ? (g.j0 + g.nyl) : (g.ny - 1)) - g.j0;
    const int big = g.scheme == 0 ? CFD_PM_ROWS_FO : 8;
    const int span = row_hi - row_lo;
    const int rows = span >= big ? big : (span >= 8 ? 8 : 4);
    const int nwc = cdiv(g.nx / 4 + 1, 62);
    const int nseg = cdiv(row_hi - row_lo, rows);
    const dim3 grid(nwc * cdiv(nseg, kBlock / 64));
#define CFD_LAUNCH_PM(SC, SPV, MK, R)                                                              \
    hipLaunchKernelGGL((k_predict_march<SC, SPV, MK, R>), grid, dim3(kBlock), 0, s, g, f, dt_override, \
                       glo, u_hi, v_hi, nwc, nseg, set_inlet ? 1 : 0, row_lo, row_hi)
#define CFD_LAUNCH_PM3(SC, SPV, MK)                                         \
    if (CFD_PM_ROWS_FO != 8 && SC == 0 && rows == CFD_PM_ROWS_FO)           \
        CFD_LAUNCH_PM(SC, SPV, MK, (SC == 0 ? CFD_PM_ROWS_FO : 8));          \
    else if (rows == 8) CFD_LAUNCH_PM(SC, SPV, MK, 8); else CFD_LAUNCH_PM(SC, SPV, MK, 4)
#define CFD_LAUNCH_PM2(SC, SPV) \
    if (f.any_pmask) { CFD_LAUNCH_PM3(SC, SPV, true); } else { CFD_LAUNCH_PM3(SC, SPV, false); }
    if (g.scheme == 0) {
        if (g.sp_pow2) { CFD_LAUNCH_PM2(0, 1); } else { CFD_LAUNCH_PM2(0, 0); }
    } else {
        if (g.sp_pow2) { CFD_LAUNCH_PM2(1, 1); } else { CFD_LAUNCH_PM2(1, 0); }
    }
#undef CFD_LAUNCH_PM3
#undef CFD_LAUNCH_PM2
#undef CFD_LAUNCH_PM
}

}
```

include/cfd.h:

```cpp
#ifndef CFD_H
#define CFD_H

#include <stddef.h>
#include <stdint.h>

#ifdef __cplusplus
extern "C" {
#endif

#define CFD_ABI_VERSION 1

typedef enum {
    CFD_OK = 0,
    CFD_EINVAL = -1,
    CFD_EHIP = -2,
    CFD_ERCCL = -3,
    CFD_ESTATE = -4,
    CFD_ENONFINITE = -5,
    CFD_ETIMEOUT = -6,
} cfd_status;

typedef struct cfd_model cfd_model;

typedef struct {
    uint64_t nx, ny;
    float lx, ly;
    int32_t has_cylinder;
    float cylinder_x, cylinder_y, cylinder_radius;
} cfd_grid;

enum { CFD_SCHEME_FIRST_ORDER = 0, CFD_SCHEME_SECOND_ORDER = 1 };
enum { CFD_INLET_UNIFORM = 0, CFD_INLET_PARABOLIC = 1 };
enum { CFD_SOLVER_JACOBI = 0, CFD_SOLVER_SOR = 1, CFD_SOLVER_MULTIGRID = 2 };
enum { CFD_BC_CHANNEL = 0, CFD_BC_CAVITY = 1 };
typedef struct {
    float dt;
    float viscosity;
    float target_inlet_velocity;
    int32_t velocity_scheme;
    int32_t inlet_profile;
    int32_t pressure_solver;
    int32_t jacobi_iters;
    int32_t corrector_passes;
    int32_t tol_enabled;
    float p_tol;
    int32_t bc_kind;
} cfd_params;

typedef struct {
    uint64_t simulation_step;
    float simulation_time;
    float dt;
    float p, u, v;
    double step_time_s;
    uint32_t piso_substeps;
    uint64_t jacobi_sweeps_total;
} cfd_residuals;

typedef struct {
    float *u, *v, *p, *u_star, *v_star, *p_prime, *rhs;
    float dt;
    float simulation_time;
    uint64_t simulation_step;
    float last_p_residual, last_u_residual, last_v_residual;
    uint64_t jacobi_sweeps_total;
} cfd_state;

void cfd_default_params(cfd_params *out);
void cfd_default_grid(cfd_grid *out);

int cfd_create(const cfd_grid *grid, const cfd_params *params, int device_ordinal,
               cfd_model **out);

int cfd_rccl_unique_id(void *out_128_bytes);
int cfd_create_sharded(const cfd_grid *grid, const cfd_params *params, int device_ordinal,
                       int n_ranks, int rank, const void *rccl_unique_id, cfd_model **out);
void *cfd_local_hub_create(int n_ranks);
void cfd_local_hub_destroy(void *hub);
int cfd_create_sharded_local(const cfd_grid *grid, const cfd_params *params, int device_ordinal,
                             int n_ranks, int rank, void *hub, cfd_model **out);
int cfd_device_count(int *n_out);
int cfd_get_comm_size(const cfd_model *m, int *n_out);
int cfd_get_slab(const cfd_model *m, uint64_t *j0, uint64_t *j1);

int cfd_update(cfd_model *m);
int cfd_update_n(cfd_model *m, int n);
int cfd_piso_step(cfd_model *m, float dt_sub);
int cfd_pressure_solve(cfd_model *m, float *residual_out);

enum {
    CFD_PHASE_U_PREDICTOR = 0,
    CFD_PHASE_V_PREDICTOR = 1,
    CFD_PHASE_DIVERGENCE = 2,
    CFD_PHASE_CORRECTOR = 3,
    CFD_PHASE_BOUNDARY = 4,
};
int cfd_run_phase(cfd_model *m, int phase, float dt_sub);

int cfd_set_params(cfd_model *m, const cfd_params *params);
int cfd_get_snapshot(cfd_model *m, float *u, float *v, float *p, float *dt_out);
int cfd_get_residuals(cfd_model *m, cfd_residuals *out);
int cfd_get_state(cfd_model *m, cfd_state *st);
int cfd_set_state(cfd_model *m, const cfd_state *st);
int cfd_get_masks(cfd_model *m, uint8_t *mask_u, uint8_t *mask_v);

int cfd_synchronize(cfd_model *m);
int cfd_profile_sweeps(cfd_model *m, int n_sweeps, double *avg_ms_out);

int cfd_timing_begin(cfd_model *m);
int cfd_timing_end(cfd_model *m, double *solve_ms, uint64_t *sweeps, double *step_ms,
                   uint64_t *steps);
int cfd_timing_phases(cfd_model *m, int on);
int cfd_timing_phase_ms(const cfd_model *m, double *predict_ms, double *finish_ms);
int cfd_timing_exchange_ms(const cfd_model *m, double *exchange_ms, uint64_t *exchanges);
int cfd_get_halo_depth(const cfd_model *m);
int cfd_get_kernel_config(const cfd_model *m, int *fastdiv, int *temporal);
int cfd_get_jacobi_kernel(const cfd_model *m, int *kind, char *name, size_t name_len);

int cfd_get_persist_blocks(const cfd_model *m, int *blocks);
int cfd_get_persist_steals(cfd_model *m, uint64_t *steals);
int cfd_get_persist_sums(cfd_model *m, uint64_t *blocks);
int cfd_get_comm_calls(const cfd_model *m, uint64_t *n);
int cfd_get_recoveries(const cfd_model *m, uint64_t *n);
int cfd_get_resident_solves(const cfd_model *m, uint64_t *solves);
int cfd_get_jacobi_geometry(const cfd_model *m, int persist, int *lds_pad, int *wgs_per_cu,
                            int *wave_cols, int *segments);

int cfd_plan_slab(uint64_t ny, int n_ranks, int rank, uint64_t *j0, uint64_t *j1);
int cfd_plan_sweep(int j0, int nyl, int ny, int halo_depth, int it, int iters, int *lo, int *hi,
                   int *exchange);
int cfd_plan_halo(int kind, int nyl, int depth, int rank, int n_ranks, int *out6);
int cfd_plan_overlap(int nyl, int halo_depth, int rank, int n_ranks, int lo, int hi, int *out6);
int cfd_plan_block(int j0, int nyl, int ny, int halo_depth, int it, int t_max, int iters, int *T,
                   int *out_lo, int *out_hi, int *exchange);

typedef enum { CFD_VIS_PRESSURE = 0, CFD_VIS_VELOCITY = 1, CFD_VIS_VORTICITY = 2 } cfd_vis_mode;

int cfd_render(cfd_model *m, int mode, uint8_t *rgba, float *min_max_out);
int cfd_derive_field(cfd_model *m, int mode, float *out, float *min_max_out);

int cfd_get_config(const cfd_model *m, cfd_grid *grid, cfd_params *params);

typedef struct cfd_runner cfd_runner;
int cfd_run_start(cfd_model *m, cfd_runner **out);
int cfd_run_stop(cfd_runner *r);
int cfd_run_pause(cfd_runner *r);
int cfd_run_resume(cfd_runner *r);
int cfd_run_set_params(cfd_runner *r, const cfd_params *p);
int cfd_run_request_snapshot(cfd_runner *r);
int cfd_run_last_snapshot(cfd_runner *r, float *u, float *v, float *p, float *dt_out,
                          int *paused_out, int *available);
int cfd_run_new_residuals(cfd_runner *r, cfd_residuals *out, int max, int *n_out);
int cfd_run_status(cfd_runner *r, char *msg, size_t msg_len);
uint64_t cfd_run_steps(cfd_runner *r);

typedef struct { double x, y; } cfd_point;
typedef struct { cfd_point center; double half_width, half_height; } cfd_aabb;
enum { CFD_POLY_OK = 0, CFD_POLY_NOT_ENOUGH_VERTICES = 1, CFD_POLY_SELF_INTERSECTING = 2,
       CFD_POLY_INVALID_HOLE = 3 };
typedef struct cfd_polygon cfd_polygon;
typedef struct cfd_quadtree cfd_quadtree;
typedef struct cfd_mesh cfd_mesh;

int cfd_polygon_new(const cfd_point *vertex_buffer, size_t n_points, const uint64_t *vertices,
                    size_t n_vertices, cfd_polygon **out, int *poly_error);
int cfd_polygon_new_rect(double x, double y, double w, double h, cfd_polygon **out);
int cfd_polygon_new_regular(cfd_point center, double radius, size_t n, double start_angle,
                            cfd_polygon **out);
int cfd_polygon_add_hole(cfd_polygon *p, cfd_polygon *hole, int *poly_error);
int cfd_polygon_contains_point(const cfd_polygon *p, cfd_point pt, int *result);
int cfd_polygon_intersects_aabb(const cfd_polygon *p, const cfd_aabb *box, int *result);
int cfd_polygon_edges_intersect_aabb(const cfd_polygon *p, const cfd_aabb *box, int *result);
int cfd_polygon_bounding_box(const cfd_polygon *p, cfd_aabb *out);
int cfd_polygon_bounding_square(const cfd_polygon *p, cfd_aabb *out);
int cfd_polygon_edges(const cfd_polygon *p, cfd_point *out, size_t max_edges, size_t *n_edges);
void cfd_polygon_destroy(cfd_polygon *p);

int cfd_geom_do_intersect(cfd_point p, cfd_point q, cfd_point a, cfd_point b, int *result);
int cfd_geom_segment_intersection(cfd_point p, cfd_point q, cfd_point a, cfd_point b,
                                  cfd_point *out, int *found);
int cfd_geom_intersect_quad_edge(cfd_point center, double hw, double hh, cfd_point p1,
                                 cfd_point p2, cfd_point *out8, int *n);

int cfd_tesselate(const cfd_polygon *p, double feature_size, double max_cell_size,
                  cfd_quadtree **out);
int cfd_quadtree_size(const cfd_quadtree *t, uint64_t *n_nodes, uint64_t *n_leaves);
int cfd_quadtree_nodes(const cfd_quadtree *t, cfd_aabb *boxes, int64_t *children4);
void cfd_quadtree_destroy(cfd_quadtree *t);

enum { CFD_FACE_EAST = 0, CFD_FACE_WEST = 1, CFD_FACE_NORTH = 2, CFD_FACE_SOUTH = 3 };
int cfd_mesh_from_quadtree(const cfd_quadtree *t, const cfd_polygon *p, int device,
                           cfd_mesh **out);
int cfd_mesh_sizes(const cfd_mesh *m, uint64_t *sizes6);
int cfd_mesh_cells(const cfd_mesh *m, double *cx, double *cy, double *hw, double *hh);
int cfd_mesh_neighbors(const cfd_mesh *m, int face, uint64_t *ranges, uint64_t *indexes);
int cfd_mesh_intersections(const cfd_mesh *m, uint64_t *ranges, cfd_point *points);
int cfd_mesh_full_bounding_box(const cfd_mesh *m, cfd_aabb *out);
int cfd_mesh_build_ms(const cfd_mesh *m, double *ms);
void cfd_mesh_destroy(cfd_mesh *m);

const char *cfd_last_error(void);
int cfd_abi_version(void);
void cfd_destroy(cfd_model *m);

#ifdef __cplusplus
}
#endif
#endif
```

Before: 2752 billion.

## Use magnitude-bounded fused-sum Jacobi update in non-persistent LDS kernel

```diff
diff --git a/cfd-demo_amd/cfdamd/__init__.py b/cfd-demo_amd/cfdamd/__init__.py
--- a/cfd-demo_amd/cfdamd/__init__.py
+++ b/cfd-demo_amd/cfdamd/__init__.py
@@ -398,6 +398,12 @@
         return int(n.value)
 
     @property
+    def sums_launches(self) -> int:
+        n = C.c_uint64()
+        check("cfd_get_sums_launches", load().cfd_get_sums_launches(self._hh(), C.byref(n)))
+        return int(n.value)
+
+    @property
     def comm_calls(self) -> int:
         n = C.c_uint64()
         check("cfd_get_comm_calls", load().cfd_get_comm_calls(self._hh(), C.byref(n)))
diff --git a/cfd-demo_amd/cfdamd/_lib.py b/cfd-demo_amd/cfdamd/_lib.py
--- a/cfd-demo_amd/cfdamd/_lib.py
+++ b/cfd-demo_amd/cfdamd/_lib.py
@@ -15,7 +15,7 @@
     "cfd_get_residuals", "cfd_get_state", "cfd_set_state", "cfd_get_masks", "cfd_synchronize",
     "cfd_profile_sweeps", "cfd_timing_begin", "cfd_timing_end", "cfd_timing_phases",
     "cfd_timing_phase_ms", "cfd_timing_exchange_ms", "cfd_get_halo_depth",
-    "cfd_get_kernel_config", "cfd_get_jacobi_kernel", "cfd_get_persist_blocks", "cfd_get_persist_steals", "cfd_get_persist_sums", "cfd_get_recoveries", "cfd_get_comm_calls", "cfd_get_resident_solves", "cfd_get_jacobi_geometry", "cfd_plan_slab", "cfd_plan_sweep", "cfd_plan_halo", "cfd_plan_block", "cfd_plan_overlap",
+    "cfd_get_kernel_config", "cfd_get_jacobi_kernel", "cfd_get_persist_blocks", "cfd_get_persist_steals", "cfd_get_persist_sums", "cfd_get_sums_launches", "cfd_get_recoveries", "cfd_get_comm_calls", "cfd_get_resident_solves", "cfd_get_jacobi_geometry", "cfd_plan_slab", "cfd_plan_sweep", "cfd_plan_halo", "cfd_plan_block", "cfd_plan_overlap",
     "cfd_render", "cfd_derive_field", "cfd_last_error", "cfd_abi_version", "cfd_destroy",
     "cfd_get_config", "cfd_run_start", "cfd_run_stop", "cfd_run_pause", "cfd_run_resume",
     "cfd_run_set_params", "cfd_run_request_snapshot", "cfd_run_last_snapshot",
@@ -133,6 +133,7 @@
         "cfd_get_persist_blocks": (i32, [vp, C.POINTER(i32)]),
         "cfd_get_persist_steals": (i32, [vp, C.POINTER(C.c_uint64)]),
         "cfd_get_persist_sums": (i32, [vp, C.POINTER(C.c_uint64)]),
+        "cfd_get_sums_launches": (i32, [vp, C.POINTER(C.c_uint64)]),
         "cfd_get_recoveries": (i32, [vp, C.POINTER(C.c_uint64)]),
         "cfd_get_comm_calls": (i32, [vp, C.POINTER(C.c_uint64)]),
         "cfd_get_resident_solves": (i32, [vp, C.POINTER(C.c_uint64)]),
diff --git a/cfd-demo_amd/csrc/cfd_device.h b/cfd-demo_amd/csrc/cfd_device.h
--- a/cfd-demo_amd/csrc/cfd_device.h
+++ b/cfd-demo_amd/csrc/cfd_device.h
@@ -28,6 +28,11 @@
 
 __device__ __forceinline__ void publish_max(uint32_t *set, int key, float m) {
     if (m > 0.0f) atomicMax(&set[(key & (kResSlots - 1)) * kResStride], __float_as_uint(m));
+}
+
+__device__ __forceinline__ uint32_t abs_bits(float x) { return __float_as_uint(x) & 0x7fffffffu; }
+__device__ __forceinline__ void raise_bits_bound(uint32_t *word, uint32_t m, uint32_t thr) {
+    if (m > thr) atomicMax(word, m);
 }
 
 __device__ __forceinline__ bool nonfinite(float x) { return !(fabsf(x) <= 3.40282347e38f); }
@@ -124,6 +129,8 @@
         if (pass >= 0 && pass + 1 <= kMaxPasses)
             c->go[pass + 1] = (go && !(check_break && g.tol_enabled && c->last_p < g.p_tol)) ? 1 : 0;
         if (exact_flips >= 2) c->spec_stop = c->spec_redo = c->spec_launch = c->spec_launches = 0;
+        c->sums_state = 0u;
+        c->sums_m0 = 0u;
         go_s = go;
     }
     __syncthreads();
diff --git a/cfd-demo_amd/csrc/cfd_internal.h b/cfd-demo_amd/csrc/cfd_internal.h
--- a/cfd-demo_amd/csrc/cfd_internal.h
+++ b/cfd-demo_amd/csrc/cfd_internal.h
@@ -7,6 +7,7 @@
 namespace cfd {
 
 constexpr int kGhostUV = 2;
+constexpr float kSumsPLim = 0x1p122f, kSumsRLim = 0x1p112f;
 constexpr int kMaxSweeps = 4096;
 constexpr int kMaxPasses = 64;
 
@@ -32,10 +33,11 @@
     uint32_t red[7];
     uint32_t nonfinite_step;
     uint32_t vis[2];
-    uint32_t done;
+    uint32_t sums_state;
     uint64_t sweeps_total;
     int32_t spec_stop, spec_redo, spec_launch, spec_launches;
-    uint32_t spec_done;
+    uint32_t sums_launches;
+    uint32_t sums_m0, sums_rm;
     int32_t go[kMaxPasses + 1];
     uint32_t err[kMaxSweeps];
 };
@@ -81,6 +83,7 @@
     uint32_t *host_nonfinite;
     uint32_t *host_progress;
     uint32_t *persist;
+    int32_t sums_track;
 };
 
 void launch_step_begin(const Geom &g, const Fields &f, int copy, hipStream_t s);
diff --git a/cfd-demo_amd/csrc/cfd_jacobi_lds.h b/cfd-demo_amd/csrc/cfd_jacobi_lds.h
--- a/cfd-demo_amd/csrc/cfd_jacobi_lds.h
+++ b/cfd-demo_amd/csrc/cfd_jacobi_lds.h
@@ -60,7 +60,7 @@
     return ((need + q - 1) / q) * q;
 }
 
-template <int T, int FAST, int MODE, bool SUMS = false>
+template <int T, int FAST, int MODE, int SUMS = 0>
 struct LdsMarch {
     static constexpr bool RES = MODE == 1 || MODE == 5, SPEC = MODE == 2, REDO = MODE == 3;
     static constexpr bool PERSIST = MODE == 4 || MODE == 5;
@@ -132,7 +132,11 @@
         const f2 h = {hx, hy};
         const f2 v = Tp + B;
         f2 s;
-        if constexpr (SUMS) {
+        if constexpr (SUMS == 2) {
+            const f2 d = __builtin_elementwise_fma(h + v, (f2){r_dx_sq, r_dx_sq}, -Rh);
+            const f2 pu = d * r_denom;
+            return 0.75f * pu + 0.25f * C;
+        } else if constexpr (SUMS == 1) {
             s = (h + v) * r_dx_sq;
         } else {
             const f2 hz = fdiv2<FAST>(h, dx_sq, r_dx_sq);
@@ -304,7 +308,7 @@
     }
 };
 
-template <int T, int FAST, int MODE, bool SUMS = false>
+template <int T, int FAST, int MODE, int SUMS = 0>
 __device__ __forceinline__ void lds_block(const Geom &g, float *__restrict__ pa,
                                           float *__restrict__ pb, const float *__restrict__ rhs,
                                           Ctl *ctl, uint32_t *res_slots, int par, int out_lo,
@@ -457,7 +461,7 @@
 __global__ __launch_bounds__(kLdsWaves * 64, lds_min_waves(MODE)) void k_jacobi_lds(
     Geom g, float *__restrict__ pa, float *__restrict__ pb, const float *__restrict__ rhs,
     Ctl *ctl, uint32_t *res_slots, int pass, int par, int out_lo, int out_hi, int nwc, int nseg,
-    int wlo, int whi, int it, int lag) {
+    int wlo, int whi, int it, int lag, float sums_c) {
     using M = LdsMarch<T, FAST, MODE>;
     [[maybe_unused]] constexpr bool RES = M::RES;
     __shared__ f2 lds[kLdsWaves * M::D * 64];
@@ -507,6 +511,17 @@
             par = ctl->spec_launch;
         }
         if (nst <= 0) return;
+    }
+    if constexpr (FAST == 1 && MODE <= 1) {
+        if (sums_c > 0.0f && ctl->sums_state == 2u) {
+            const float bound = __uint_as_float(ctl->sums_m0) * g.r_dx_sq + sums_c * __uint_as_float(ctl->sums_rm);
+            if (bound < 0x1p123f) {
+                if (blockIdx.x == 0 && threadIdx.x == 0) atomicAdd(&ctl->sums_launches, 1u);
+                lds_block<T, FAST, MODE, 2>(g, pa, pb, rhs, ctl, res_slots, par, out_lo, out_hi, nwc, nseg,
+                                            wlo, whi, lds, nst, xcd_block(g));
+                return;
+            }
+        }
     }
     lds_block<T, FAST, MODE>(g, pa, pb, rhs, ctl, res_slots, par, out_lo, out_hi, nwc, nseg, wlo,
                              whi, lds, nst, xcd_block(g));
@@ -784,6 +799,15 @@
     return std::max(1, std::min(per_round * rounds, nrows / kMinRows));
 }
 
+inline bool lds_sums_grid(const Geom &g) {
+    const char *ue = getenv("CFD_JACOBI_SUMS");
+    int exp2 = 0;
+    const float R = g.r_dx_sq;
+    const bool pow2 = R >= 1.0f && std::frexp(R, &exp2) == 0.5f;
+    return !(ue && atoi(ue) == 0) && g.fastdiv == 1 && g.dx_sq == g.dy_sq && g.r_dx_sq == g.r_dy_sq &&
+           pow2;
+}
+
 template <int T, int MODE>
 void launch_lds_t(const Geom &g, const Fields &f, int pass, int par, int it, int out_lo, int out_hi,
                   uint32_t *rs, hipStream_t s, int lag = 0) {
@@ -800,9 +824,11 @@
     const int reach = T + 2;
     const int wlo = out_lo - reach <= 1 - g.j0 ? kEdgeWeight : 16;
     const int whi = out_hi + reach >= g.ny - 2 - g.j0 ? kEdgeWeight : 16;
-#define CFD_LDS_LAUNCH(FASTV)                                                                      \
+    const float sums_c =
+        MODE <= 1 && g.j0 == 0 && g.nyl == g.ny && lds_sums_grid(g) ? 0.1875f * kMaxSweeps : 0.0f;
+#define CFD_LDS_LAUNCH(FASTV)                                                                     \
     hipLaunchKernelGGL((k_jacobi_lds<T, FASTV, MODE>), grid, block, pad, s, g, pa, pb, f.rhs, f.ctl, \
-                       rs, pass, par, out_lo, out_hi, nwc, nseg, wlo, whi, it, lag)
+                       rs, pass, par, out_lo, out_hi, nwc, nseg, wlo, whi, it, lag, sums_c)
     if (g.fastdiv == 1)
         CFD_LDS_LAUNCH(1);
     else if (g.fastdiv == 2)
@@ -879,12 +905,8 @@
     const uint32_t steal = (uint32_t)std::min(4.0e9, st_us * 100.0);
     const char *le = getenv("CFD_PERSIST_LATE");
     const int late = le ? std::max(0, atoi(le)) : 0;
-    const char *ue = getenv("CFD_JACOBI_SUMS");
-    int exp2 = 0;
     const float R = g.r_dx_sq;
-    const bool pow2 = R >= 1.0f && std::frexp(R, &exp2) == 0.5f;
-    const int sums = !(ue && atoi(ue) == 0) && g.fastdiv == 1 && g.dx_sq == g.dy_sq &&
-                     g.r_dx_sq == g.r_dy_sq && pow2;
+    const int sums = lds_sums_grid(g);
     const float plim = sums ? std::ldexp(1.0f, 124) / R : 0.0f, rlim = std::ldexp(1.0f, 124);
 #define CFD_LDS_PLAUNCH(FASTV)                                                                     \
     hipLaunchKernelGGL((k_jacobi_persist<T, FASTV>), grid, block, pad, s, g, pa, pb, f.rhs, f.ctl, \
diff --git a/cfd-demo_amd/csrc/cfd_kernels.hip b/cfd-demo_amd/csrc/cfd_kernels.hip
--- a/cfd-demo_amd/csrc/cfd_kernels.hip
+++ b/cfd-demo_amd/csrc/cfd_kernels.hip
@@ -1072,6 +1072,7 @@
     Ctl *c = f.ctl;
     const int nx = g.nx;
     float du = 0.f, dv = 0.f, mu = 0.f, mv = 0.f;
+    uint32_t pm = 0u;
     bool bad = false;
     const int bid = xcd_block(g);
     const int i0 = 4 * ((bid % nbx) * kBlock + (int)threadIdx.x);
@@ -1092,10 +1093,21 @@
             if (lj < g.nyl || vrow) pc = *reinterpret_cast<const float4 *>(pp + (long)lj * nx + i0);
             cf4_row<SP>(g, f, pp, inlet, dt, i0, lj, pc, vrow ? pb : make_float4(0.f, 0.f, 0.f, 0.f),
                         du, dv, mu, mv, bad);
+            if (f.sums_track && lj < g.nyl)
+                pm = max(max(pm, max(abs_bits(pc.x), abs_bits(pc.y))), max(abs_bits(pc.z), abs_bits(pc.w)));
             pb = pc;
         }
     }
     flag_nonfinite(c, bad);
+    if (f.sums_track) {
+        const uint32_t thr = __float_as_uint(kSumsPLim * g.dx_sq);
+        raise_bits_bound(&c->sums_m0, pm, thr);
+        if (blockIdx.x == 0 && threadIdx.x == 0) {
+            atomicMax(&c->sums_m0, thr);
+            c->sums_rm = 0u;
+            c->sums_state = 1u;
+        }
+    }
     __shared__ float red[kBlock / 64][4];
     du = wave_max(du);
     dv = wave_max(dv);
diff --git a/cfd-demo_amd/csrc/cfd_model.hip b/cfd-demo_amd/csrc/cfd_model.hip
--- a/cfd-demo_amd/csrc/cfd_model.hip
+++ b/cfd-demo_amd/csrc/cfd_model.hip
@@ -1637,6 +1637,10 @@
         ck_open = false;
         ck_replay.clear();
     }
+    int invalidate_sums() {
+        HIP_TRY(hipMemsetAsync(&ctl->sums_state, 0, 4, stream));
+        return 0;
+    }
     int clear_abort_words() {
         HIP_TRY(hipMemset(f.persist, 0, (size_t)kPersistHeadLines * kPersistFlagStride * 4));
         return 0;
@@ -1764,6 +1768,16 @@
     m->g.tol_enabled = p->tol_enabled ? 1 : 0;
     m->g.p_tol = p->p_tol;
     m->g.jacobi_iters = p->jacobi_iters;
+}
+
+void set_sums_track(cfd_model *m) {
+    const Geom &g = m->g;
+    const char *ue = getenv("CFD_JACOBI_SUMS");
+    int e2 = 0;
+    const bool pow2 = g.r_dx_sq >= 1.0f && std::frexp(g.r_dx_sq, &e2) == 0.5f;
+    m->f.sums_track = !(ue && atoi(ue) == 0) && m->n_ranks == 1 && g.j0 == 0 && g.nyl == g.ny &&
+                      m->params.pressure_solver == CFD_SOLVER_JACOBI && !g.tol_enabled &&
+                      g.fastdiv == 1 && g.dx_sq == g.dy_sq && g.r_dx_sq == g.r_dy_sq && pow2;
 }
 
 std::mutex g_div_mu;
@@ -2017,6 +2031,8 @@
     f.vis_slots = f.red_slots + (size_t)4 * kResSlots * kResStride;
     f.persist = m->slots + (size_t)(kMaxSweeps + 16) * kResSlots * kResStride;
 
+    set_sums_track(m);
+
     Ctl c0;
     std::memset(&c0, 0, sizeof(c0));
     c0.dt = p->dt;
@@ -2280,6 +2296,7 @@
 int cfd_piso_step(cfd_model *m, float dt_sub) {
     if (!m) return fail(CFD_EINVAL, "null model");
     HIP_TRY(hipSetDevice(m->device));
+    if (int rc = m->invalidate_sums()) return rc;
     if (int rc = m->ck_begin()) return rc;
     auto run = [m, dt_sub]() {
         int rc = m->exchange_uv();
@@ -2294,6 +2311,7 @@
     if (!m) return fail(CFD_EINVAL, "null model");
     HIP_TRY(hipSetDevice(m->device));
     int rc;
+    if ((rc = m->invalidate_sums())) return rc;
     if (m->host_driven()) {
         return m->enqueue_solve_host_driven(residual_out);
     }
@@ -2315,6 +2333,7 @@
 int cfd_run_phase(cfd_model *m, int phase, float dt_sub) {
     if (!m) return fail(CFD_EINVAL, "null model");
     HIP_TRY(hipSetDevice(m->device));
+    if (int rc = m->invalidate_sums()) return rc;
     switch (phase) {
     case CFD_PHASE_U_PREDICTOR: {
         int rc = m->exchange_uv();
@@ -2353,6 +2372,9 @@
         m->host_cur = c.cur;
     }
     apply_params(m, p);
+    set_sums_track(m);
+    rc = m->invalidate_sums();
+    if (rc) return rc;
     HIP_TRY(hipMemcpy(&m->ctl->dt, &p->dt, 4, hipMemcpyHostToDevice));
     return 0;
 }
@@ -2498,6 +2520,8 @@
     c.nonfinite_step = 0;
     c.red[4] = 0;
     c.red[6] = 0;
+    c.sums_state = 0;
+    c.sums_m0 = 0;
     rc = m->clear_abort_words();
     if (rc) return rc;
     HIP_TRY(hipMemcpy(m->f.ctl, &c, offsetof(Ctl, go), hipMemcpyHostToDevice));
@@ -2526,6 +2550,7 @@
     if (!m) return fail(CFD_EINVAL, "null model");
     if (n_sweeps < 1 || n_sweeps > kMaxSweeps) return fail(CFD_EINVAL, "n_sweeps out of range");
     HIP_TRY(hipSetDevice(m->device));
+    if (int rc = m->invalidate_sums()) return rc;
     const int lo = std::max(0, 1 - (int)m->j0), hi = std::min(m->g.nyl, (int)m->g.ny - 1 - (int)m->j0);
     hipEvent_t a = m->ev_prof0, b = m->ev_prof1;
     Geom g = m->g;
@@ -2691,6 +2716,15 @@
     return 0;
 }
 
+int cfd_get_sums_launches(cfd_model *m, uint64_t *launches) {
+    if (!m || !launches) return fail(CFD_EINVAL, "null argument");
+    Ctl c;
+    int rc = m->read_ctl(&c);
+    if (rc) return rc;
+    *launches = c.sums_launches;
+    return 0;
+}
+
 int cfd_get_comm_calls(const cfd_model *m, uint64_t *n) {
     if (!m || !n) return fail(CFD_EINVAL, "null argument");
     *n = m->comm_calls;
diff --git a/cfd-demo_amd/csrc/cfd_predict_march.hip b/cfd-demo_amd/csrc/cfd_predict_march.hip
--- a/cfd-demo_amd/csrc/cfd_predict_march.hip
+++ b/cfd-demo_amd/csrc/cfd_predict_march.hip
@@ -37,6 +37,7 @@
     float VQ[D][4];
     float UB[D], VB[D];
     float vs[4];
+    uint32_t rmax;
     const Geom *g;
     Fields f;
     __amdgpu_buffer_rsrc_t rs_u, rs_v, rs_us, rs_vs;
@@ -154,6 +155,9 @@
                     rh.z = (sdiv<SP>(us[3] - us[2], dx, rdx) + sdiv<SP>(vn[2] - vs[2], dy, rdy)) / dt;
                     rh.w = (sdiv<SP>(east - us[3], dx, rdx) + sdiv<SP>(vn[3] - vs[3], dy, rdy)) / dt;
                     *reinterpret_cast<float4 *>(f.rhs + (long)k * nx + i0) = rh;
+                    if (f.sums_track)
+                        rmax = max(max(rmax, max(abs_bits(rh.x), abs_bits(rh.y))),
+                                   max(abs_bits(rh.z), abs_bits(rh.w)));
                 } else if (c == nch && upred) {
                     f.u_star[ku] = us[0];
                 }
@@ -196,6 +200,11 @@
         const uint32_t st = c->step;
         c->inlet = st < 100u ? ((float)st / 100.0f) * g.target_inlet : g.target_inlet;
         c->go[0] = 1;
+    }
+    if (f.sums_track && blockIdx.x == 0 && threadIdx.x == 0 && row_lo == 0 && row_hi == g.nyl &&
+        f.ctl->sums_state == 1u) {
+        atomicMax(&f.ctl->sums_rm, __float_as_uint(kSumsRLim));
+        f.ctl->sums_state = 2u;
     }
     PredMarch<SCHEME, SP, MASK, R> m;
     const int wave = __builtin_amdgcn_readfirstlane((int)threadIdx.x >> 6);
@@ -227,6 +236,7 @@
     m.dt = dt_of(f.ctl, dt_override);
 #pragma unroll
     for (int q = 0; q < 4; ++q) m.vs[q] = 0.0f;
+    m.rmax = 0u;
     const int c_lo = wc * 62 - 1, c_hi = wc * 62 + 62;
     const bool interior = 4 * c_lo >= 3 && 4 * c_hi + 3 <= nx - 3 &&
                           g.j0 + m.r0 + 1 >= 2 && g.j0 + m.r1 - 2 <= g.ny - 3;
@@ -234,6 +244,7 @@
         m.template run<true>();
     else
         m.template run<false>();
+    if (f.sums_track) raise_bits_bound(&f.ctl->sums_rm, m.rmax, __float_as_uint(kSumsRLim));
 }
 
 }
diff --git a/include/cfd.h b/include/cfd.h
--- a/include/cfd.h
+++ b/include/cfd.h
@@ -120,6 +120,7 @@
 int cfd_get_persist_blocks(const cfd_model *m, int *blocks);
 int cfd_get_persist_steals(cfd_model *m, uint64_t *steals);
 int cfd_get_persist_sums(cfd_model *m, uint64_t *blocks);
+int cfd_get_sums_launches(cfd_model *m, uint64_t *launches);
 int cfd_get_comm_calls(const cfd_model *m, uint64_t *n);
 int cfd_get_recoveries(const cfd_model *m, uint64_t *n);
 int cfd_get_resident_solves(const cfd_model *m, uint64_t *solves);
```

Result: faster. 2926 billion, median of 6 (+6.3%).
